# mierl/rootless-coll-mpi-ops

Measured on AMD Instinct MI355X. Metric: rootless bcast msgs/s, higher is better.
Workload: dtype u8; 1 GPU; rootless bcast storm over one world of 256 workgroup-ranks (256 per GPU), 64 B payload, random originators, 262144 bcasts per step; value = rootless bcasts/s, each delivered to all 255 other ranks; ranks_per_gpu=256, world_ranks=256, payload_bytes=64, waves_per_rank=8, parallelism=one world sharded over 1 GPU(s), contiguous rank ranges

## Files before the change

include/rlo_hip.h:

```cpp
#ifndef RLO_HIP_H
#define RLO_HIP_H
#include <stddef.h>
#include <stdint.h>

#ifdef __cplusplus
extern "C" {
#endif

#define RLO_OK 0
#define RLO_E_INVAL (-1)
#define RLO_E_HIP (-2)
#define RLO_E_OCCUPANCY (-3)
#define RLO_E_DEVICE (-4)
#define RLO_E_NOPROGRAM (-5)
#define RLO_E_NODEVICE (-6)
#define RLO_E_NOTCONNECTED (-7)
#define RLO_E_AGAIN (-8)
#define RLO_E_TIMEOUT (-9)
#define RLO_E_STALE (-10)

#define RLO_DERR_TIMEOUT 1
#define RLO_DERR_VOTE_RING 2
#define RLO_DERR_PID_COLLISION 3
#define RLO_DERR_VOTE_ORPHAN 4
#define RLO_DERR_LOG_FULL 5
#define RLO_DERR_BAD_SLOT 6
#define RLO_DERR_HOST_CMD 7
#define RLO_DERR_BULK 8
#define RLO_DERR_XCD 9

int rlo_topology(int n, int rank, int* level, int* last_wall, int* send_channel_cnt, int* send_list_len,
                 int* send_list );
int rlo_children(int n, int rank, int origin, int from , int* out );

typedef struct rlo_world rlo_world_t;

typedef struct {
    int32_t n_ranks;
    uint32_t max_payload;
    uint32_t ring_slots;
    int32_t device;
    uint64_t bulk_max;
    uint32_t bulk_slots;
    uint32_t movers;
    uint32_t proposal_pool;
    uint32_t flags;
} rlo_world_cfg_t;

typedef struct {
    int32_t n_ranks, max_in_degree, max_fanout, edges;
    uint32_t ring_slots, slot_stride, vote_slots;
    uint32_t peers;
    uint64_t fwd_bytes, vote_bytes, ctrl_bytes;
    int32_t cus, blocks_per_cu;
    int32_t part, n_parts, rank_begin, rank_end;
    int32_t sys_scope;
    int32_t waves;
    uint32_t bulk_slots, movers;
    uint64_t bulk_max, heap_bytes;
    uint32_t proposal_pool;
    uint32_t pull;
    uint32_t nsmall;
    uint32_t stage2_bytes;
    uint32_t ll_ok;
    uint32_t pend_hbm;
    uint32_t dyn_lds, static_lds;
    uint32_t last_kernel;
    uint32_t info_pad;
} rlo_world_info_t;

int rlo_world_create(const rlo_world_cfg_t* cfg, rlo_world_t** out);

#define RLO_PART_BLOB_BYTES 512u
#define RLO_PEER_OTHER_GPU 1u
#define RLO_PEER_IMPORTED 2u
#define RLO_PART_UNCACHED 1u
#define RLO_PART_PEND_HBM 4u
#define RLO_PART_ONE_XCD 8u
#define RLO_PART_CHUNKED 2u
typedef struct {
    int32_t n_ranks;
    int32_t n_parts, part;
    const int32_t* part_begin;
    uint32_t max_payload, ring_slots;
    int32_t device;
    uint32_t flags;
    uint64_t bulk_max;
    uint32_t bulk_slots, movers;
    uint32_t proposal_pool, pad;
} rlo_part_cfg_t;
int rlo_part_create(const rlo_part_cfg_t* cfg, rlo_world_t** out);
int rlo_part_export(rlo_world_t* w, void* blob, uint32_t cap);
int rlo_part_connect(rlo_world_t* w, const void* blobs , int n_parts);
int rlo_part_import(rlo_world_t* w, const void* blob , int q);
int rlo_world_destroy(rlo_world_t* w);
int rlo_part_close_imports(rlo_world_t* w);
int rlo_world_query(const rlo_world_t* w, rlo_world_info_t* out);

#define RLO_TRIM_IMPORTS 1u
#define RLO_TRIM_FREE 2u
#define RLO_TRIM_RETIRED 4u
#define RLO_TRIM_EXPORTED 8u
int rlo_pool_trim(uint32_t what, uint64_t* freed_bytes);
int rlo_pool_stats(uint64_t* out, uint32_t cap);

#define RLO_FLAG_LOG 1u
#define RLO_FLAG_HIST 2u
#define RLO_FLAG_PROF 4u
#define RLO_FLAG_TIMELINE 8u

#define RLO_ORDER_RANDOM 0u
#define RLO_ORDER_SLOTS 1u
typedef struct {
    uint64_t seed;
    int64_t k;
    uint32_t len;
    uint32_t window;
    uint32_t flags;
    uint32_t log_cap;
    uint32_t len_max;
    uint32_t order;
// ... 30 lines not shown
} rlo_log_rec_t;

typedef struct {
    uint32_t cmd_slots;
    uint32_t pickup_slots;
    uint32_t idle_timeout_s;
    uint32_t flags;
    uint32_t pool;
    uint32_t pad;
} rlo_host_cfg_t;
int rlo_program_host(rlo_world_t* w, const rlo_host_cfg_t* cfg);

#define RLO_CMD_BCAST 0u
#define RLO_CMD_PROPOSAL 2u
#define RLO_CMD_JUDGE 16u
#define RLO_CMD_OWN_JUDGE 17u
#define RLO_CMD_QUIT 18u
#define RLO_CMD_BULK 10u
#define RLO_CMD_BULK_RELEASE 19u
typedef struct {
    uint32_t kind;
    int32_t origin;
    int32_t id;
    uint32_t pseq;
    int32_t vote;
    uint32_t pad;
} rlo_cmd_t;
int rlo_host_post(rlo_world_t* w, int rank, const rlo_cmd_t* cmd, const void* payload, uint32_t len);

#define RLO_EV_DELIVER_BCAST (1u | (0u << 8))
#define RLO_EV_DELIVER_DECISION (1u | (4u << 8))
#define RLO_EV_DELIVER_BULK (1u | (10u << 8))
#define RLO_EV_ACTION 3u
#define RLO_EV_RESULT 4u
#define RLO_EV_JUDGE 6u
#define RLO_EV_OWN_JUDGE 7u
#define RLO_EV_JUDGED 8u
int rlo_host_poll(rlo_world_t* w, int rank, rlo_log_rec_t* ev, void* payload, uint32_t cap);
int rlo_host_running(rlo_world_t* w);
int rlo_host_cmd_count(rlo_world_t* w, int rank, uint64_t* consumed, uint64_t* posted);
int rlo_device_count(void);
int rlo_device_numa_node(int device);

typedef struct { uint32_t nchunks, stripe, chunk, tile, total_tiles, direct; } rlo_bulk_plan_t;
int rlo_bulk_plan(int n, uint64_t len, int cross, rlo_bulk_plan_t* out);
typedef struct {
    int32_t n_ranks, n_parts, part;
    uint32_t max_payload, ring_slots, flags;
    uint64_t bulk_max;
    uint32_t bulk_slots, movers, proposal_pool;
    int32_t cus;
} rlo_plan_cfg_t;
int rlo_layout_plan(const rlo_plan_cfg_t* cfg, rlo_world_info_t* out);
int rlo_storm_lengths(uint64_t seed, uint64_t k, uint32_t len, uint32_t len_max, uint32_t* out);
int rlo_host_bulk_stage(rlo_world_t* w, int rank, const void* data, uint64_t len, uint32_t timeout_us, uint32_t* q);
int rlo_host_bulk_copy(rlo_world_t* w, int rank, const rlo_log_rec_t* ev, void* dst);

int rlo_host_share(rlo_world_t* w, const char* shm_name, uint64_t stage_bytes);
int rlo_host_unlink(rlo_world_t* w);
int rlo_host_proxy(rlo_world_t* w);
int rlo_host_wait_started(rlo_world_t* w, uint32_t timeout_ms);
int rlo_host_fail(rlo_world_t* w);
int rlo_host_device_judge(rlo_world_t* w, const rlo_iar_cfg_t* cfg);

typedef struct rlo_client rlo_client_t;
int rlo_client_attach(const char* shm_name, int rank, rlo_client_t** out);
int rlo_client_detach(rlo_client_t* c);
int rlo_client_state(rlo_client_t* c);
int rlo_client_post(rlo_client_t* c, const rlo_cmd_t* cmd, const void* payload, uint32_t len);
int rlo_client_poll(rlo_client_t* c, rlo_log_rec_t* ev, void* payload, uint32_t cap);
int rlo_client_cmd_count(rlo_client_t* c, uint64_t* consumed, uint64_t* posted);
int rlo_client_bulk_put(rlo_client_t* c, const void* data, uint64_t len, uint32_t timeout_us, uint32_t* q);
int rlo_client_bulk_get(rlo_client_t* c, const rlo_log_rec_t* ev, void* dst);
int rlo_client_debug(rlo_client_t* c, uint64_t* out);
int rlo_client_hdiag(rlo_client_t* c, uint64_t* out);
int rlo_client_fwd(rlo_client_t* c, uint64_t* fwd, int64_t* fwd_ns);

int rlo_reset(rlo_world_t* w, void* stream);
#define RLO_LAUNCH_NO_RESET 1u
int rlo_launch_ex(rlo_world_t* w, void* stream, uint32_t flags);
int rlo_launch(rlo_world_t* w, void* stream);
int rlo_stream_create(int device, void** stream);
int rlo_stream_destroy(void* stream);
int rlo_wait(rlo_world_t* w);
int rlo_run(rlo_world_t* w, void* stream, float* kernel_ms);
int rlo_last_kernel_ms(rlo_world_t* w, float* ms);

typedef struct {
    uint64_t bcast_delivered, bcast_sum, originated;
    uint64_t dec_delivered, dec_approved, actions, judge_calls;
    uint64_t own_decided, own_approved, proposals_recv;
    uint64_t iterations, busy_iterations, stalls, log_count;
    uint64_t t_start, t_end;
    uint32_t error, error_aux;
    uint64_t prof[8];
    uint64_t dbg[8];
    uint32_t hist[128];
    uint64_t unmarked_slots;
} rlo_rank_stats_t;


int rlo_stats(rlo_world_t* w, rlo_rank_stats_t* out, int n);
int rlo_log(rlo_world_t* w, int rank, rlo_log_rec_t* out, uint32_t cap, uint8_t* payload, uint32_t payload_stride);
int rlo_latencies(rlo_world_t* w, uint64_t* ticks, uint32_t cap);
int rlo_round_ticks(rlo_world_t* w, uint64_t* ticks, uint32_t cap);

int rlo_device_error(rlo_world_t* w, uint32_t* code, uint32_t* aux);
int rlo_bulk_debug(rlo_world_t* w, uint64_t* out, uint32_t cap);
const char* rlo_strerror(int code);
int rlo_last_hip_error(void);

#ifdef __cplusplus
}
#endif
#endif
```

rootless-coll-mpi-ops_amd/csrc/rlo_device.hpp:

```cpp
#pragma once
#include <stdint.h>

namespace rlo {

constexpr int kBlock = 256;
constexpr int kWaves = kBlock / 64;
constexpr int kMaxFanout = 16;
constexpr int kMaxIn = 32;
constexpr int kMaxOut = 2 * kMaxFanout;
constexpr int kHdr = 16;
constexpr int kVoteSlot = 16;
constexpr int kMaxCand = 256;
constexpr int kStagePasses = 4;
constexpr int kHistBins = 128;
constexpr int kMaxParts = 64;
constexpr int kPoolMax = 16;
constexpr int kCtrlHdrWords = 16;
constexpr int kCtrlNonceWord = 15;
constexpr uint32_t kTlRoundsMax = 64, kTlGlobal = 8, kTlCols = 9;
enum TlCol : uint32_t { TLC_ARRIVE = 0, TLC_DONE = 1, TLC_PARENT = 2, TLC_ISSUE = 3, TLC_PASS = 4,
                        TLC_FWD = 5,
                        TLC_NEXT = 6,
                        TLC_P1 = 7, TLC_P2 = 8 };
enum TlEvent : uint32_t { TL_ORIGIN = 0, TL_POSTED = 1, TL_CLAIMED = 2, TL_MOVED = 3, TL_ROUND = 4, TL_VERIFIED = 5,
                          TL_GEN = 6, TL_DRAINED = 7 };
constexpr int kLatCap = 8192;
constexpr int kLatWords = 16 + kLatCap / 2;

enum Tag : uint32_t { TAG_BCAST = 0, TAG_PROPOSAL = 2, TAG_VOTE = 3, TAG_DECISION = 4, TAG_BULK = 10 };

enum Mode : uint32_t {
    MODE_STORM = 1u,
    MODE_LAT = 2u,
    MODE_IAR = 4u,
    MODE_LOG = 16u,
    MODE_HIST = 32u,
    MODE_PROF = 64u,
    MODE_LAZYPUB = 256u,
    MODE_NOSPIN = 512u,
    MODE_NOACQ = 1024u,
    MODE_NOFAST = 2048u,
    MODE_HDIAG = 4096u,
    MODE_PIPE = 8192u,
    MODE_LL = 16384u,
    MODE_TL = 32768u,
    MODE_HOPPROF = 131072u,
    MODE_NOHPW = 262144u,
    MODE_XCD1 = 524288u,
    MODE_CORRUPT = 65536u,
    MODE_HOST = 128u,
};

enum HostCmd : uint32_t { CMD_JUDGE = 16, CMD_OWN_JUDGE = 17, CMD_QUIT = 18, CMD_BULK_RELEASE = 19 };
constexpr int kHctlWords = 64;
constexpr int kHctlInjTail = 0, kHctlInjHead = 16, kHctlPkTail = 32, kHctlPkHead = 48;
constexpr int kHctlState = 40;
constexpr int kHctlDiag = 20;
constexpr int kHctlBeat = 41;

enum Judge : uint32_t { JUDGE_APPROVE = 0, JUDGE_MASK = 1, JUDGE_ISP = 2, JUDGE_HASH = 3 };

enum LogKind : uint32_t { LOG_DELIVER = 1, LOG_JUDGE = 2, LOG_ACTION = 3, LOG_RESULT = 4, LOG_ERROR = 5,
                          LOG_JREQ = 6,
                          LOG_OWN_JREQ = 7,
                          LOG_JUDGED = 8 };

enum Err : uint32_t { ERR_NONE = 0, ERR_TIMEOUT = 1, ERR_VOTE_RING = 2, ERR_PID_COLLISION = 3, ERR_VOTE_ORPHAN = 4,
                      ERR_LOG_FULL = 5, ERR_BAD_SLOT = 6, ERR_HOST_CMD = 7,
                      ERR_BULK = 8, ERR_XCD = 9 };


struct RankTopo {
    int32_t level, last_wall, scc, sll;
    int32_t send_list[kMaxFanout];
    int32_t n_in;
    int32_t in_src[kMaxIn];
    uint32_t in_data[kMaxIn][2];
    uint32_t vin_data[kMaxFanout];
    uint32_t inbox_ctrl, n_inbox;
    uint32_t outbox_ctrl, n_outbox;
    uint64_t out_ring[kMaxFanout][2];
    uint64_t out_tail[kMaxFanout][2];
    uint64_t in_head[kMaxIn][2];
    uint64_t vout_ring[kMaxIn];
    uint64_t vout_tail[kMaxIn];
    uint64_t vin_head[kMaxFanout];
    uint64_t in_base[kMaxIn];
    uint32_t orig_data, orig_pad;
    uint32_t in_bell, vin_bell;
    uint64_t out_bell[kMaxFanout];
    uint64_t vout_bell[kMaxIn];
};

constexpr uint32_t kBellChunks = 8;
__host__ __device__ inline uint32_t bell_tag(uint64_t s) { return ((uint32_t)s & 0x3fffffffu) + 1u; }
constexpr uint32_t kBellWords = 2 * kBellChunks * 2;

struct RankStats {
    uint64_t bcast_delivered, bcast_sum, originated;
    uint64_t dec_delivered, dec_approved, actions, judge_calls;
    uint64_t own_decided, own_approved, proposals_recv;
    uint64_t iterations, busy_iterations, stalls, log_count;
    uint64_t t_start, t_end;
    uint32_t error, error_aux;
    uint64_t prof[8];
    uint64_t dbg[8];
    uint32_t hist[kHistBins];
    uint64_t unmarked_slots;
};

constexpr uint32_t kPkRecBytes = 32, kPkMaxSlots = 16384, kPkNoPayload = 0xffffu, kPkTaggedPayload = 0x8000u;
__host__ __device__ inline uint32_t pk_tag(uint64_t seq, uint32_t epoch) { return (((uint32_t)seq << 1) | 1u) ^ epoch; }
__host__ __device__ inline uint32_t pk_tag16(uint64_t seq, uint32_t epoch) { return pk_tag(seq, epoch) & 0xffffu; }
__host__ __device__ inline uint32_t pk_payload_stride(uint32_t max_payload) { return max_payload >= 256u ? max_payload : 256u; }

struct LogRec {
    uint32_t kind;
    int32_t origin;
    int32_t from;
    uint32_t id;
    uint32_t len;
    int32_t vote;
    uint32_t aux;
    uint32_t payload_idx;
};

struct Params {
    int32_t n, rank_begin, rank_end;
    uint32_t mode;
    const RankTopo* topo;
    uint8_t* fwd_region;
    uint32_t fwd_region_bytes;
    uint32_t fwd_cap, fwd_stride;
    uint8_t* vote_region;
    uint32_t vote_region_bytes;
    uint32_t vote_cap;
    uint64_t* ctrl;
    uint32_t ctrl_bytes;
    uint32_t sys_scope;
    uint32_t n_parts;
    uint32_t* err_flag[kMaxParts];
    uint64_t seed;
    uint32_t len, window;
    const int64_t* sched_off;
    const uint32_t* sched_ids;
    const int64_t* expect_bcast;
    uint32_t lat_rounds;
    const int32_t* lat_origin;
    uint32_t* lat_count;
    uint64_t* lat_out;
    uint32_t* lat_round;
    uint32_t* xcd_word;
    uint64_t* lat_obs;
    uint32_t* tl;
    uint32_t tl_rounds;
    const uint32_t* lat_own_off;
    const uint32_t* lat_own;
    uint32_t judge_kind, judge_ppm;
    uint64_t judge_seed;
    const uint8_t* judge_mask;
    const char* judge_isp;
// ... 171 lines not shown
```

rootless-coll-mpi-ops_amd/csrc/rlo_kernel.hip:

```cpp
#include <hip/hip_runtime.h>

#include <type_traits>

#include "rlo_kernel_common.hpp"

namespace rlo {

struct CandL {
    uint32_t w0, id, w2, t0;
    uint32_t src;
    uint32_t need;
    uint32_t logidx;
    uint32_t kind, group;
    uint32_t relay;
};

struct PostReq {
    uint32_t cls, kind, origin, lr, slot, bid, len, ntiles, from, logidx, q, gen;
    uint64_t j0;
};
constexpr uint32_t kPostQ = 16;
struct BulkSh {
    PostReq pq[kPostQ];
    uint32_t npost;
    BulkJob mv_job;
    uint32_t mv_ti, mv_stop;
    unsigned long long mv_sum;
    uint32_t bq[kPass];
    uint32_t blen[kPass];
    uint32_t bact[kMaxPend];
    uint32_t nbact, ncomp;
    uint64_t fbase, dbase;
    uint32_t nstable;
    uint64_t cmask[kMaxPend / 64];
    uint32_t bonw[kMaxPend / 32];
    uint64_t sdone[8];
    uint32_t bulk_q;
};
struct NoBulkSh {};
struct BulkPend {
    uint32_t bid, len, ntiles;
    int32_t from;
    uint32_t t0, q, pad0, pad1;
};

template <int W, bool BULK>
struct Shared {
    typename std::conditional<BULK, BulkSh, NoBulkSh>::type b;
    static constexpr int kWaves = W, kMaxCand = 64 * W;
    RankTopo t;
    uint64_t ring_head[2 * kMaxIn];
    uint32_t ring_base[2 * kMaxIn], ring_take[2 * kMaxIn];
    uint64_t ract;
    uint64_t out_tail0[kMaxOut];
    uint32_t ofree[kMaxOut];
    uint32_t n_oi[kMaxOut];
    uint32_t R, C, nstorm, storm_base, loc_kind, lat_id, exit_now;
    uint32_t hbase, nh, ev_n, quit, gap_lo, gap_hi, nchmax;
    uint64_t hhead, hin_head, pk_tail;
    int64_t prop_idx;
    uint32_t storm_ids[kPass];
    uint64_t vhead[kMaxFanout];
    uint32_t vbase[kMaxFanout], va[kMaxFanout], vtot;
    uint32_t wcnt[kWaves][kMaxOut];
    uint32_t first_bad[kGroups];
    CandL cand[kMaxCand];
    alignas(16) uint16_t pos[kMaxCand][kMaxFanout];
    uint16_t big[kMaxCand];
    uint32_t nbig, bm, bq0, nblk;
    uint32_t blk_c[128], blk_q0[128];
    uint32_t nblk2[2];
    uint64_t vout_tail[kMaxIn], vout_head[kMaxIn];
    uint64_t pubw[4][64], snap[4][64];
    int32_t own_pid[kPoolMax];
    uint32_t own_word[kPoolMax], own_state[kPoolMax], own_decision[kPoolMax];
    uint32_t own_needed, own_rr;
    unsigned long long own_iter;
    int64_t own_n;
    uint32_t loc_nd, loc_n;
    uint8_t loc_slot[2 * kPoolMax];
    uint32_t lat_pos, lat_pos_n, lat_own_next, lat_seen, error, error_aux, progressed;
    uint32_t hwait;
    uint64_t hp[2];
    uint32_t a_done, cseq;
    uint64_t hd[8], hd_t0;
    uint64_t relay_tail, relay_rel;
    uint32_t relay_n, ref_any, rq_n, rq_h, relay_free;
    uint64_t rq_relay[kRelQ];
    uint64_t rq_out[kRelQ][kMaxOut];
    unsigned long long bcast_delivered, dec_delivered, dec_approved, actions, judge_calls, originated;
    unsigned long long own_decided, own_approved, proposals_recv, log_count, stalls, stale;
    uint64_t prof[8], prof_t, dbg[8];
    uint64_t hpt[9];
    uint32_t tl_clk[4];
    uint32_t tl_bfid;
    int64_t expect_dec;
    uint32_t hist[kHistBins];
};



// ... 518 lines not shown
                }
                for (int sh = 32; sh >= 1; sh >>= 1) acc += __shfl_xor(acc, sh);
                if ((tid & 63) == 0) atomicAdd((unsigned long long*)&S.mv_sum, acc);
            }
        }
        if (tid == 0) atomicAdd((unsigned long long*)&P.jctl[kJctlTilesDone + cls], (unsigned long long)jb.ntiles);
        if (jb.kind == JOB_VERIFY) {
            __syncthreads();
            if (tid == 0) {
                const uint32_t ps = jb.parent;
                (void)__hip_atomic_fetch_add(&P.jsum[cls * P.jslots + ps], (uint64_t)S.mv_sum, __ATOMIC_RELAXED,
                                             __HIP_MEMORY_SCOPE_AGENT);
                S.mv_sum = 0;
                __builtin_amdgcn_fence(__ATOMIC_RELEASE, "agent");
                asm volatile("s_waitcnt vmcnt(0)" ::: "memory");
                const uint32_t old = atomicAdd(&P.jdone[cls * P.jslots + ps], jb.ntiles);
                if (old + jb.ntiles == jb.total) {
                    __builtin_amdgcn_fence(__ATOMIC_ACQUIRE, "agent");
                    const uint64_t part = __hip_atomic_load(&P.jsum[cls * P.jslots + ps], __ATOMIC_RELAXED,
                                                            __HIP_MEMORY_SCOPE_AGENT);
                    const uint64_t tot = part + chunk_mix(0xFFFFFFFFu, u32x4{(uint32_t)o, jb.bid, TAG_BCAST, len});
                    atomicAdd((unsigned long long*)&P.stats[jb.lr].bcast_sum, (unsigned long long)tot);
                    if (jb.logidx != ~0u)
                        st_sys16(reinterpret_cast<u32x4*>(&P.log[(size_t)jb.lr * P.log_cap + jb.logidx]) + 1,
                                 u32x4{len, 0xffffffffu, (uint32_t)tot, (uint32_t)(tot >> 32)});
                    const uint32_t nt = n > 2 ? bulk_stripe_tiles(pl, len, (uint32_t)((me - o - 1 + n) % n)) : 0u;
                    bulk_slot_release(P, me, o, s, sys, bulk_total_tiles(pl, len) + nt, jb.bid);
                    tl_mark(P, jb.bid, TL_VERIFIED);
                    __hip_atomic_store(&P.jdone[cls * P.jslots + ps], 0u, __ATOMIC_RELAXED, __HIP_MEMORY_SCOPE_AGENT);
                    __hip_atomic_store(&P.jsum[cls * P.jslots + ps], 0ull, __ATOMIC_RELAXED, __HIP_MEMORY_SCOPE_AGENT);
                    __builtin_amdgcn_fence(__ATOMIC_RELEASE, "agent");
                    asm volatile("s_waitcnt vmcnt(0)" ::: "memory");
                    __hip_atomic_store(&P.jfree[cls * P.jslots + ps], (uint64_t)(jb.pjob >> lg) + 1ull, __ATOMIC_RELAXED,
                                       __HIP_MEMORY_SCOPE_AGENT);
                }
            }
        }
        BAR();
    }
}


constexpr uint32_t kPmAll = 0xFFFFFFFFu;
constexpr uint32_t kPmLat = ~(uint32_t)(MODE_STORM | MODE_IAR | MODE_HOST);
constexpr uint32_t kPmIar = ~(uint32_t)(MODE_STORM | MODE_LAT | MODE_HOST);
constexpr uint32_t kPmStorm = ~(uint32_t)(MODE_LAT | MODE_IAR | MODE_HOST);
constexpr uint32_t kPmHost = ~(uint32_t)(MODE_STORM | MODE_LAT);

template <int W, bool BULK, bool LL, bool PH = false, uint32_t PM = kPmAll>
__global__ __launch_bounds__(64 * W) void rlo_progress_kernel(Params P) {
#define PMODE(x) ((PM & (uint32_t)(x)) ? (P.mode & (uint32_t)(x)) : 0u)
#define PULL_ON (W == 4 && !BULK && P.pull != 0u)
    constexpr int kWaves = W, kBlock = 64 * W, kMaxCand = 64 * W;
    constexpr uint32_t kHostBase = kMaxCand - kPass;
    extern __shared__ __attribute__((aligned(16))) uint8_t dyn_lds[];
    __shared__ Shared<W, BULK> S;
    if constexpr (BULK) {
        if (blockIdx.x >= P.n_local) {
            if (threadIdx.x == 0) S.b.mv_sum = 0;
            __syncthreads();
            mover_run<W>(P, S, (int)threadIdx.x);
            return;
        }
    }
    const uint32_t nsmall = P.nsmall;
    const uint32_t nmagic = nsmall > 1 ? 0xFFFFFFFFu / nsmall + 1u : 0u;
    const uint32_t pend_bytes = P.pend_hbm ? 0u : 16u * (uint32_t)P.n * P.pend_slots;
    PendState* pend;
    if constexpr (PH)
        pend = (PendState*)(__attribute__((address_space(1))) PendState*)(P.pend_hbm + (size_t)blockIdx.x * (uint32_t)P.n * P.pend_slots);
    else
        pend = reinterpret_cast<PendState*>(dyn_lds);
    uint16_t* olist = reinterpret_cast<uint16_t*>(dyn_lds + pend_bytes);
    uint8_t* stage = dyn_lds + pend_bytes + P.nout_max * (2u * kMaxCand);
    uint8_t* stage2 = stage + (uint32_t)kMaxCand * nsmall * 16u;
    constexpr uint32_t kSubMax = W == 4 ? 4u : 1u;
    constexpr uint32_t kPair = W == 4 ? 2u : 1u;

    const uint32_t s2_units = P.stage2_bytes >> 10;
#define STG(c, q) (stage + (((uint32_t)(c) * nsmall + (uint32_t)(q)) << 4))
#define OL(oi, r) olist[(uint32_t)(oi) * (uint32_t)kMaxCand + (uint32_t)(r)]
#define PEND(o, q) pend[(uint32_t)(o) * P.pend_slots + ((uint32_t)(q) & (P.pend_slots - 1u))]

    const int lr = blockIdx.x;
    const int me = P.rank_begin + lr;
    const int tid = threadIdx.x, w = tid >> 6;
    int lane = tid & 63;
    uint64_t lt_mask = (1ull << lane) - 1ull;
    const __amdgpu_buffer_rsrc_t rf = mk_rsrc(P.fwd_region, P.fwd_region_bytes);
    const __amdgpu_buffer_rsrc_t rv = mk_rsrc(P.vote_region, P.vote_region_bytes);
    const uint32_t fcap_m = P.fwd_cap - 1, vcap_m = P.vote_cap - 1;
    const bool host = PM == kPmHost || (PMODE(MODE_HOST)) != 0;
    const bool eager = host || !(PMODE(MODE_LAZYPUB | MODE_STORM));
    const bool hjudge = host && P.host_judge != 0;
    const uint32_t my_mask = ((PMODE(MODE_IAR)) && !hjudge && P.judge_kind == JUDGE_MASK) ? P.judge_mask[me] : 0u;
    const __amdgpu_buffer_rsrc_t rh =
        mk_rsrc(host ? P.hin + (size_t)lr * P.hin_cap * P.fwd_stride : P.fwd_region, host ? P.hin_cap * P.fwd_stride : 16u);
    uint64_t* const hctl = host ? P.hctl + (size_t)lr * kHctlWords : nullptr;
    uint64_t* const hctl_dev = host ? P.hctl_dev + (size_t)lr * kHctlWords : nullptr;
    const uint32_t hcap_m = host ? P.hin_cap - 1u : 0u;
    constexpr uint32_t kLLCmdSlotB = kBellChunks * 32u;
    const __amdgpu_buffer_rsrc_t rll = mk_rsrc(host && P.hll ? P.hll + (size_t)lr * P.hin_cap * kLLCmdSlotB : P.fwd_region,
                                               host && P.hll ? P.hin_cap * kLLCmdSlotB : 16u);
    const bool ll_cmds = host && (uint32_t)kMaxCand * nsmall * 16u >= kLLCmdBell + 256u;
    [[maybe_unused]] BulkPend* const bpend = reinterpret_cast<BulkPend*>(dyn_lds + (BULK ? P.bpend_off : 0u));
    [[maybe_unused]] const uint32_t bsl = BULK ? P.bulk_slots : 1u;

    {
        const uint32_t* src = reinterpret_cast<const uint32_t*>(&P.topo[lr]);
        uint32_t* dst = reinterpret_cast<uint32_t*>(&S.t);
        for (int i = tid; i < (int)(sizeof(RankTopo) / 4); i += kBlock) dst[i] = src[i];
        if (PH || !P.pend_hbm)
            for (int i = tid; i < P.n * (int)P.pend_slots; i += kBlock) pend[i] = PendState{0, 0, 0, 0, 0, 0};
        if constexpr (BULK) {
            for (int i = tid; i < P.n * (int)P.bulk_slots; i += kBlock) bpend[i] = BulkPend{0u, 0u, 0u, -1, 0u, 0u, 0u, 0u};
        }
        for (int i = tid; i < kHistBins; i += kBlock) S.hist[i] = 0;
        for (int i = tid; i < 4 * 64; i += kBlock) { (&S.pubw[0][0])[i] = 0; (&S.snap[0][0])[i] = 0; }
        if (tid < kMaxIn) { S.vout_tail[tid] = 0; S.vout_head[tid] = 0; }
        if (tid < 8) { S.prof[tid] = 0; S.dbg[tid] = 0; S.hd[tid] = 0; }
        if (tid == 0) S.tl_bfid = 0;
        if (tid == 0) {
            S.prof_t = __builtin_amdgcn_s_memtime();
            for (int k = 0; k < kPoolMax; k++) {
                S.own_pid[k] = -1;
                S.own_word[k] = 0; S.own_state[k] = 0; S.own_decision[k] = 0;
            }
            S.own_needed = 0; S.own_rr = 0; S.loc_nd = 0; S.loc_n = 0;
            S.own_iter = 0;
            S.own_n = ((PMODE(MODE_IAR)) && !host) ? (P.prop_off[lr + 1] - P.prop_off[lr]) : 0;
            S.lat_pos = 0;
            S.lat_seen = 0;
            S.lat_pos_n = (PMODE(MODE_LAT)) ? P.lat_own_off[lr + 1] - P.lat_own_off[lr] : 0u;
            S.lat_own_next = S.lat_pos_n ? P.lat_own[P.lat_own_off[lr]] : 0xffffffffu;
            S.expect_dec = ((PMODE(MODE_IAR)) && !host) ? P.expect_dec[lr] : 0;
            S.hbase = 0; S.nh = 0; S.ev_n = 0; S.quit = 0; S.hhead = 0; S.hin_head = 0; S.pk_tail = 0;
            S.bcast_delivered = S.dec_delivered = S.dec_approved = S.actions = S.judge_calls = S.originated = 0;
            S.own_decided = S.own_approved = S.proposals_recv = S.log_count = S.stalls = S.stale = 0;
            S.error = 0; S.error_aux = 0; S.exit_now = 0; S.progressed = 0; S.hd_t0 = 0; S.hwait = 0;
            S.hp[0] = 0; S.hp[1] = 0; S.a_done = 0; S.cseq = 0;
            S.relay_tail = 0; S.relay_rel = 0; S.relay_n = 0; S.ref_any = 0; S.rq_n = 0; S.rq_h = 0; S.relay_free = 0;
            if constexpr (BULK) {
                S.b.nbact = 0; S.b.ncomp = 0; S.b.bulk_q = 0; S.b.nstable = 0; S.b.npost = 0;
                S.b.fbase = reinterpret_cast<uint64_t>(bulk_flags(P, me, 0, 0));
                S.b.dbase = reinterpret_cast<uint64_t>(bulk_done(P, me, 0u));
                for (int i = 0; i < kMaxPend / 64; i++) S.b.cmask[i] = 0;
                for (int i = 0; i < kMaxPend / 32; i++) S.b.bonw[i] = 0;
            }
        }
    }
    if constexpr (PH) VM_DRAIN();
    BAR();
    if (host && tid == 0) pub64_sys(&hctl[kHctlState], 1ull);
    if (!PH && P.pend_hbm && (PMODE(MODE_IAR | MODE_HOST)) && tid == 0) set_error(S, P, ERR_HOST_CMD, 0x9E4Du);
    const uint64_t t_start = now_ticks();
    unsigned long long acc_sum = 0;

    const RankTopo& t = S.t;
    const int level = uni(t.level), last_wall = uni(t.last_wall), scc = uni(t.scc), sll = uni(t.sll);
    const int n_in = uni(t.n_in), n_in2 = 2 * n_in, nout = 2 * sll;
    const uint32_t inbox = (uint32_t)uni((int)t.inbox_ctrl), outbox = (uint32_t)uni((int)t.outbox_ctrl);
    const uint32_t sl_r = lane < sll ? (uint32_t)t.send_list[lane] : 0u;
    const bool sys = P.sys_scope != 0;
    const uint32_t oring_bytes = P.fwd_cap * P.fwd_stride;
#define OTPTR t.out_tail[lane >> 1][lane & 1]
#define IHPTR t.in_head[lane >> 1][lane & 1]
#define VHPTR t.vin_head[lane]
#define VTPTR t.vout_tail[lane]
#define ORING(oi) uni64(t.out_ring[(oi) >> 1][(oi) & 1])
    uint64_t in_head_r = 0, out_tail_r = 0, vin_head_r = 0;
#define PUB_IN S.pubw[0][lane]
#define PUB_OUT S.pubw[1][lane]
#define PUB_VIN S.pubw[2][lane]
#define PUB_VOUT S.pubw[3][lane]
    uint32_t win_r = kMaxCand;
    uint64_t hpoll = 0;
    bool peer_failed = false;
    uint64_t idle_since = 0;
    uint32_t idle_n = 0;
    bool idle_prev = false;
    uint64_t p_h = 0;
    uint32_t p_lat = 0;
    const int64_t sched_base = (PMODE(MODE_STORM)) ? P.sched_off[lr] : 0;
    const int64_t sched_n = (PMODE(MODE_STORM)) ? P.sched_off[lr + 1] - sched_base : 0;
    const int64_t expect_bcast = (PMODE(MODE_STORM | MODE_LAT)) ? P.expect_bcast[lr] : 0;
    int64_t sched_next = 0;
    uint64_t n_iter = 0, n_busy = 0, n_stalls = 0;
    bool done_w0 = false;
    uint32_t rbase_r = 0, rtake_r = 0, noi_r = 0;
    const bool llm = LL && (PMODE(MODE_LL)) && !(PMODE(MODE_PROF | MODE_NOFAST));
    const bool hpw = W == 4 && host && llm && ll_cmds && P.hll != nullptr && !(P.mode & MODE_NOHPW);
    uint32_t a_it = 0;
    const __amdgpu_buffer_rsrc_t rc = mk_rsrc(P.ctrl, P.ctrl_bytes);
    const uint32_t in_bell = (uint32_t)uni((int)t.in_bell), vin_bell = (uint32_t)uni((int)t.vin_bell);
    bool ll_prog = false;

#define KIDS_U(o, f) (PM != kPmAll ? kids_of_u(me, (o), (f), level, last_wall, scc, sll, sl_r, lane) \
                               : kids_of(me, (o), (f), level, last_wall, scc, sll, sl_r))
#define NEED_U(k, o) (PM != kPmAll ? need_of_u((k), (o), sll, sl_r, lane) : need_of((k), (o), sll, sl_r))
    auto fwd_small = [&](u32x4 v, uint32_t nch, uint32_t need) {
        const uint32_t q = (uint32_t)lane;
        uint64_t obase = 0, bbase = 0;
        if constexpr (PM != kPmAll) {
            if (lane < nout) {
                obase = t.out_ring[lane >> 1][lane & 1];
                if (LL && llm) bbase = t.out_bell[lane >> 1];
            }
        }
        for (uint32_t m = need; m; m &= m - 1) {
            const int oi = __builtin_ctz(m);
            const uint64_t slot = rdl64(out_tail_r, oi);
            const __amdgpu_buffer_rsrc_t ro =
                mk_rsrc(reinterpret_cast<void*>(PM != kPmAll ? rdl64(obase, oi) : ORING(oi)), oring_bytes);
            if (q < nch) st_ring(ro, (uint32_t)(slot & fcap_m) * P.fwd_stride + 16u * q, v, sys);
            if (LL && llm && nch <= kBellChunks && q < nch) {
                const uint32_t T = bell_tag(slot) | ((uint32_t)(oi & 1) << 31);
                const __amdgpu_buffer_rsrc_t rb = mk_rsrc(
// ... 554 lines not shown

    auto lat_observe = [&](uint32_t latr) {
        const uint32_t done_r = rdl32(latr, 1), seen = S.lat_seen;
        if (done_r > seen) {
            const uint64_t tn = now_ticks();
            for (uint32_t k = seen + (uint32_t)lane; k < done_r && k < P.lat_rounds; k += 64u) P.lat_obs[k] = tn;
            if (lane == 0) S.lat_seen = done_r;
        }
    };

    auto bulk_eval = [&]() -> bool {
        bool any = false;
        if constexpr (BULK) {
            const uint32_t nb = (uint32_t)uni((int)S.b.nbact);
            if (TL_ON(P) && lane == 0) S.tl_clk[1] = (uint32_t)now_ticks();
            const __amdgpu_buffer_rsrc_t rfl = mk_rsrc(reinterpret_cast<void*>(uni64(S.b.fbase)), (uint32_t)P.n * bsl * kBulkLine);
            for (uint32_t u = 0; u * 64u < nb; u++) {
                const uint32_t i = u * 64u + (uint32_t)lane;
                bool dn = false;
                if (i < nb) {
                    const uint32_t e = S.b.bact[i];
                    uint32_t tc = 0;
                    if (e >= (uint32_t)P.n * bsl) {
                        bulk_fault(P, 7, e);
                    } else if (P.bulk_cross) {
                        tc = bflag_ld(reinterpret_cast<uint32_t*>(uni64(S.b.fbase) + (uint64_t)e * kBulkLine) + kBulkTflag, sys);
                    } else {
                        u32x4 q[4];
#pragma unroll
                        for (int k = 0; k < 4; k++) q[k] = sys ? ld_sys(rfl, e * kBulkLine + 16u * k) : ld_sc1(rfl, e * kBulkLine + 16u * k);
#pragma unroll
                        for (int k = 0; k < 4; k++) tc += q[k].x + q[k].y + q[k].z + q[k].w;
                    }
                    dn = e < (uint32_t)P.n * bsl && tc >= bpend[e].ntiles;
                    if (TL_ON(P) && dn) {
                        tl_put(P, bpend[e].bid, TLC_PASS, lr, (uint32_t)now_ticks());
                        tl_put(P, bpend[e].bid, TLC_ISSUE, lr, S.tl_clk[1]);
                    }
                }
                const uint64_t m = __ballot(dn);
                any |= m != 0ull;
                if (lane == 0) S.b.cmask[u] = m;
            }
            if (lane == 0) S.b.nstable = nb;
        }
        return any;
    };

    for (;;) {
        asm volatile("" : "+v"(lane));
        lt_mask = (1ull << lane) - 1ull;
        a_it++;
        uint64_t in_tail_r = 0, out_head_r = 0, vin_tail_r = 0, vout_head_r = 0;
        uint32_t errf = 0, sid = 0, latr = 0;
        if (w == 0) {
            uint32_t ll_run = 0;
            bool bev = false;
            uint64_t dnw = 0;
            for (uint32_t sp = 0;; sp++) {
                bev = false;
                if (hpw) {
                    if (lane < 2) hpoll = S.hp[lane];
                } else if (host && lane < 2 && ((sp & 3u) == 0u || S.hwait != 0u)) {
                    hpoll = poll64_sys(&hctl_dev[lane == 0 ? kHctlInjTail : kHctlPkHead]);
                }
                if (TL_ON(P) && lane == 0) {
                    S.tl_clk[0] = (uint32_t)now_ticks();
                    if (BULK && S.tl_bfid) { tl_put(P, S.tl_bfid - 1u, TLC_NEXT, lr, S.tl_clk[0]); S.tl_bfid = 0; }
                }
                [[maybe_unused]] u32x4 ba, bb, vb;
                if constexpr (LL) {
                    const uint32_t bk = (uint32_t)lane >> 3, bq = (uint32_t)lane & 7u;
                    const uint32_t bo = llm && (int)bk < n_in ? (in_bell + bk * kBellWords) * 8u + 32u * bq : kOob;
                    ba = ld_sc1(rc, bo);
                    bb = ld_sc1(rc, bo == kOob ? kOob : bo + 16u);
                    vb = ld_sc1(rc, llm && lane < sll ? (vin_bell + 2u * (uint32_t)lane) * 8u : kOob);
                }
                in_tail_r = ld64_sc1(rc, lane < n_in2 ? (inbox + (uint32_t)lane) * 8u : kOob);
                vin_tail_r = ld64_sc1(rc, lane < sll ? (inbox + (uint32_t)(n_in2 + lane)) * 8u : kOob);
                out_head_r = ld64_sc1(rc, lane < nout ? (outbox + (uint32_t)lane) * 8u : kOob);
                vout_head_r = ld64_sc1(rc, lane < n_in ? (outbox + (uint32_t)(nout + lane)) * 8u : kOob);
                errf = ld32_sc1(rc, 0u);
                if constexpr (BULK) {
                    const __amdgpu_buffer_rsrc_t rd = mk_rsrc(reinterpret_cast<void*>(uni64(S.b.dbase)), bsl * kBulkLine);
                    dnw = ld64_sys(rd, lane < (int)bsl ? (uint32_t)lane * kBulkLine : kOob);
                }
                if constexpr ((PM & MODE_LAT) != 0u)
                    latr = __hip_atomic_load((PMODE(MODE_LAT)) ? P.lat_round : P.error_flag, __ATOMIC_RELAXED,
                                             __HIP_MEMORY_SCOPE_SYSTEM);
                if constexpr (LL) {
                    if (llm) {
                        if ((PMODE(MODE_LAT)) && me == 0) lat_observe(latr);
                        bool need_full = false;
                        const uint32_t nb0 = nact_of(S.b);
                        const uint32_t nll = ll_pass(ba, bb, vb, in_tail_r, vin_tail_r, out_head_r, hpoll, latr, errf, need_full);
                        if (nll) ll_prog = true;
                        if (need_full) { SPIN_WHY(2); break; }
                        if (BULK && nact_of(S.b) != nb0) { SPIN_WHY(3); break; }
                        if (nll) {
                            if (++ll_run < 64u) { sp = 0; continue; }
                            SPIN_WHY(3);
                            break;
                        }
                    }
                }
                if ((PMODE(MODE_LAT)) && me == 0 && !(LL && llm)) lat_observe(latr);
                if (!idle_prev || sp >= kIdleSpin) { SPIN_WHY(idle_prev ? 1 : 0); break; }
                bool bmoved = false;
                if constexpr (BULK) {
                    if (uni((int)S.b.npost) != 0) { SPIN_WHY(4); break; }
                    if (uni((int)S.b.nbact) != 0) {
                        bev = true;
                        if (bulk_eval()) { SPIN_WHY(5); break; }
                    }
                    bmoved = lane < (int)bsl && dnw != S.b.sdone[lane];
                }
                const bool moved =
                    llm ? (in_tail_r != S.snap[0][lane] && in_tail_r > in_head_r) ||
                              (vin_tail_r != S.snap[1][lane] && vin_tail_r > vin_head_r) ||
                              (latr != p_lat && rdl32(latr, 1) == S.lat_own_next) || errf != 0
                        : in_tail_r != S.snap[0][lane] || vin_tail_r != S.snap[1][lane] || out_head_r != S.snap[2][lane] ||
                              vout_head_r != S.snap[3][lane] || hpoll != p_h || latr != p_lat || errf != 0 || bmoved;
                if (__ballot(moved)) { SPIN_WHY(6); break; }
            }
            if (hpw && lane == 0) S.a_done = a_it;
            S.snap[0][lane] = in_tail_r; S.snap[1][lane] = vin_tail_r; S.snap[2][lane] = out_head_r;
            S.snap[3][lane] = vout_head_r; p_h = hpoll; p_lat = latr;
            if (host && (n_iter & 4095u) == 0 && lane < 3) pub64_sys(&hctl[kHctlBeat + lane], lane == 2 ? n_iter : hpoll);
            if constexpr (BULK) {
                if (lane < (int)bsl) S.b.sdone[lane] = dnw;
                if (!bev) (void)bulk_eval();
            }
            if ((PMODE(MODE_LAT)) && me == 0) lat_observe(latr);
            if ((PMODE(MODE_STORM)) && sched_next + lane < sched_n && (uint32_t)lane < P.window)
                sid = P.sched_ids[sched_base + sched_next + lane];
        } else if (hpw && w == 1) {
            for (;;) {
                const uint64_t hh = uni64(S.hin_head);
                const uint8_t* slot = reinterpret_cast<const uint8_t*>(
                    uni64(reinterpret_cast<uint64_t>(P.hll + ((uint64_t)lr * P.hin_cap + (hh & hcap_m)) * kLLCmdSlotB)));
                su16 sa;
                uint64_t ht = 0, hk = 0;
                u32x4 cv = {0u, 0u, 0u, 0u};
                uint32_t scov = 2u;
                if constexpr (PM == kPmHost) {
                    su16 sb;
                    su8 sc;
                    spoll_cmd5(slot, &hctl_dev[kHctlInjTail], &hctl_dev[kHctlPkHead], sa, sb, sc, ht, hk);
#pragma unroll
                    for (int p = 0; p < 4; p++) {
                        if (lane == p) cv = u32x4{sa[4 * p], sa[4 * p + 1], sa[4 * p + 2], sa[4 * p + 3]};
                        if (lane == 4 + p) cv = u32x4{sb[4 * p], sb[4 * p + 1], sb[4 * p + 2], sb[4 * p + 3]};
                    }
                    if (lane == 8) cv = u32x4{sc[0], sc[1], sc[2], sc[3]};
                    if (lane == 9) cv = u32x4{sc[4], sc[5], sc[6], sc[7]};
                    scov = 5u;
                } else {
                    spoll_cmd(slot, &hctl_dev[kHctlInjTail], &hctl_dev[kHctlPkHead], sa, ht, hk);
#pragma unroll
                    for (int p = 0; p < 4; p++)
                        if (lane == p) cv = u32x4{sa[4 * p], sa[4 * p + 1], sa[4 * p + 2], sa[4 * p + 3]};
                }
                if (lane == 0) { S.hp[0] = ht; S.hp[1] = hk; }
                {
                    const uint32_t T0 = bell_tag(hh);
                    const bool head_ok = sa[1] == T0 && sa[3] == T0 && sa[5] == T0 && sa[7] == T0;
                    if (head_ok && ((kHdr + (sa[4] & 0xffffu) + 15u) >> 4) > scov && lane >= (int)(2u * scov) && lane < 16)
                        cv = ld_sys(rll, (uint32_t)(hh & hcap_m) * kLLCmdSlotB + 16u * (uint32_t)lane);
                }
                const uint32_t T = bell_tag(hh);
                const uint64_t tok = __ballot(lane < 16 && cv.y == T && cv.w == T);
                const uint32_t cn = (kHdr + (rdl32(cv.x, 1) & 0xffffu) + 15u) >> 4;
                const uint64_t cm = (1ull << (2u * min(cn, kBellChunks))) - 1ull;
                if ((tok & 3ull) == 3ull && cn <= kBellChunks && (tok & cm) == cm &&
                    (uint32_t)uni((int)S.cseq) != T) {
                    if (lane == 0) *lds_word(&S.cseq) = 0u;
                    asm volatile("s_waitcnt lgkmcnt(0)" ::: "memory");
                    if (lane < 16)
                        *lds_dword(stage + kLLCmdBell + 8u * (uint32_t)lane) = (uint64_t)cv.x | ((uint64_t)cv.z << 32);
                    asm volatile("s_waitcnt lgkmcnt(0)" ::: "memory");
                    if (lane == 0) *lds_word(&S.cseq) = T;
                }
                if (__builtin_amdgcn_readfirstlane((int)S.a_done) == (int)a_it) break;
            }
        }
        VM_DRAIN();
        BAR();
        PROF_STAMP(0);

        if (w == 0) {
            if (lane < nout && out_tail_r != PUB_OUT) { PUB_OUT = out_tail_r; pub64(OTPTR, out_tail_r, sys); }
            if (lane < n_in2 && in_head_r != PUB_IN) { PUB_IN = in_head_r; pub64(IHPTR, in_head_r, sys); }
            if (lane < sll && vin_head_r != PUB_VIN) { PUB_VIN = vin_head_r; pub64(VHPTR, vin_head_r, sys); }
            if (lane < n_in) {
                const uint64_t vt = S.vout_tail[lane];
                if (vt != PUB_VOUT) { PUB_VOUT = vt; pub64(VTPTR, vt, sys); }
                S.vout_head[lane] = vout_head_r;
            }
            peer_failed = __builtin_amdgcn_readfirstlane(errf) != 0;
            PSX(1);
            uint32_t relay_free = kMaxCand;
            if (PULL_ON) {
                const uint32_t nq = S.rq_n;
                uint32_t nrel = 0, e = S.rq_h;
                uint64_t rel = S.relay_rel;
                for (; nrel < nq; nrel++, e = (e + 1u) % (uint32_t)kRelQ) {
                    const bool ok = lane >= nout || out_head_r >= S.rq_out[e][lane];
                    if (__ballot(!ok)) break;
                    rel = S.rq_relay[e];
                }
                if (lane == 0 && nrel) { S.rq_h = e; S.rq_n = nq - nrel; S.relay_rel = rel; }
                const uint64_t used = S.relay_tail - rel;
                relay_free = used >= P.relay_cap ? 0u : P.relay_cap - (uint32_t)used;
                if (lane == 0) S.relay_free = relay_free;
            }
            bool hblock = false;
            uint32_t hlim = kMaxCand;
            if (host) {
                if (lane == 0) pub64_sys(&hctl[kHctlInjHead], S.hin_head);
                if (lane == 1) pub64_sys(&hctl[kHctlPkTail], S.pk_tail);
                const uint64_t pk_head = rdl64(hpoll, 1);
                const uint32_t pk_free = P.log_cap - (uint32_t)(S.pk_tail - pk_head);
                const uint32_t own_ev = 2u * P.own_pool + 2u;
                hblock = pk_free < own_ev + 4u;
                hlim = hblock ? 0u : (pk_free - own_ev) / 2u;
                if ((PMODE(MODE_HDIAG)) && lane == 0) {
                    S.hd[3]++;
                    if (hblock) S.hd[2]++;
                }
            }
            if constexpr (BULK) {
                const uint32_t nb = S.b.nbact;
                const uint32_t nst = S.b.nstable;
                if (nb) {
                    uint32_t climit = kMaxPend;
                    if (host) {
                        const uint32_t pk_free = P.log_cap - (uint32_t)(S.pk_tail - rdl64(hpoll, 1));
                        climit = pk_free >= 24u ? (pk_free - 16u) / 2u : 0u;
                    }
                    uint32_t seen = 0, kept = 0;
                    for (uint32_t u = 0; u * 64u < nb; u++) {
                        const uint32_t i = u * 64u + (uint32_t)lane;
                        const uint64_t m = S.b.cmask[u];
                        const uint64_t mv = u * 64u < nst ? m & (nst - u * 64u >= 64u ? ~0ull : ((1ull << (nst - u * 64u)) - 1ull)) : 0ull;
                        bool fin = ((mv >> lane) & 1ull) && seen + (uint32_t)__popcll(mv & lt_mask) < climit;
// ... 204 lines not shown
                    nh = run;
                    gap_lo = C;
                    hbase = kHostBase + ncp;
                    if ((uint32_t)lane >= ncp && (uint32_t)lane < ncp + nh) {
                        S.cand[kHostBase + lane].src = (uint32_t)((S.hin_head + lane) & hcap_m) * P.fwd_stride;
                        S.cand[kHostBase + lane].group = kGroupLocal + K_HOST;
                    }
                    if (lane == 0) { S.hhead = S.hin_head + ncp; S.hin_head += ncp; }
                    if (nh) C = hbase + nh;
                }
            }
            if (!LL && (PMODE(MODE_STORM)) && sched_next < sched_n) {
                const bool deep = lane < nout && (out_tail_r - out_head_r) * 2 >= P.fwd_cap;
                const bool allow = !backlog && R < 2 * kPass && __ballot(deep) == 0;
                if ((PMODE(MODE_PROF)) && lane == 0) { if (!allow) S.dbg[5]++; else S.dbg[2]++; }
                if (allow) {
                    const int64_t rem = sched_n - sched_next;
                    uint32_t ww = rem < (int64_t)P.window ? (uint32_t)rem : P.window;
                    if (ww > kMaxCand - C) ww = kMaxCand - C;
                    if constexpr (BULK) {
                        uint32_t ln = 0, isb = 0;
                        if ((uint32_t)lane < ww) {
                            ln = P.len_hi > P.len_lo ? storm_len_of(P.seed, sid, P.len_lo, P.len_hi) : P.len;
                            isb = ln > P.ring_cap ? 1u : 0u;
                        }
                        uint32_t nbk = 0;
                        const uint32_t q = S.b.bulk_q + wave_excl_scan(isb, &nbk);
                        const bool ok = !isb || S.b.sdone[q & (bsl - 1u)] >= (uint64_t)(q / bsl) * (uint64_t)(P.n - 1);
                        const uint64_t bad = __ballot((uint32_t)lane < ww && !ok);
                        if (bad) ww = (uint32_t)__builtin_ctzll(bad);
                        if (bad && lane == 0) atomicAdd((unsigned long long*)&P.jctl[kJctlSlotWaits], 1ull);
                        if ((uint32_t)lane < ww) {
                            S.b.bq[lane] = isb ? q : ~0u;
                            S.b.blen[lane] = ln;
                        }
                    }
                    storm_base = C;
                    nstorm = ww;
                    C += ww;
                    if ((uint32_t)lane < ww) S.storm_ids[lane] = sid;
                }
            }
            if ((PMODE(MODE_LAT)) && C < kMaxCand) {
                bool lat_ok = true;
                if constexpr (BULK) {
                    if (P.len > P.ring_cap) {
                        const uint32_t q = S.b.bulk_q;
                        lat_ok = S.b.sdone[q & (bsl - 1u)] >= (uint64_t)(q / bsl) * (uint64_t)(P.n - 1);
                    }
                }
                if (lat_ok && S.lat_own_next != 0xffffffffu && rdl32(latr, 1) == S.lat_own_next) { lat_id = S.lat_own_next; C++; }
            }
            uint32_t fastdone = 0;
            if ((!host || hlim >= 2u) && R == 1u && C == 1u && vtot == 0u && !(PMODE(MODE_PROF | MODE_NOFAST))) {
                const int fg = __builtin_ctzll(__ballot(lane < n_in2 && take > 0u));
                const uint64_t h0 = rdl64(in_head_r, fg);
                const uint32_t fsrc = (uint32_t)uni((int)t.in_data[fg >> 1][fg & 1]) + (uint32_t)(h0 & fcap_m) * P.fwd_stride;
                u32x4 v = {0u, 0u, 0u, 0u};
                if ((uint32_t)lane < nsmall) v = ld_sc1(rf, fsrc + 16u * (uint32_t)lane);
                const uint32_t fneed = lone(v, fg, fsrc, false, out_head_r);
                if (fneed == kHeld || fneed == kAsked) {
                    VM_DRAIN();
                    if (lane == fg) rtake_r = 0u;
                    R = 0;
                    C = 0;
                    fastdone = fneed == kAsked ? 1u : 0u;
                } else if (fneed != ~0u) {
                    VM_DRAIN();
                    noi_r = lane < nout ? ((fneed >> lane) & 1u) : 0u;
                    R = 0;
                    C = 0;
                    fastdone = 1;
                }
            }
            if (lane == 0) {
                S.ract = ract;
                S.vtot = vtot;
                S.R = R; S.C = C; S.nstorm = nstorm; S.storm_base = storm_base; S.loc_kind = loc_kind;
                S.lat_id = lat_id; S.prop_idx = prop_idx; S.nbig = 0; S.progressed = fastdone | (ll_prog ? 1u : 0u);
                S.hbase = hbase; S.nh = nh; S.gap_lo = gap_lo; S.gap_hi = hbase; S.nchmax = 0;
                S.exit_now = done_w0;
                if (PMODE(MODE_PROF)) S.dbg[0] += R;
            }
            ll_prog = false;
        }
        BAR();
        PST(7, 3);
        if (S.exit_now) {
            if constexpr (BULK) {
                if (w == 0) flush_posts(S.b, P, lane);
            }
            break;
        }
        const uint32_t R = S.R, C = S.C;
        const uint32_t nstorm = S.nstorm, storm_base = S.storm_base, loc_kind = S.loc_kind;

        if (C != 0 || S.vtot != 0) {
            const uint32_t vtot = S.vtot;
            u32x4 vreg[4] = {{0u, 0u, 0u, 0u}, {0u, 0u, 0u, 0u}, {0u, 0u, 0u, 0u}, {0u, 0u, 0u, 0u}};
            if (w == 1 && vtot) {
    #pragma unroll
                for (int u = 0; u < 4; u++) {
                    const uint32_t i = (uint32_t)u * 64u + lane;
                    if (i < vtot) {
                        int j = 0;
                        while (i >= S.vbase[j] + S.va[j]) j++;
                        const uint64_t slot = S.vhead[j] + (i - S.vbase[j]);
// ... 266 lines not shown
                    const uint32_t x = S.wcnt[v][lane];
                    if (v < w) pre += x;
                    tot += x;
                }
                const uint32_t f = S.ofree[lane];
                room_r = f > pre ? f - pre : 0u;
                tight_l = tot > f;
            }
            bool fits = active && judge >= 0;
            for (uint32_t m = wneed & (uint32_t)__ballot(tight_l); m; m &= m - 1) {
                const int oi = __builtin_ctz(m);
                const bool bit = (need >> oi) & 1u;
                const uint64_t b = __ballot(bit);
                if (b && bit && (uint32_t)__popcll(b & lt_mask) >= rdl32(room_r, oi)) {
                    fits = false;
                    if ((PMODE(MODE_PROF | MODE_HIST)) == MODE_PROF) atomicAdd(&S.hist[oi], 1u);
                }
            }
            if (active && !fits) atomicMin(&S.first_bad[group], c);
            BAR();
            const bool admitted = active && fits && c < S.first_bad[group];
            const uint32_t an = admitted ? need : 0u;
            const uint32_t len = w2 & 0xffffu;
            const bool isbig = admitted && ((kHdr + len + 15u) >> 4) > nsmall;
            const uint32_t nch_s = (kHdr + len + 15u) >> 4;
            const uint32_t wadm = wave_or(an);
            for (uint32_t m = wave_or(active && !admitted ? need : 0u); m; m &= m - 1) {
                const int oi = __builtin_ctz(m);
                const uint64_t b = __ballot((an >> oi) & 1u);
                if (lane == 0) S.wcnt[w][oi] = (uint32_t)__popcll(b);
            }
            {
                const uint32_t mx = wave_max(admitted && !isbig ? (kHdr + len + 15u) >> 4 : 0u);
                if (lane == 0 && mx) atomicMax(&S.nchmax, mx);
            }
            BAR();
            uint32_t pre_r = 0;
            if (lane < nout) {
                uint32_t tot = 0;
                for (int v = 0; v < kWaves; v++) {
                    const uint32_t x = S.wcnt[v][lane];
                    if (v < w) pre_r += x;
                    tot += x;
                }
                if (w == 0) { S.n_oi[lane] = tot; noi_r = tot; }
            }
            for (uint32_t m = wadm; m; m &= m - 1) {
                const int oi = __builtin_ctz(m);
                const bool bit = (an >> oi) & 1u;
                const uint64_t b = __ballot(bit);
                if (bit) {
                    const uint32_t rel = rdl32(pre_r, oi) + (uint32_t)__popcll(b & lt_mask);
                    OL(oi, rel) = (uint16_t)(c | (isbig ? kBigFlag : (nch_s << 9)));
                    if (isbig) S.pos[c][oi >> 1] = (uint16_t)rel;
                }
            }
            const uint64_t amask = __ballot(admitted);
            PST(3, 7);

            const uint32_t tag = (w0 >> 16) & 0xffu;
            const int vote = (int)(int8_t)(w0 >> 24);
            const uint32_t pseq = w2 >> 24;
            uint32_t logidx = ~0u;
            bool lat_deliv = false;
            uint32_t lat_tn = 0;
            if (admitted) {
                if (kind == K_RING) {
                    if (tag == TAG_BCAST) {
                        if (PMODE(MODE_HIST | MODE_LAT)) {
                            const uint64_t tn = now_ticks();
                            if (PMODE(MODE_HIST)) atomicAdd(&S.hist[hist_bin((uint32_t)tn - t0)], 1u);
                            if (PMODE(MODE_LAT)) {
                                tl_mark(P, id, kTlGlobal + (uint32_t)lr);
                                tl_parent(P, id, lr, from);
                                lat_deliv = true;
                                lat_tn = (uint32_t)tn - t0;
                            }
                        }
                        logidx = log_put<PM>(S, P, lr, LOG_DELIVER | (TAG_BCAST << 8), origin, from, id, len, -1,
                                         (uint32_t)now_ticks() - t0);
                    } else if (tag == TAG_PROPOSAL) {
                        const int32_t pid = (int32_t)id;
                        const int k = (int)(group >> 1);
                        atomicAdd(&S.proposals_recv, 1ull);
                        if (own_has(S, P, pid)) {
                            set_error(S, P, ERR_PID_COLLISION, (uint32_t)pid);
                        } else {
                            atomicAdd(&S.judge_calls, 1ull);
                            if (!host) log_put<PM>(S, P, lr, LOG_JUDGE, origin, from, (uint32_t)pid, len, judge, 0);
                            else if (!hjudge) {
                                const uint32_t slot = log_put<PM>(S, P, lr, LOG_JUDGED, origin, from, (uint32_t)pid, len, judge,
                                                              pseq);
                                uint8_t* dst = P.log_payload + ((size_t)lr * P.log_cap + slot) * P.log_stride;
                                for (uint32_t q = 0; 16u * q < len && 16u * q < P.log_stride; q++)
                                    st_sys16(dst + 16u * q, ld_sc1(rf, src + kHdr + 16u * q));
                            }
                            PendState* ps = &PEND(origin, pseq);
                            if (!judge) {
                                ps->valid = PS_NONE;
                                emit_vote<LL>(S, P, me, (uint32_t)k, origin, pid, pseq, 0);
                            } else {
                                const uint32_t nk = (uint32_t)__builtin_popcount(kids);
                                ps->pid = pid;
                                ps->word = 0;
                                ps->parent_k = (uint16_t)k;
                                ps->needed = (uint8_t)nk;
                                ps->pseq = pseq | ((len - 16u) << 8);
// ... 187 lines not shown
                    if (cl.kind == K_RING) {
                        if (PULL_ON && ((cl.w2 >> 16) & 0xffu) == kRefMark) {
                            const u32x4 ref = *reinterpret_cast<const u32x4*>(STG(cc, 1));
                            const uint32_t roff = (uint32_t)uni((int)ref.x);
                            const bool rok = uni((int)ref.y) == (int)~roff && (uint32_t)uni((int)ref.z) == kRefMagic;
                            if (!rok && lane == 0) set_error(S, P, ERR_BAD_SLOT, 0x5EF0000u | (pq & 0xffffu));
                            const __amdgpu_buffer_rsrc_t rr =
                                mk_rsrc(reinterpret_cast<void*>(uni64(t.in_base[cl.group >> 1]) + roff),
                                        (uint32_t)uni((int)(rok ? (pch + 1u) * 16u : 0u)));
                            if (rok && pq < pch) {
                                if (sys) __builtin_amdgcn_raw_ptr_buffer_load_lds(rr, lds_ptr(dst), 16, 16u * (pq + 1u), 0, 0, kAuxSc1 | 1);
                                else __builtin_amdgcn_raw_ptr_buffer_load_lds(rr, lds_ptr(dst), 16, 16u * (pq + 1u), 0, 0, kAuxSc1);
                            }
                        } else if (pq < pch) {
                            dma16(rf, dst, cl.src + 16u * (pq + 1u));
                        }
                    } else if (cl.kind == K_HOST) {
                        if (pq < pch)
                            __builtin_amdgcn_raw_ptr_buffer_load_lds(rh, lds_ptr(dst), 16, cl.src + 16u * (pq + 1u), 0, 0, kAuxSc1 | 1);
                    } else if (pq < pch) {
                        *reinterpret_cast<u32x4*>(dst + 16u * lane) =
                            gen_chunk(P, cl.kind, me, cl.id, cl.w2 & 0xffffu, cl.src, (int)(int8_t)(cl.w0 >> 24), pq + 1u);
                    }
                    }
                }
            };
            auto big_drain = [&]() {
                if ((PMODE(MODE_PROF)) && tid == 0) {
                    const uint64_t c0 = __builtin_amdgcn_s_memtime();
                    VM_DRAIN();
                    S.dbg[3] += __builtin_amdgcn_s_memtime() - c0;
                    if (!PULL_ON) S.dbg[4]++;
                } else {
                    VM_DRAIN();
                }
            };
            if (nbig) {
                if (tid == 0) { S.bm = 0; S.bq0 = 0; }
                plan_big(0u);
                BAR();
                issue_big(0u);
                big_drain();
                ACQ_NEXT();
            }

#ifdef RLO_AB_NQ2
            const uint32_t nq = min(max(S.nchmax, 1u), 2u);
#else
            const uint32_t nq = max(S.nchmax, 1u);
#endif
            const uint32_t qmagic = nq > 1 ? 0xFFFFFFFFu / nq + 1u : 0u;
            const uint32_t dr = div_small(64u, qmagic), dq = 64u - dr * nq;
            const uint32_t stg_msg = nsmall << 4, stride = P.fwd_stride;
            const uint32_t nit_r = lane < nout ? S.n_oi[lane] * nq : 0u;
            uint32_t items = 0;
            const uint32_t ibase_r = wave_excl_scan(nit_r, &items);
            const uint32_t lo = items * (uint32_t)w / (uint32_t)kWaves, hi = items * (uint32_t)(w + 1) / (uint32_t)kWaves;
            for (uint64_t mo = __ballot(nit_r != 0 && ibase_r < hi && ibase_r + nit_r > lo); mo; mo &= mo - 1) {
                const int oi = __builtin_ctzll(mo);
                const uint32_t ib = rdl32(ibase_r, oi), ie = ib + rdl32(nit_r, oi);
                const uint32_t a = max(lo, ib) - ib, b = min(hi, ie) - ib;
                const uint32_t s0 = (uint32_t)S.out_tail0[oi];
                const __amdgpu_buffer_rsrc_t ro = mk_rsrc(reinterpret_cast<void*>(ORING(oi)), oring_bytes);
                uint32_t i = a + (uint32_t)lane;
                uint32_t r = div_small(i, qmagic), q = i - r * nq;
                for (; i < b; i += 256u) {
                    uint32_t rr[4], qq[4], e[4];
                    rr[0] = r;
                    qq[0] = q;
#pragma unroll
                    for (int u = 1; u < 4; u++) {
                        rr[u] = rr[u - 1] + dr;
                        qq[u] = qq[u - 1] + dq;
                        if (qq[u] >= nq) { qq[u] -= nq; rr[u]++; }
                    }
#pragma unroll
                    for (int u = 0; u < 4; u++) e[u] = i + 64u * u < b ? (uint32_t)OL(oi, rr[u]) : (uint32_t)kBigFlag;
                    u32x4 x[4];
#pragma unroll
                    for (int u = 0; u < 4; u++) {
                        const bool v = !(e[u] & kBigFlag) && qq[u] < ((e[u] >> 9) & 0x3fu);
                        x[u] = u32x4{0u, 0u, 0u, 0u};
                        if (v) x[u] = *reinterpret_cast<const u32x4*>(stage + __umul24(e[u] & 0x1ffu, stg_msg) + (qq[u] << 4));
                        e[u] = v ? 1u : 0u;
                    }
#pragma unroll
                    for (int u = 0; u < 4; u++)
                        if (e[u]) st_ring(ro, __umul24((s0 + rr[u]) & fcap_m, stride) + (qq[u] << 4), x[u], sys);
                    r = rr[3] + dr;
                    q = qq[3] + dq;
                    if (q >= nq) { q -= nq; r++; }
                }
            }
            if (admitted && !isbig && kind == K_RING && tag == TAG_BCAST) {
                const uint32_t nch = (kHdr + len + 15u) >> 4;
                acc_sum += chunk_mix(0xFFFFFFFFu, u32x4{(uint32_t)origin, id, TAG_BCAST, len});
                for (uint32_t q = 1; q < nch; q++) {
                    const u32x4 v = *reinterpret_cast<const u32x4*>(STG(c, q));
                    acc_sum += chunk_mix(q - 1u, v);
                    if (logidx != ~0u)
                        st_sys16(P.log_payload + ((size_t)lr * P.log_cap + logidx) * P.log_stride + 16u * (q - 1), v);
                }
            }


            if (nbig) {
                constexpr bool kRegs = W == 4;
                const uint32_t ot0_r = kRegs && lane < nout ? (uint32_t)S.out_tail0[lane] : 0u;
                const uint64_t oring_r = kRegs && lane < nout ? t.out_ring[lane >> 1][lane & 1] : 0ull;
#define G3_SLOT(oi) (kRegs ? rdl32(ot0_r, oi) + rdl32(posr, (oi) >> 1) : (uint32_t)S.out_tail0[oi] + S.pos[cc][(oi) >> 1])
#define G3_RING(oi) (kRegs ? rdl64(oring_r, oi) : ORING(oi))
                uint32_t cur = 0;
                for (;;) {
                    const bool more = S.bm < nbig;
                    if (more && pipe) {
                        BAR();
                        plan_big(cur ^ 1u);
                        BAR();
                        issue_big(cur ^ 1u);
                    }
                    const uint32_t nblk = S.nblk2[cur];
                    for (uint32_t b0 = (uint32_t)w; b0 < nblk; b0 += kWaves) {
                        const uint32_t b = cur * hg + b0;
                        const uint32_t cc = S.blk_c[b], qw = S.blk_q0[b], q0b = qw & 0xffffu;
                        const CandL& cl = S.cand[cc];
                        const uint32_t blen = cl.w2 & 0xffffu, pch = (blen + 15u) >> 4;
                        const uint32_t nsub = min(gsub, (pch - q0b + 63u) >> 6);
                        const uint32_t rly = cl.relay;
                        const uint32_t posr = kRegs && lane < sll ? (uint32_t)S.pos[cc][lane] : 0u;
                        const bool hdr = q0b == 0u && lane == 0;
                        const uint32_t hw2 = cl.w2 & 0xff00ffffu;
                        const bool bc = cl.kind == K_RING && ((cl.w0 >> 16) & 0xffu) == TAG_BCAST;
                        if (bc && hdr) acc_sum += chunk_mix(0xFFFFFFFFu, u32x4{cl.w0 & 0xffffu, cl.id, TAG_BCAST, blen});
                        if (PULL_ON && rly != ~0u && q0b == 0u) {
                            const u32x4 hv = lane == 0 ? u32x4{cl.w0, cl.id, hw2 | (kRefMark << 16), cl.t0}
                                                       : u32x4{rly, ~rly, kRefMagic, 0u};
                            for (uint32_t a2 = (uint32_t)uni((int)cl.need); a2; a2 &= a2 - 1) {
                                const int oi = __builtin_ctz(a2);
                                const uint32_t slot = G3_SLOT(oi);
                                const __amdgpu_buffer_rsrc_t ro = mk_rsrc(reinterpret_cast<void*>(G3_RING(oi)), oring_bytes);
                                if (lane <= 1) st_ring(ro, (slot & fcap_m) * P.fwd_stride + 16u * lane, hv, sys);
                            }
                        }
                        for (uint32_t u0 = 0; u0 < nsub; u0 += kPair) {
// ... 16 lines not shown
#pragma unroll
                                    for (uint32_t u = 0; u < kPair; u++)
                                        if (u0 + u < nsub && pq + 64u * u < pch) st_ring(ro, s0 + 16u * (pq + 1u) + 1024u * u, vv[u], sys);
                                    if (hdr && u0 == 0u) st_ring(ro, s0, hv, sys);
                                }
                            }
                            if (bc) {
#pragma unroll
                                for (uint32_t u = 0; u < kPair; u++) {
                                    const uint32_t pp = pq + 64u * u;
                                    if (u0 + u < nsub && pp < pch) {
                                        acc_sum += chunk_mix(pp, vv[u]);
                                        if (cl.logidx != ~0u && 16u * (pp + 1u) <= P.log_stride)
                                            st_sys16(P.log_payload + ((size_t)lr * P.log_cap + cl.logidx) * P.log_stride + 16u * pp, vv[u]);
                                    }
                                }
                            }
                        }
                    }
                    if (!more) break;
                    if (pipe) {
                        cur ^= 1u;
                    } else {
                        BAR();
                        plan_big(cur);
                        BAR();
                        issue_big(cur);
                    }
                    big_drain();
                    ACQ_NEXT();
                }
#undef G3_SLOT
#undef G3_RING
            }
            if (lat_deliv) {
                const uint32_t old = sys ? __hip_atomic_fetch_add(&P.lat_count[id], 1u, __ATOMIC_RELAXED, __HIP_MEMORY_SCOPE_SYSTEM)
                                         : atomicAdd(&P.lat_count[id], 1u);
                if (old + 1u == (uint32_t)(P.n - 1)) {
                    tl_mark(P, id, TL_ROUND);
                    P.lat_out[id] = (uint64_t)lat_tn;
                    if (sys) __hip_atomic_store(P.lat_round, id + 1u, __ATOMIC_RELAXED, __HIP_MEMORY_SCOPE_SYSTEM);
                    else __hip_atomic_store(P.lat_round, id + 1u, __ATOMIC_RELAXED, __HIP_MEMORY_SCOPE_AGENT);
                }
            }
            PST(5, 7);
        }

        if (eager && (C != 0 || S.vtot != 0)) {
            VM_DRAIN();
            BAR();
        }
        if (w == 0) {
            if constexpr (BULK) flush_posts(S.b, P, lane);
            if (lane < n_in2) {
                const uint32_t bse = rbase_r, tk = rtake_r, fb = S.first_bad[lane];
                if (fb < bse + tk) n_stalls++;
                uint32_t adm = fb == 0xffffffffu ? tk : (fb > bse ? fb - bse : 0u);
                if (adm > tk) adm = tk;
                in_head_r += adm;
                if (adm < tk) win_r = max(adm + adm / 2u, 16u);
                else if (adm == tk && tk == win_r) win_r = min(2u * win_r, (uint32_t)kMaxCand);
                if (PMODE(MODE_PROF)) atomicAdd((unsigned long long*)&S.dbg[1], (unsigned long long)adm);
            }
            PSX(4);
            if (eager) {
                if (lane < n_in2 && in_head_r != PUB_IN) { PUB_IN = in_head_r; pub64(IHPTR, in_head_r, sys); }
                if (lane < n_in) {
                    const uint64_t vt = S.vout_tail[lane];
                    if (vt != PUB_VOUT) { PUB_VOUT = vt; pub64(VTPTR, vt, sys); }
                }
            }
            if (lane < nout) {
                out_tail_r += noi_r;
                if (PULL_ON && S.ref_any) {
                    const uint32_t qn = S.rq_n;
                    const uint32_t e = (S.rq_h + (qn == (uint32_t)kRelQ ? qn - 1u : qn)) % (uint32_t)kRelQ;
                    S.rq_out[e][lane] = out_tail_r;
                }
            }
            if (PULL_ON && lane == 0) {
                if (S.ref_any) {
                    const uint32_t qn = S.rq_n;
                    const uint32_t e = (S.rq_h + (qn == (uint32_t)kRelQ ? qn - 1u : qn)) % (uint32_t)kRelQ;
                    S.relay_tail += min(S.relay_n, S.relay_free);
                    S.rq_relay[e] = S.relay_tail;
                    if (qn < (uint32_t)kRelQ) S.rq_n = qn + 1u;
                }
                S.relay_n = 0;
                S.ref_any = 0;
            }
            if (lane < nout) {
                if (eager && out_tail_r != PUB_OUT) { PUB_OUT = out_tail_r; pub64(OTPTR, out_tail_r, sys); }
                if ((PMODE(MODE_PROF | MODE_HIST)) == MODE_PROF) {
                    S.hist[32 + lane] += noi_r;
                    S.hist[64 + lane] += S.ofree[lane] >> 4;
                }
                if (PMODE(MODE_PROF))
                    atomicMax((unsigned long long*)&S.dbg[7], (unsigned long long)(out_tail_r - S.out_tail0[lane] +
                                                                                   (P.fwd_cap - S.ofree[lane])));
            }
            PSX(5);
            if constexpr (BULK) {
                if (nstorm) {
                    const uint32_t fb = S.first_bad[kGroupLocal + K_STORM];
                    uint32_t adm = fb == 0xffffffffu ? nstorm : (fb > storm_base ? fb - storm_base : 0u);
                    if (adm > nstorm) adm = nstorm;
                    const uint64_t bm = __ballot((uint32_t)lane < adm && S.b.bq[lane] != ~0u);
                    if (lane == 0) S.b.bulk_q += (uint32_t)__popcll(bm);
                }
            }
            if (lane == 0) {
                if (nstorm) {
                    const uint32_t fb = S.first_bad[kGroupLocal + K_STORM];
                    uint32_t adm = fb == 0xffffffffu ? nstorm : (fb > storm_base ? fb - storm_base : 0u);
                    if (adm > nstorm) adm = nstorm;
                    sched_next += adm;
                }
                if (host) {
                    if (S.nh) {
                        const uint32_t fb = S.first_bad[kGroupLocal + K_HOST];
                        uint32_t adm = fb == 0xffffffffu ? S.nh : (fb > S.hbase ? fb - S.hbase : 0u);
                        if (adm > S.nh) adm = S.nh;
                        S.hin_head = S.hhead + adm;
                    }
                    if (S.ev_n) {
                        S.pk_tail += S.ev_n;
                        S.log_count += S.ev_n;
                        S.ev_n = 0;
                        pub64_sys(&hctl[kHctlPkTail], S.pk_tail);
                    }
                }
                n_iter++;
                if (S.progressed) {
                    n_busy++;
                    idle_n = 0;
                } else if ((++idle_n & 63u) == 1u) {
                    const uint64_t tn = now_ticks();
                    if (idle_n == 1) idle_since = tn;
                    else if (tn - idle_since > P.timeout_ticks) set_error(S, P, ERR_TIMEOUT, 0);
                }
                if ((n_iter & 1023u) == 0 && now_ticks() - t_start > P.deadline_ticks) set_error(S, P, ERR_TIMEOUT, 1);
                bool done = true;
                if (PMODE(MODE_STORM)) done &= sched_next == sched_n;
                if (PMODE(MODE_STORM | MODE_LAT)) done &= (int64_t)S.bcast_delivered == expect_bcast;
                if (PMODE(MODE_LAT)) done &= S.lat_pos >= S.lat_pos_n;
                if ((PMODE(MODE_IAR)) && !host) {
                    bool idle = true;
                    for (uint32_t k = 0; k < P.pend_slots; k++) idle &= S.own_state[k] == 0u;
                    done &= (int64_t)S.own_iter == S.own_n && idle && (int64_t)S.dec_delivered == S.expect_dec;
                }
                if (host) done = S.quit != 0;
                if (S.error == ERR_TIMEOUT) done = true;
                if (peer_failed) done = true;
                done_w0 = done;
            }
            done_w0 = __builtin_amdgcn_readfirstlane((int)done_w0) != 0;
            sched_next = (int64_t)uni64((uint64_t)sched_next);
            idle_prev = C == 0 && S.vtot == 0 && !done_w0 && !(PMODE(MODE_NOSPIN));
        }
        PROF_STAMP(6);
    }
#undef STG
#undef OL
#undef OTPTR
#undef IHPTR
#undef VHPTR
#undef VTPTR
#undef ORING
#undef PUB_IN
#undef PUB_OUT
#undef PUB_VIN
#undef PUB_VOUT

    if constexpr (BULK) {
        if (tid == 0 && !(P.mode & (MODE_PROF | MODE_TL | MODE_HOPPROF))) {
            const uint32_t nb = S.b.nbact;
            S.dbg[0] = ((uint64_t)S.b.bulk_q << 32) | nb;
            for (uint32_t i = 0; i < 3 && i < nb; i++) {
                const uint32_t e = S.b.bact[i];
                const uint32_t tf = bulk_tcount(P, bulk_flags(P, me, (int)(e / bsl), e % bsl), sys);
                const uint32_t sf = bflag_ld(bulk_flags(P, me, (int)(e / bsl), e % bsl), sys);
                S.dbg[1 + 2 * i] = ((uint64_t)e << 32) | bpend[e].ntiles;
                S.dbg[2 + 2 * i] = ((uint64_t)sf << 32) | tf;
            }
            for (uint32_t i = 0; i < bsl && i < 1; i++) S.dbg[7] = S.b.sdone[0] | (S.b.sdone[bsl > 1 ? 1 : 0] << 32);
        }
    }
    __syncthreads();
    if (w == 0) atomicAdd((unsigned long long*)&S.stalls, (unsigned long long)n_stalls);
    atomicAdd((unsigned long long*)&P.stats[lr].bcast_sum, acc_sum);
    for (int i = tid; i < kHistBins; i += kBlock) P.stats[lr].hist[i] = S.hist[i];
    if (tid < 8) { P.stats[lr].prof[tid] = S.prof[tid]; P.stats[lr].dbg[tid] = S.dbg[tid]; }
    if constexpr (BULK) {
        if (tid == 0) {
            __builtin_amdgcn_fence(__ATOMIC_RELEASE, "agent");
            asm volatile("s_waitcnt vmcnt(0)" ::: "memory");
            atomicAdd((unsigned long long*)&P.jctl[kJctlExited], 1ull);
        }
    }
    if (tid == 0) {
        RankStats& st = P.stats[lr];
        st.bcast_delivered = S.bcast_delivered;
        st.originated = S.originated;
        st.dec_delivered = S.dec_delivered;
        st.dec_approved = S.dec_approved;
        st.actions = S.actions;
        st.judge_calls = S.judge_calls;
        st.own_decided = S.own_decided;
        st.own_approved = S.own_approved;
        st.proposals_recv = S.proposals_recv;
        st.iterations = n_iter;
        st.busy_iterations = n_busy;
        st.stalls = S.stalls;
        st.unmarked_slots = S.stale;
        st.log_count = S.log_count;
        st.t_start = t_start;
        st.t_end = now_ticks();
        st.error = S.error;
        st.error_aux = S.error_aux;
        if (host && (PMODE(MODE_HDIAG)))
            for (int i = 0; i < 8; i++) pub64_sys(&hctl[kHctlDiag + i], S.hd[i]);
        if (host) pub64_sys(&hctl[kHctlState], 2ull);
    }
}

}

template <int W, bool B, bool L, bool H = false, uint32_t PM = rlo::kPmAll>
static hipError_t grant_dyn_lds(size_t dyn_lds) {
    static size_t granted = 0;
    if (dyn_lds > granted) {
        hipError_t e = hipFuncSetAttribute((const void*)rlo::rlo_progress_kernel<W, B, L, H, PM>,
                                           hipFuncAttributeMaxDynamicSharedMemorySize, (int)dyn_lds);
        if (e != hipSuccess) return e;
        granted = dyn_lds;
    }
    return hipSuccess;
}

template <int W, bool B, bool L, bool H = false, uint32_t PM = rlo::kPmAll>
static hipError_t launch_v(const rlo::Params* p, int blocks, size_t dyn_lds, hipStream_t stream) {
    hipError_t e = grant_dyn_lds<W, B, L, H, PM>(dyn_lds);
    if (e != hipSuccess) return e;
    hipLaunchKernelGGL((rlo::rlo_progress_kernel<W, B, L, H, PM>), dim3(blocks), dim3(64 * W), dyn_lds, stream, *p);
    return hipGetLastError();
}

template <int W, bool B, bool L, bool H = false, uint32_t PM = rlo::kPmAll>
static hipError_t occ_one(int* blocks, size_t dyn_lds) {
    hipError_t e = grant_dyn_lds<W, B, L, H, PM>(dyn_lds);
    if (e != hipSuccess) return e;
    return hipOccupancyMaxActiveBlocksPerMultiprocessor(blocks, rlo::rlo_progress_kernel<W, B, L, H, PM>, 64 * W, dyn_lds);
}

template <int W, bool B, bool L, bool H, uint32_t... PMs>
static hipError_t occ_v(int* blocks, size_t dyn_lds) {
    hipError_t e = occ_one<W, B, L, H>(blocks, dyn_lds);
    if (e != hipSuccess) return e;
    const hipError_t es[] = {hipSuccess, [&]() -> hipError_t {
        int b = 0;
        const hipError_t r = occ_one<W, B, L, H, PMs>(&b, dyn_lds);
        if (r == hipSuccess && b < *blocks) *blocks = b;
        return r;
    }()...};
    for (hipError_t x : es)
        if (x != hipSuccess) return x;
    return hipSuccess;
// ... 58 lines not shown
```

rootless-coll-mpi-ops_amd/csrc/rlo_kernel_common.hpp:

```cpp
#pragma once
#include <hip/hip_runtime.h>

#include "rlo_device.hpp"

namespace rlo {

typedef uint32_t u32x4 __attribute__((ext_vector_type(4)));

static constexpr int kAuxSc1 = 16;
static constexpr uint32_t kGolden32 = 0x9E3779B9u;
static constexpr uint64_t kGolden64 = 0x9E3779B97F4A7C15ull;
static constexpr int kPass = 64;
static constexpr uint32_t kIdleSpin = 256;
static constexpr int kRelQ = 16;
static constexpr uint32_t kLLBell = 0, kLLBellVote = 1024, kLLVote = 1152, kLLRing = 2176, kBellJudge = 3328;
static constexpr uint32_t kLLVotes = 4;
static constexpr uint32_t kLLCmd = 4096, kLLCmds = 8;
static constexpr uint32_t kLLCmdBell = 5120;
static constexpr uint32_t kHeld = 0xFFFFFFFEu, kAsked = 0xFFFFFFFDu;

enum CandKind : uint32_t { K_RING = 0, K_STORM = 1, K_PROP = 2, K_DEC = 3, K_LAT = 4, K_HOST = 5, K_BAD = 7 };
enum PendValid : uint8_t { PS_NONE = 0, PS_ACTIVE = 1, PS_JREQ = 2, PS_JYES = 3, PS_JNO = 4 };
static constexpr int kGroupLocal = 2 * kMaxIn;
static constexpr int kGroups = kGroupLocal + 8;
// ... 16 lines not shown
        asm volatile("" ::: "memory");                     \
    } while (0)
#define VM_DRAIN() asm volatile("s_waitcnt vmcnt(0)" ::: "memory")
#define ACQ_NEXT()                                                             \
    do {                                                                       \
        if (!(P.mode & MODE_NOACQ)) asm volatile("buffer_inv sc1" ::: "memory"); \
    } while (0)

__device__ __forceinline__ __amdgpu_buffer_rsrc_t mk_rsrc(void* base, uint32_t bytes) {
    return __builtin_amdgcn_make_buffer_rsrc(base, 0, bytes, 0x00020000);
}
__device__ __forceinline__ u32x4 ld_sc1(__amdgpu_buffer_rsrc_t r, uint32_t off) {
    return __builtin_amdgcn_raw_buffer_load_b128(r, off, 0, kAuxSc1);
}
constexpr uint32_t kOob = 0xFFFFFFF0u;
__device__ __forceinline__ uint64_t ld64_sc1(__amdgpu_buffer_rsrc_t r, uint32_t off) {
    typedef uint32_t u32x2 __attribute__((ext_vector_type(2)));
    const u32x2 v = __builtin_amdgcn_raw_buffer_load_b64(r, off, 0, kAuxSc1);
    return (uint64_t)v.x | ((uint64_t)v.y << 32);
}
__device__ __forceinline__ uint64_t ld64_sys(__amdgpu_buffer_rsrc_t r, uint32_t off) {
    typedef uint32_t u32x2 __attribute__((ext_vector_type(2)));
    const u32x2 v = __builtin_amdgcn_raw_buffer_load_b64(r, off, 0, kAuxSc1 | 1);
    return (uint64_t)v.x | ((uint64_t)v.y << 32);
}
__device__ __forceinline__ uint32_t ld32_sc1(__amdgpu_buffer_rsrc_t r, uint32_t off) {
    return __builtin_amdgcn_raw_buffer_load_b32(r, off, 0, kAuxSc1);
}
__device__ __forceinline__ void st_sc1(__amdgpu_buffer_rsrc_t r, uint32_t off, u32x4 v) {
    __builtin_amdgcn_raw_buffer_store_b128(v, r, off, 0, kAuxSc1);
}
__device__ __forceinline__ uint8_t ld8_sc1(__amdgpu_buffer_rsrc_t r, uint32_t off) {
    return __builtin_amdgcn_raw_buffer_load_b8(r, off, 0, kAuxSc1);
}
__device__ __forceinline__ __attribute__((address_space(3))) void* lds_ptr(uint8_t* p) {
    return (__attribute__((address_space(3))) void*)(p);
}
__device__ __forceinline__ void dma16(__amdgpu_buffer_rsrc_t r, uint8_t* dst, uint32_t off) {
    __builtin_amdgcn_raw_ptr_buffer_load_lds(r, lds_ptr(dst), 16, off, 0, 0, kAuxSc1);
}
__device__ __forceinline__ uint64_t poll64(uint64_t* p) {
    return __hip_atomic_load(p, __ATOMIC_RELAXED, __HIP_MEMORY_SCOPE_AGENT);
}
typedef __attribute__((address_space(1))) uint64_t gu64;
__device__ __forceinline__ gu64* gptr64(uint64_t addr) { return (gu64*)addr; }
__device__ __forceinline__ void pub64(uint64_t addr, uint64_t v, bool sys) {
    gu64* p = gptr64(addr);
    if (sys) __hip_atomic_store(p, v, __ATOMIC_RELAXED, __HIP_MEMORY_SCOPE_SYSTEM);
    else __hip_atomic_store(p, v, __ATOMIC_RELAXED, __HIP_MEMORY_SCOPE_AGENT);
}
__device__ __forceinline__ void st_ring(__amdgpu_buffer_rsrc_t r, uint32_t off, u32x4 v, bool sys) {
    if (sys) __builtin_amdgcn_raw_buffer_store_b128(v, r, off, 0, kAuxSc1 | 1);
    else __builtin_amdgcn_raw_buffer_store_b128(v, r, off, 0, kAuxSc1);
}
__device__ __forceinline__ void st_sys16(void* p, u32x4 v) {
    gu64* q = gptr64(reinterpret_cast<uint64_t>(p));
    __hip_atomic_store(q, (uint64_t)v.x | ((uint64_t)v.y << 32), __ATOMIC_RELAXED, __HIP_MEMORY_SCOPE_SYSTEM);
    __hip_atomic_store(q + 1, (uint64_t)v.z | ((uint64_t)v.w << 32), __ATOMIC_RELAXED, __HIP_MEMORY_SCOPE_SYSTEM);
}
__device__ __forceinline__ u32x4 ld_sys(__amdgpu_buffer_rsrc_t r, uint32_t off) {
    return __builtin_amdgcn_raw_buffer_load_b128(r, off, 0, kAuxSc1 | 1);
}
__device__ __forceinline__ uint64_t poll64_sys(uint64_t* p) {
    return __hip_atomic_load(p, __ATOMIC_RELAXED, __HIP_MEMORY_SCOPE_SYSTEM);
}
typedef uint32_t su16 __attribute__((ext_vector_type(16)));
typedef uint32_t su8 __attribute__((ext_vector_type(8)));
__device__ __forceinline__ void spoll_cmd5(const uint8_t* slot, const uint64_t* w0, const uint64_t* w1, su16& a, su16& b,
                                           su8& c, uint64_t& x0, uint64_t& x1) {
    asm volatile(
        "s_load_dwordx16 %0, %5, 0x0 glc\n\t"
        "s_load_dwordx16 %1, %5, 0x40 glc\n\t"
        "s_load_dwordx8 %2, %5, 0x80 glc\n\t"
        "s_load_dwordx2 %3, %6, 0x0 glc\n\t"
        "s_load_dwordx2 %4, %7, 0x0 glc\n\t"
        "s_waitcnt lgkmcnt(0)"
        : "=&s"(a), "=&s"(b), "=&s"(c), "=&s"(x0), "=&s"(x1)
        : "s"(slot), "s"(w0), "s"(w1)
        : "memory");
}
__device__ __forceinline__ void spoll_cmd(const uint8_t* slot, const uint64_t* w0, const uint64_t* w1, su16& a,
                                          uint64_t& x0, uint64_t& x1) {
    asm volatile(
        "s_load_dwordx16 %0, %3, 0x0 glc\n\t"
        "s_load_dwordx2 %1, %4, 0x0 glc\n\t"
        "s_load_dwordx2 %2, %5, 0x0 glc\n\t"
        "s_waitcnt lgkmcnt(0)"
        : "=&s"(a), "=&s"(x0), "=&s"(x1)
        : "s"(slot), "s"(w0), "s"(w1)
        : "memory");
}
__device__ __forceinline__ void pub64_sys(uint64_t* p, uint64_t v) {
    __hip_atomic_store(gptr64(reinterpret_cast<uint64_t>(p)), v, __ATOMIC_RELAXED, __HIP_MEMORY_SCOPE_SYSTEM);
}
__device__ __forceinline__ uint32_t poll32(uint32_t* p) {
    return __hip_atomic_load(p, __ATOMIC_RELAXED, __HIP_MEMORY_SCOPE_AGENT);
}
__device__ __forceinline__ uint64_t now_ticks() { return __builtin_amdgcn_s_memrealtime(); }
#ifdef RLO_DIAG
#define TL_ON(P) (((P).mode & MODE_TL) != 0u)
#else
#define TL_ON(P) false
#endif
typedef __attribute__((address_space(1))) uint32_t gu32;
__device__ __forceinline__ void tl_mark(const Params& P, uint32_t r, uint32_t ev) {
    if (TL_ON(P) && r < P.tl_rounds)
// ... 360 lines not shown
```

rootless-coll-mpi-ops_amd/csrc/rlo_world.cpp:

```cpp
#include <fcntl.h>
#include <hip/hip_runtime.h>
#include <sys/mman.h>
#include <sys/stat.h>
#include <unistd.h>

#include <algorithm>
#include <atomic>
#include <cctype>
#include <chrono>
#include <mutex>
#include <cstddef>
#include <cstdio>
#include <cstdlib>
#include <cstring>
#include <random>
#include <string>
#include <thread>
#include <vector>

#include "rlo_device.hpp"
#include "rlo_hip.h"
#include "rlo_shm.hpp"

extern "C" hipError_t rlo_launch_progress(const rlo::Params* p, int blocks, size_t dyn_lds, hipStream_t stream, int variant);
// ... 85 lines not shown
uint32_t pow2_floor(uint64_t x) {
    uint32_t p = 1;
    while ((uint64_t)p * 2 <= x && p < (1u << 30)) p <<= 1;
    return p;
}

template <class T>
struct DevBuf {
    T* p = nullptr;
    size_t n = 0;
    void release() {
        if (p) (void)hipFree(p);
        p = nullptr;
        n = 0;
    }
    int alloc(size_t count) {
        release();
        if (count == 0) count = 1;
        if (hipMalloc(&p, count * sizeof(T)) != hipSuccess) { p = nullptr; return RLO_E_HIP; }
        n = count;
        return RLO_OK;
    }
    int upload(const std::vector<T>& v) {
        int rc = alloc(v.size());
        if (rc) return rc;
        if (!v.empty() && hipMemcpy(p, v.data(), v.size() * sizeof(T), hipMemcpyHostToDevice) != hipSuccess) return RLO_E_HIP;
        return RLO_OK;
    }
};

struct Edge { int src, dst, j, k; };

struct Layout {
    int n = 0, nparts = 0;
    std::vector<int> pb;
    std::vector<int> part_of;
    std::vector<Topo> T;
    std::vector<Edge> E;
    std::vector<std::vector<int>> in_edges;
    int max_in = 0, max_fan = 0;
    uint32_t cap = 0, stride = 0, vote_cap = 0;
    std::vector<uint64_t> fwd_bytes, vote_bytes, ctrl_words;
    std::vector<uint64_t> fwd_off, vote_off;
    std::vector<uint32_t> inbox, outbox;
    std::vector<uint32_t> fbell, vbell;
    std::vector<uint64_t> lat_base;
    uint64_t bulk_max = 0;
    uint32_t bslots = 0, bcap = 0;
    std::vector<uint64_t> heap_bytes, bflag_bytes;
    uint32_t pend_slots = 2;
    bool pull = false;
    uint32_t relay_cap = 0;
    std::vector<uint64_t> orig_off;
};

int build_layout(int n, int nparts, const int32_t* pb, uint32_t max_payload, uint32_t ring_slots, uint64_t bulk_max,
                 uint32_t bulk_slots, Layout& L) {
    if (n < 2 || n > 65535 || nparts < 1 || nparts > rlo::kMaxParts) return RLO_E_INVAL;
    L.n = n;
    L.nparts = nparts;
    L.pb.assign(nparts + 1, 0);
    if (pb) {
        for (int p = 0; p <= nparts; p++) L.pb[p] = pb[p];
    } else {
        for (int p = 0; p <= nparts; p++) L.pb[p] = (int)((int64_t)n * p / nparts);
    }
    if (L.pb[0] != 0 || L.pb[nparts] != n) return RLO_E_INVAL;
    for (int p = 0; p < nparts; p++)
        if (L.pb[p + 1] <= L.pb[p]) return RLO_E_INVAL;
    L.part_of.assign(n, 0);
    for (int p = 0; p < nparts; p++)
        for (int r = L.pb[p]; r < L.pb[p + 1]; r++) L.part_of[r] = p;
    L.stride = rlo::kHdr + max_payload;

    L.T.assign(n, Topo{});
    for (int r = 0; r < n; r++)
        if (topo_of(n, r, &L.T[r])) return RLO_E_INVAL;
    L.in_edges.assign(n, {});
    for (int r = 0; r < n; r++)
        for (int j = 0; j < L.T[r].sll; j++) {
            L.in_edges[L.T[r].send_list[j]].push_back((int)L.E.size());
            L.E.push_back({r, L.T[r].send_list[j], j, 0});
        }
    for (int c = 0; c < n; c++) {
        if ((int)L.in_edges[c].size() > rlo::kMaxIn) return RLO_E_INVAL;
        L.max_in = std::max(L.max_in, (int)L.in_edges[c].size());
        for (int k = 0; k < (int)L.in_edges[c].size(); k++) L.E[L.in_edges[c][k]].k = k;
    }
    for (int r = 0; r < n; r++) L.max_fan = std::max(L.max_fan, L.T[r].sll);

    std::vector<uint64_t> rings(nparts, 0), vrings(nparts, 0);
    for (const Edge& e : L.E) {
        rings[L.part_of[e.dst]] += 2;
        vrings[L.part_of[e.src]] += 1;
    }
    {
        const char* pe = std::getenv("RLO_PULL");
        const bool want = pe ? std::atoi(pe) != 0 : L.stride / 16u > 24u;
        L.pull = want && L.stride > 8u * 16u && !bulk_max;
    }
    if (L.pull)
        for (int r = 0; r < n; r++) rings[L.part_of[r]] += 1;
    const uint64_t max_rings = *std::max_element(rings.begin(), rings.end());
    uint32_t cap = ring_slots ? pow2_ceil(ring_slots) : (L.stride <= 384u ? 2048u : 512u);
    const uint64_t limit = 0xFFFF0000ull;
    if (max_rings * cap * L.stride > limit) cap = pow2_floor(limit / (max_rings * L.stride));
    if (cap < 16) return RLO_E_INVAL;
    L.cap = cap;
    L.vote_cap = std::max<uint32_t>(64u, pow2_ceil(L.pend_slots * (uint32_t)n));

    const uint64_t ring_bytes = (uint64_t)cap * L.stride;
    L.fwd_bytes.assign(nparts, 0);
    L.vote_bytes.assign(nparts, 0);
    L.fwd_off.assign(L.E.size(), 0);
    L.vote_off.assign(L.E.size(), 0);
    for (size_t e = 0; e < L.E.size(); e++) {
        const int pd = L.part_of[L.E[e].dst], ps = L.part_of[L.E[e].src];
        L.fwd_off[e] = L.fwd_bytes[pd];
        L.fwd_bytes[pd] += 2 * ring_bytes;
        L.vote_off[e] = L.vote_bytes[ps];
        L.vote_bytes[ps] += (uint64_t)L.vote_cap * rlo::kVoteSlot;
    }
    L.orig_off.assign(n, 0);
    if (L.pull) {
        L.relay_cap = cap;
        for (uint32_t f = 4; f > 1; f /= 2) {
            bool fits = true;
            for (int p = 0; p < nparts; p++) {
                const uint64_t nlp = (uint64_t)(L.pb[p + 1] - L.pb[p]);
                fits &= L.fwd_bytes[p] + nlp * f * ring_bytes <= limit;
            }
            if (fits) { L.relay_cap = f * cap; break; }
        }
        for (int r = 0; r < n; r++) {
            L.orig_off[r] = L.fwd_bytes[L.part_of[r]];
            L.fwd_bytes[L.part_of[r]] += (uint64_t)L.relay_cap * L.stride;
        }
    }
    if (*std::max_element(L.vote_bytes.begin(), L.vote_bytes.end()) > limit) return RLO_E_INVAL;

    L.ctrl_words.assign(nparts, 0);
    L.lat_base.clear();
    L.inbox.assign(n, 0);
    L.outbox.assign(n, 0);
    L.fbell.assign(n, 0);
    L.vbell.assign(n, 0);
    for (int p = 0; p < nparts; p++) {
        uint64_t words = rlo::kCtrlHdrWords;
        for (int r = L.pb[p]; r < L.pb[p + 1]; r++) {
            L.inbox[r] = (uint32_t)words;
            words += (2 * L.in_edges[r].size() + L.T[r].sll + 15) & ~15ull;
            L.outbox[r] = (uint32_t)words;
            words += (2 * L.T[r].sll + L.in_edges[r].size() + 15) & ~15ull;
        }
        L.lat_base.push_back(words);
        words += rlo::kLatWords;
        for (int r = L.pb[p]; r < L.pb[p + 1]; r++) {
            L.fbell[r] = (uint32_t)words;
            words += (uint64_t)L.in_edges[r].size() * rlo::kBellWords;
            L.vbell[r] = (uint32_t)words;
            words += (2ull * L.T[r].sll + 15) & ~15ull;
        }
        L.ctrl_words[p] = words;
    }
    L.heap_bytes.assign(nparts, 0);
    L.bflag_bytes.assign(nparts, 0);
    if (bulk_max) {
        L.bslots = bulk_slots ? bulk_slots : ((uint64_t)n * 2u <= (uint64_t)rlo::kMaxPend ? 2u : 1u);
        if ((L.bslots & (L.bslots - 1)) || L.bslots > 8 || (uint64_t)n * L.bslots > (uint64_t)rlo::kMaxPend) return RLO_E_INVAL;
        if (bulk_max > 0xFFF00000ull) return RLO_E_INVAL;
        L.bulk_max = bulk_max;
        L.bcap = (uint32_t)((bulk_max + 65535u) & ~65535ull);
        for (int p = 0; p < nparts; p++) {
            const uint64_t nlp = (uint64_t)(L.pb[p + 1] - L.pb[p]);
            L.heap_bytes[p] = nlp * (uint64_t)n * L.bslots * L.bcap;
            L.bflag_bytes[p] = (nlp * (uint64_t)n * L.bslots + nlp * L.bslots) * rlo::kBulkLine;
        }
    }
    return RLO_OK;
}

struct PartBlob {
    uint32_t magic, version;
    int32_t part, nparts, n, device;
    uint32_t cap, stride, vote_cap, pad;
    uint64_t token;
    uint64_t fwd_ptr, vote_ptr, ctrl_ptr;
    uint64_t fwd_bytes, vote_bytes, ctrl_bytes;
    char bus[32];
    hipIpcMemHandle_t hf, hv, hc;
    uint64_t heap_ptr, bflag_ptr, heap_bytes, bflag_bytes;
    hipIpcMemHandle_t hh, hb;
    uint64_t nonce;
};
static_assert(sizeof(PartBlob) <= RLO_PART_BLOB_BYTES, "blob");
constexpr uint32_t kBlobMagic = 0x524C4F50u;

uint64_t process_token() {
    static uint64_t tok = 0;
    if (!tok) {
        std::random_device rd;
        tok = ((uint64_t)rd() << 32) ^ rd() ^ ((uint64_t)getpid() << 17) ^ (uint64_t)(uintptr_t)&tok;
        if (!tok) tok = 1;
    }
    return tok;
}
// ... 305 lines not shown
}

int plan_lds(const Layout& L, int nl, int nmov, int cus, uint32_t flags, OccFn occ, LdsPlan* out) {
    uint32_t ns_force = 0;
    if (const char* e = diag_env("RLO_NSMALL"))
        if (L.stride / 16u > 24u) ns_force = std::max(2u, std::min(8u, (uint32_t)std::atoi(e)));
    if (L.bulk_max) return plan_variant(L, nl, nmov, cus, 5, false, occ, ns_force, out);
    const char* env = diag_env("RLO_WAVES");
    const int force = env ? std::atoi(env) : 0;
    const bool small = L.stride <= 8u * 16u;
    const bool hbm_only = (flags & RLO_PART_PEND_HBM) != 0;
    if (force != 4 && (small || force == 8) && nl <= cus) {
        if (!hbm_only && plan_variant(L, nl, nmov, cus, 8, false, occ, ns_force, out) == RLO_OK) return RLO_OK;
        if (plan_variant(L, nl, nmov, cus, 8, true, occ, ns_force, out) == RLO_OK) return RLO_OK;
    }
    if (force == 8) return RLO_E_OCCUPANCY;
    const uint32_t ns0 = ns_force ? ns_force : (L.stride / 16u <= 24u ? L.stride / 16u : 5u);
    for (uint32_t ns = ns0; ns >= 1; ns--) {
        if (!hbm_only && plan_variant(L, nl, nmov, cus, 4, false, occ, ns, out) == RLO_OK) return RLO_OK;
        if (plan_variant(L, nl, nmov, cus, 4, true, occ, ns, out) == RLO_OK) return RLO_OK;
    }
    return RLO_E_OCCUPANCY;
}

int size_lds(rlo_world* w) {
    LdsPlan p;
    const int rc = plan_lds(w->L, w->nl, (int)w->nmov, w->cus, w->flags, occ_device, &p);
    if (rc) return rc;
    w->variant = p.variant;
    w->waves = p.waves;
    w->nsmall = p.nsmall;
    w->stage2 = p.stage2;
    w->dyn_lds = p.dyn_lds;
    w->bpend_off = p.bpend_off;
    w->blocks_per_cu = p.blocks_per_cu;
    w->ll_ok = p.ll_ok;
    w->pend_hbm = p.pend_hbm;
    return RLO_OK;
}

void build_topo(rlo_world* w) {
    const Layout& L = w->L;
    const uint64_t ring_bytes = (uint64_t)L.cap * L.stride;
    w->topo.assign(w->nl, rlo::RankTopo{});
    for (int r = w->rb; r < w->rb + w->nl; r++) {
        rlo::RankTopo& t = w->topo[r - w->rb];
        t.level = L.T[r].level;
        t.last_wall = L.T[r].last_wall;
        t.scc = L.T[r].scc;
        t.sll = L.T[r].sll;
        for (int j = 0; j < L.T[r].sll; j++) t.send_list[j] = L.T[r].send_list[j];
        t.n_in = (int)L.in_edges[r].size();
        t.inbox_ctrl = L.inbox[r];
        t.n_inbox = 2 * t.n_in + t.sll;
        t.outbox_ctrl = L.outbox[r];
        t.n_outbox = 2 * t.sll + t.n_in;
        t.orig_data = (uint32_t)L.orig_off[r];
        t.in_bell = L.fbell[r];
        t.vin_bell = L.vbell[r];
    }
    for (size_t e = 0; e < L.E.size(); e++) {
        const Edge& ed = L.E[e];
        const int ps = L.part_of[ed.src], pd = L.part_of[ed.dst];
        if (ps == w->part) {
            rlo::RankTopo& t = w->topo[ed.src - w->rb];
            for (int vc = 0; vc < 2; vc++) {
                t.out_ring[ed.j][vc] = (uint64_t)(uintptr_t)(w->pf[pd] + L.fwd_off[e] + vc * ring_bytes);
                t.out_tail[ed.j][vc] = (uint64_t)(uintptr_t)(w->pc[pd] + L.inbox[ed.dst] + 2 * ed.k + vc);
            }
            t.vin_data[ed.j] = (uint32_t)L.vote_off[e];
            t.vin_head[ed.j] = (uint64_t)(uintptr_t)(w->pc[pd] + L.outbox[ed.dst] + 2 * L.T[ed.dst].sll + ed.k);
            t.out_bell[ed.j] = (uint64_t)(uintptr_t)(w->pc[pd] + L.fbell[ed.dst] + (uint64_t)rlo::kBellWords * ed.k);
        }
        if (pd == w->part) {
            rlo::RankTopo& t = w->topo[ed.dst - w->rb];
            for (int vc = 0; vc < 2; vc++) {
                t.in_data[ed.k][vc] = (uint32_t)(L.fwd_off[e] + vc * ring_bytes);
                t.in_head[ed.k][vc] = (uint64_t)(uintptr_t)(w->pc[ps] + L.outbox[ed.src] + 2 * ed.j + vc);
            }
            t.in_src[ed.k] = ed.src;
            t.in_base[ed.k] = (uint64_t)(uintptr_t)w->pf[ps];
            t.vout_ring[ed.k] = (uint64_t)(uintptr_t)(w->pv[ps] + L.vote_off[e]);
            t.vout_tail[ed.k] = (uint64_t)(uintptr_t)(w->pc[ps] + L.inbox[ed.src] + 2 * L.in_edges[ed.src].size() + ed.j);
            t.vout_bell[ed.k] = (uint64_t)(uintptr_t)(w->pc[ps] + L.vbell[ed.src] + 2 * ed.j);
        }
    }
}

}


extern "C" {

int rlo_last_hip_error(void) { return g_last_hip; }

const char* rlo_strerror(int code) {
    switch (code) {
        case RLO_OK: return "ok";
        case RLO_E_INVAL: return "invalid argument";
        case RLO_E_HIP: return "HIP runtime error";
        case RLO_E_OCCUPANCY: return "ranks cannot all be co-resident";
        case RLO_E_DEVICE: return "device-side engine error";
        case RLO_E_NOPROGRAM: return "no program loaded";
        case RLO_E_NODEVICE: return "no HIP device";
        case RLO_E_NOTCONNECTED: return "part not connected";
        case RLO_E_AGAIN: return "ring full, retry";
        case RLO_E_TIMEOUT: return "shared host service: no answer in time";
        case RLO_E_STALE: return "a peer part's mapped memory is not that part's current memory (stale IPC mapping)";
        default: return "unknown";
    }
}

int rlo_topology(int n, int rank, int* level, int* last_wall, int* scc, int* sll, int* send_list) {
    Topo t;
    int rc = topo_of(n, rank, &t);
    if (rc) return rc;
    if (level) *level = t.level;
    if (last_wall) *last_wall = t.last_wall;
    if (scc) *scc = t.scc;
    if (sll) *sll = t.sll;
    if (send_list) std::memcpy(send_list, t.send_list, sizeof(int) * t.sll);
    return RLO_OK;
}

int rlo_children(int n, int rank, int origin, int from, int* out) {
    Topo t;
    int rc = topo_of(n, rank, &t);
    if (rc) return rc;
    int c = 0;
    if (from < 0) {
        for (int i = t.sll - 1; i >= 0; i--) out[c++] = t.send_list[i];
    } else if (t.level > 0) {
        if (from > t.last_wall) {
            for (int j = t.scc; j >= 0; j--) out[c++] = t.send_list[j];
        } else {
            for (int j = t.scc - 1; j >= 0; j--)
                if (!passed(rank, origin, t.send_list[j])) out[c++] = t.send_list[j];
        }
    }
    return c;
}

int rlo_part_create(const rlo_part_cfg_t* cfg, rlo_world_t** out) {
    if (!cfg || !out || cfg->n_parts < 1 || cfg->part < 0 || cfg->part >= cfg->n_parts) return RLO_E_INVAL;
    int ndev = 0;
    if (hipGetDeviceCount(&ndev) != hipSuccess || ndev == 0) return RLO_E_NODEVICE;
    rlo_world* w = new rlo_world();
    w->max_payload = (std::max<uint32_t>(cfg->max_payload ? cfg->max_payload : 4096u, 16u) + 15u) & ~15u;
    if (w->max_payload > 65520u) { delete w; return RLO_E_INVAL; }
    w->flags = cfg->flags;
    const bool one_xcd = (cfg->flags & RLO_PART_ONE_XCD) != 0;
    if (one_xcd && (cfg->n_parts != 1 || cfg->bulk_max || cfg->n_ranks > 256)) { delete w; return RLO_E_INVAL; }
    if (!diag_env("RLO_CACHED_RINGS") && !one_xcd) w->flags |= RLO_PART_UNCACHED;
    {
        const uint32_t pp = cfg->proposal_pool ? cfg->proposal_pool : 2u;
        if ((pp & (pp - 1u)) || pp > (uint32_t)rlo::kPoolMax) { delete w; return RLO_E_INVAL; }
        w->L.pend_slots = pp;
    }
    int rc = build_layout(cfg->n_ranks, cfg->n_parts, cfg->part_begin, w->max_payload, cfg->ring_slots, cfg->bulk_max,
                          cfg->bulk_slots, w->L);
    if (rc) { delete w; return rc; }
    w->part = cfg->part;
    w->rb = w->L.pb[w->part];
    w->nl = w->L.pb[w->part + 1] - w->rb;
    if (cfg->device >= 0 && hipSetDevice(cfg->device) != hipSuccess) { delete w; return RLO_E_HIP; }
    (void)hipGetDevice(&w->device);
    hipDeviceProp_t prop;
    if (hipGetDeviceProperties(&prop, w->device) != hipSuccess) { delete w; return RLO_E_HIP; }
    w->cus = prop.multiProcessorCount;
    if (w->L.bulk_max) {
        int mv = (int)cfg->movers;
        if (mv == 0) mv = std::max(16, w->cus - w->nl) & ~1;
        if (mv < 2) { delete w; return RLO_E_OCCUPANCY; }
        w->nmov = (uint32_t)mv;
        {
            const uint32_t bm = (uint32_t)std::min<uint64_t>(w->L.bulk_max, 0xFFF00000ull);
            const rlo::BulkPlan pl = rlo::bulk_plan(w->L.n, bm, true);
            const rlo::BulkPlan p1 = rlo::bulk_plan(w->L.n, bm, false);
            const uint64_t ts = std::max(rlo::bulk_total_tiles(pl, bm), rlo::bulk_total_tiles(p1, bm));
            const uint64_t tg = std::max(rlo::bulk_stripe_tiles(pl, bm, 0), rlo::bulk_stripe_tiles(p1, bm, 0));
            const uint64_t tv = (bm + rlo::kVerifyTile - 1) / rlo::kVerifyTile;
            const uint64_t K = rlo::kMaxSub;
            const uint64_t nl = (uint64_t)w->nl, B = w->L.bslots, N = (uint64_t)w->L.n;
            const uint64_t need = nl * B * std::min<uint64_t>(rlo::kMaxSubScatter, ts) + nl * N * B * (std::min(K, tg) + std::min(K, tv)) + 64;
            if (need > (1ull << 26)) { delete w; return RLO_E_INVAL; }
            w->jslots = pow2_ceil((uint32_t)need);
        }
    }
    rc = size_lds(w);
    if (rc) { delete w; return rc; }
    const int me = w->part;
    if (alloc_region(w, (void**)&w->fwd, w->L.fwd_bytes[me] + kNonceTail) || alloc_region(w, (void**)&w->vote, w->L.vote_bytes[me]) ||
        alloc_region(w, (void**)&w->ctrl, w->L.ctrl_words[me] * 8)) {
        rlo_world_destroy(w);
        return RLO_E_HIP;
    }
    if (one_xcd) {
        const hipError_t e = hipExtMallocWithFlags((void**)&w->d_xcd, 256, hipDeviceMallocUncached);
        if (e != hipSuccess) { g_last_hip = (int)e; w->d_xcd = nullptr; rlo_world_destroy(w); return RLO_E_HIP; }
    }
    if (w->pend_hbm) {
        const uint32_t keep = w->flags;
        w->flags |= RLO_PART_UNCACHED;
        const int e = alloc_region(w, (void**)&w->pend_mem, (uint64_t)w->nl * w->L.n * w->L.pend_slots * 16u);
        w->flags = keep;
        if (e) { rlo_world_destroy(w); return RLO_E_HIP; }
    }
    if (w->L.bulk_max) {
        w->jmem_bytes = job_mem(w->jslots, (uint32_t)w->nl).bytes;
        const uint32_t keep = w->flags;
        w->flags |= RLO_PART_UNCACHED;
        const int e = alloc_region(w, (void**)&w->heap, w->L.heap_bytes[me]) ||
                      alloc_region(w, (void**)&w->bflag, w->L.bflag_bytes[me] + kNonceTail) || alloc_region(w, (void**)&w->jmem, w->jmem_bytes);
        w->flags = keep;
        if (e) { rlo_world_destroy(w); return RLO_E_HIP; }
        (void)hipMemset(w->bflag, 0, w->L.bflag_bytes[me]);
        w->host_bulk_q.assign(w->nl, 0);
    }
    (void)hipMemset(w->fwd, 0, std::max<uint64_t>(w->L.fwd_bytes[me], 1));
    (void)hipMemset(w->vote, 0, std::max<uint64_t>(w->L.vote_bytes[me], 1));
    (void)hipMemset(w->ctrl, 0, w->L.ctrl_words[me] * 8);
    if (w->d_stats.alloc(w->nl)) { rlo_world_destroy(w); return RLO_E_HIP; }
// ... 310 lines not shown
    for (void* r : {(void*)w->fwd, (void*)w->vote, (void*)w->ctrl, (void*)w->heap, (void*)w->bflag, (void*)w->jmem,
                    (void*)w->pend_mem})
        release_region(r);
    w->d_bheap.release(); w->d_bflag.release(); w->d_part_of.release(); w->d_part_begin.release();
    w->d_topo.release(); w->d_stats.release();
    w->d_sched_off.release(); w->d_expect_bcast.release(); w->d_prop_off.release(); w->d_expect_dec.release();
    w->d_sched_ids.release(); w->d_prop_data_off.release(); w->d_prop_data_len.release(); w->d_isp_off.release();
    w->d_lat_count.release(); w->d_lat_round.release(); w->d_lat_origin.release(); w->d_prop_pid.release();
    w->d_lat_out.release(); w->d_lat_own_off.release(); w->d_lat_own.release(); w->d_mask.release(); w->d_prop_data.release(); w->d_log_payload.release();
    w->d_isp.release(); w->d_log.release();
    if (w->d_xcd) (void)hipFree(w->d_xcd);
    host_free(w);
    if (w->ev0) (void)hipEventDestroy(w->ev0);
    if (w->ev1) (void)hipEventDestroy(w->ev1);
    delete w;
    return RLO_OK;
}

int rlo_world_query(const rlo_world_t* w, rlo_world_info_t* o) {
    if (!w || !o) return RLO_E_INVAL;
    std::memset(o, 0, sizeof *o);
    o->n_ranks = w->L.n;
    o->max_in_degree = w->L.max_in;
    o->max_fanout = w->L.max_fan;
    o->edges = (int)w->L.E.size();
    o->ring_slots = w->L.cap;
    o->slot_stride = w->L.stride;
    o->vote_slots = w->L.vote_cap;
    o->fwd_bytes = w->L.fwd_bytes[w->part];
    o->vote_bytes = w->L.vote_bytes[w->part];
    o->ctrl_bytes = w->L.ctrl_words[w->part] * 8;
    o->cus = w->cus;
    o->blocks_per_cu = w->blocks_per_cu;
    o->part = w->part;
    o->n_parts = w->L.nparts;
    o->rank_begin = w->rb;
    o->rank_end = w->rb + w->nl;
    o->sys_scope = w->sys_scope;
    o->peers = w->peers;
    o->waves = w->waves;
    o->bulk_slots = w->L.bslots;
    o->movers = w->nmov;
    o->bulk_max = w->L.bulk_max;
    o->heap_bytes = w->L.heap_bytes[w->part];
    o->proposal_pool = w->L.pend_slots;
    o->pull = w->L.pull && w->nsmall >= 2 ? 1u : 0u;
    o->nsmall = w->nsmall;
    o->stage2_bytes = w->stage2;
    o->ll_ok = w->ll_ok ? 1u : 0u;
    o->pend_hbm = w->pend_hbm ? 1u : 0u;
    o->dyn_lds = (uint32_t)w->dyn_lds;
    o->last_kernel = w->last_hop ? 1u : 0u;
    o->static_lds = (uint32_t)rlo_kernel_static_lds(w->variant);
    return RLO_OK;
}

static uint32_t ll_mode(const rlo_world* w, uint32_t max_msg) {
    if (!w->ll_ok || diag_env("RLO_NO_LL")) return 0u;
    if (w->variant == 8 && (rlo::kHdr + max_msg + 15u) / 16u > w->nsmall) return 0u;
    return rlo::MODE_LL;
}

static void base_params(rlo_world* w) {
    w->have_program = false;
    rlo::Params& P = w->P;
    std::memset(&P, 0, sizeof P);
    P.n = w->L.n;
    P.rank_begin = w->rb;
    P.rank_end = w->rb + w->nl;
    P.topo = w->d_topo.p;
    P.fwd_region = w->fwd;
    P.fwd_region_bytes = (uint32_t)std::max<uint64_t>(w->L.fwd_bytes[w->part], 1);
    P.fwd_cap = w->L.cap;
    P.fwd_stride = w->L.stride;
    P.vote_region = w->vote;
    P.vote_region_bytes = (uint32_t)std::max<uint64_t>(w->L.vote_bytes[w->part], 1);
    P.vote_cap = w->L.vote_cap;
    P.ctrl = w->ctrl;
    P.ctrl_bytes = (uint32_t)(w->L.ctrl_words[w->part] * 8);
    P.sys_scope = (uint32_t)w->sys_scope;
    P.n_parts = (uint32_t)w->L.nparts;
    for (int q = 0; q < w->L.nparts; q++) P.err_flag[q] = reinterpret_cast<uint32_t*>(w->pc[q]);
    P.error_flag = reinterpret_cast<uint32_t*>(w->ctrl);
    P.stats = w->d_stats.p;
    P.nsmall = w->nsmall;
    P.nout_max = 2u * (uint32_t)w->L.max_fan;
    P.stage2_bytes = w->stage2;
    P.timeout_ticks = 100000000ull * 10;
    P.deadline_ticks = 100000000ull * 120;
    P.window = 32;
    P.n_local = (uint32_t)w->nl;
    P.ring_cap = w->L.stride - rlo::kHdr;
    P.pend_slots = w->L.pend_slots;
    P.pend_hbm = reinterpret_cast<rlo::PendState*>(w->pend_mem);
    P.pull = w->L.pull && w->nsmall >= 2 ? 1u : 0u;
    P.relay_cap = w->L.relay_cap;
    P.own_pool = 1;
    if (w->L.bulk_max) {
        const JobMem m = job_mem(w->jslots, (uint32_t)w->nl);
        P.bulk_slots = w->L.bslots;
        P.bulk_cap = w->L.bcap;
        P.nmov = w->nmov;
        P.bulk_cross = ((w->peers & RLO_PEER_OTHER_GPU) || (w->flags & RLO_PART_CHUNKED)) ? 1u : 0u;
        P.bheap = w->d_bheap.p;
        P.bflag = w->d_bflag.p;
        P.part_of = w->d_part_of.p;
// ... 1 lines not shown
        P.jslots = w->jslots;
        P.bpend_off = w->bpend_off;
        P.jobs = reinterpret_cast<rlo::BulkJob*>(w->jmem + m.jobs);
        P.jctl = reinterpret_cast<uint64_t*>(w->jmem + m.jctl);
        P.jclaim = reinterpret_cast<uint64_t*>(w->jmem + m.jclaim);
        P.jfree = reinterpret_cast<uint64_t*>(w->jmem + m.jfree);
        P.jdone = reinterpret_cast<uint32_t*>(w->jmem + m.jdone);
        P.jsum = reinterpret_cast<uint64_t*>(w->jmem + m.jsum);
    }
}

static int setup_log(rlo_world* w, uint32_t flags, uint32_t log_cap, bool payload) {
    rlo::Params& P = w->P;
    if (!(flags & RLO_FLAG_LOG)) return RLO_OK;
    if (log_cap == 0) log_cap = 1024;
    if (w->d_log.alloc((size_t)w->nl * log_cap)) return RLO_E_HIP;
    P.log = w->d_log.p;
    P.log_cap = log_cap;
    P.mode |= rlo::MODE_LOG;
    if (payload) {
        P.log_stride = w->max_payload;
        if (w->d_log_payload.alloc((size_t)w->nl * log_cap * P.log_stride)) return RLO_E_HIP;
        P.log_payload = w->d_log_payload.p;
    }
    return RLO_OK;
}

int rlo_program_storm(rlo_world_t* w, const rlo_storm_cfg_t* cfg) {
    if (!w || !cfg || cfg->k < 0 || cfg->k > 0xFFFFFFFFll || cfg->order > RLO_ORDER_SLOTS) return RLO_E_INVAL;
    const uint32_t hi = std::max(cfg->len, cfg->len_max);
    if (hi > (w->L.bulk_max ? w->L.bulk_max : w->max_payload)) return RLO_E_INVAL;
    if (cfg->len_max > cfg->len && !w->L.bulk_max) return RLO_E_INVAL;
    if (!w->connected) return RLO_E_NOTCONNECTED;
    base_params(w);
    rlo::Params& P = w->P;
    const int n = w->L.n, nl = w->nl, rb = w->rb;
    std::vector<int64_t> off(nl + 1, 0), expect(nl, 0), per(n, 0);
    std::vector<uint32_t> org((size_t)std::max<int64_t>(cfg->k, 1));
    for (int64_t b = 0; b < cfg->k; b++) {
        org[b] = cfg->order == RLO_ORDER_SLOTS ? (uint32_t)(b % n)
                                               : (uint32_t)(splitmix64(cfg->seed + (uint64_t)b) % (uint64_t)n);
        per[org[b]]++;
        if ((int)org[b] >= rb && (int)org[b] < rb + nl) off[org[b] - rb + 1]++;
    }
    for (int r = 0; r < nl; r++) off[r + 1] += off[r];
    std::vector<uint32_t> ids((size_t)std::max<int64_t>(off[nl], 1));
    std::vector<int64_t> fill(off.begin(), off.end() - 1);
    for (int64_t b = 0; b < cfg->k; b++)
        if ((int)org[b] >= rb && (int)org[b] < rb + nl) ids[fill[org[b] - rb]++] = (uint32_t)b;
    for (int r = 0; r < nl; r++) expect[r] = cfg->k - per[rb + r];
    if (w->d_sched_off.upload(off) || w->d_sched_ids.upload(ids) || w->d_expect_bcast.upload(expect)) return RLO_E_HIP;
    P.mode = rlo::MODE_STORM | ((cfg->flags & RLO_FLAG_HIST) ? rlo::MODE_HIST : 0u) |
             ((cfg->flags & RLO_FLAG_PROF) ? rlo::MODE_PROF : 0u);
    P.seed = cfg->seed;
    P.len = cfg->len;
    P.len_lo = cfg->len;
    P.len_hi = hi;
    P.storm_order = cfg->order;
    P.window = std::min<uint32_t>(cfg->window ? cfg->window : 64, 64u);
    P.sched_off = w->d_sched_off.p;
    P.sched_ids = w->d_sched_ids.p;
    P.expect_bcast = w->d_expect_bcast.p;
    int rc = setup_log(w, cfg->flags, cfg->log_cap, true);
    if (rc) return rc;
    w->have_program = true;
    return RLO_OK;
}

int rlo_program_latency(rlo_world_t* w, uint32_t rounds, uint32_t len, uint64_t seed, uint32_t flags) {
    if (!w || rounds == 0 || len > (w->L.bulk_max ? w->L.bulk_max : w->max_payload)) return RLO_E_INVAL;
    if (!w->connected) return RLO_E_NOTCONNECTED;
    if (w->L.nparts != 1 && rounds > (uint32_t)rlo::kLatCap) return RLO_E_INVAL;
#ifndef RLO_DIAG
    if (flags & RLO_FLAG_TIMELINE) return RLO_E_INVAL;
#endif
    base_params(w);
    rlo::Params& P = w->P;
    const int n = w->L.n;
    std::vector<int32_t> org(rounds);
    std::vector<int64_t> expect(w->nl, 0);
    for (uint32_t i = 0; i < rounds; i++) org[i] = (int32_t)(splitmix64(seed + i) % (uint64_t)n);
    for (int lr = 0; lr < w->nl; lr++)
        for (uint32_t i = 0; i < rounds; i++) expect[lr] += org[i] != w->rb + lr;
    std::vector<uint32_t> own_off(w->nl + 1, 0), own;
    for (int lr = 0; lr < w->nl; lr++) {
        for (uint32_t i = 0; i < rounds; i++)
            if (org[i] == w->rb + lr) own.push_back(i);
        own_off[lr + 1] = (uint32_t)own.size();
    }
    if (own.empty()) own.push_back(0);
    if (w->d_lat_own_off.upload(own_off) || w->d_lat_own.upload(own)) return RLO_E_HIP;
    if (w->d_lat_origin.upload(org) || w->d_expect_bcast.upload(expect) || w->d_lat_count.alloc(rounds) ||
        w->d_lat_out.alloc(rounds) || w->d_lat_round.alloc(1) || w->d_lat_obs.alloc(rounds))
        return RLO_E_HIP;
    P.mode = rlo::MODE_LAT | ((flags & RLO_FLAG_HIST) ? rlo::MODE_HIST : 0u) | ((flags & RLO_FLAG_PROF) ? rlo::MODE_PROF : 0u) |
             ll_mode(w, len);
    P.len = len;
    P.seed = seed;
    P.lat_rounds = rounds;
    P.hop_chunks = (rlo::kHdr + len + 15u) / 16u;
    P.lat_origin = w->d_lat_origin.p;
    P.lat_count = w->d_lat_count.p;
    P.lat_out = w->d_lat_out.p;
    P.lat_round = w->d_lat_round.p;
    P.lat_obs = w->d_lat_obs.p;
    if (w->L.nparts != 1) {
// ... 591 lines not shown
int rlo_latencies(rlo_world_t* w, uint64_t* ticks, uint32_t cap) {
    if (!w || !ticks || !w->d_lat_out.p) return RLO_E_INVAL;
    uint32_t n = std::min(cap, w->lat_rounds);
    HIPCHK(hipSetDevice(w->device));
    HIPCHK(hipMemcpy(ticks, w->d_lat_out.p, sizeof(uint64_t) * n, hipMemcpyDeviceToHost));
    return (int)n;
}

int rlo_timeline(rlo_world_t* w, uint32_t* out, uint64_t cap, uint32_t* stride) {
    if (!w || !out) return RLO_E_INVAL;
    const uint32_t st = rlo::kTlGlobal + rlo::kTlCols * (uint32_t)w->nl;
    if (stride) *stride = st;
    if (!w->tl_rows || !w->d_tl.p) return 0;
    const uint32_t rows = (uint32_t)std::min<uint64_t>(w->tl_rows, cap / st);
    HIPCHK(hipSetDevice(w->device));
    HIPCHK(hipMemcpy(out, w->d_tl.p, sizeof(uint32_t) * rows * st, hipMemcpyDeviceToHost));
    return (int)rows;
}

int rlo_round_ticks(rlo_world_t* w, uint64_t* ticks, uint32_t cap) {
    if (!w || !ticks || !w->d_lat_obs.p) return RLO_E_INVAL;
    if (w->rb != 0) return RLO_E_INVAL;
    uint32_t n = std::min(cap, w->lat_rounds);
    HIPCHK(hipSetDevice(w->device));
    HIPCHK(hipMemcpy(ticks, w->d_lat_obs.p, sizeof(uint64_t) * n, hipMemcpyDeviceToHost));
    return (int)n;
}

}


extern "C" {

int rlo_bulk_plan(int n, uint64_t len, int cross, rlo_bulk_plan_t* out) {
    if (n < 2 || !out || len == 0 || len > 0xFFF00000ull) return RLO_E_INVAL;
    const rlo::BulkPlan p = rlo::bulk_plan(n, (uint32_t)len, cross != 0);
    out->nchunks = p.nchunks;
    out->stripe = p.stripe;
    out->chunk = p.chunk;
    out->tile = p.tile;
    out->total_tiles = rlo::bulk_total_tiles(p, (uint32_t)len);
    out->direct = p.direct;
    return RLO_OK;
}

int rlo_layout_plan(const rlo_plan_cfg_t* cfg, rlo_world_info_t* o) {
    if (!cfg || !o || cfg->n_parts < 1 || cfg->part < 0 || cfg->part >= cfg->n_parts) return RLO_E_INVAL;
    Layout L;
    const uint32_t mp = (std::max<uint32_t>(cfg->max_payload ? cfg->max_payload : 4096u, 16u) + 15u) & ~15u;
    if (mp > 65520u) return RLO_E_INVAL;
    const uint32_t pp = cfg->proposal_pool ? cfg->proposal_pool : 2u;
    if ((pp & (pp - 1u)) || pp > (uint32_t)rlo::kPoolMax) return RLO_E_INVAL;
    L.pend_slots = pp;
    int rc = build_layout(cfg->n_ranks, cfg->n_parts, nullptr, mp, cfg->ring_slots, cfg->bulk_max, cfg->bulk_slots, L);
    if (rc) return rc;
    const int cus = cfg->cus > 0 ? cfg->cus : 256;
    const int nl = L.pb[cfg->part + 1] - L.pb[cfg->part];
    int nmov = 0;
    if (L.bulk_max) nmov = cfg->movers ? (int)cfg->movers : (std::max(16, cus - nl) & ~1);
    LdsPlan p;
    rc = plan_lds(L, nl, nmov, cus, cfg->flags, occ_model, &p);
    if (rc) return rc;
    std::memset(o, 0, sizeof *o);
    o->n_ranks = L.n;
    o->max_in_degree = L.max_in;
    o->max_fanout = L.max_fan;
    o->edges = (int)L.E.size();
    o->ring_slots = L.cap;
    o->slot_stride = L.stride;
    o->vote_slots = L.vote_cap;
    o->fwd_bytes = L.fwd_bytes[cfg->part];
    o->vote_bytes = L.vote_bytes[cfg->part];
    o->ctrl_bytes = L.ctrl_words[cfg->part] * 8;
    o->cus = cus;
    o->blocks_per_cu = p.blocks_per_cu;
    o->part = cfg->part;
    o->n_parts = L.nparts;
    o->rank_begin = L.pb[cfg->part];
    o->rank_end = L.pb[cfg->part + 1];
    o->waves = p.waves;
    o->bulk_slots = L.bslots;
    o->movers = (uint32_t)nmov;
    o->bulk_max = L.bulk_max;
    o->heap_bytes = L.heap_bytes[cfg->part];
    o->proposal_pool = L.pend_slots;
    o->pull = L.pull && p.nsmall >= 2 ? 1u : 0u;
    o->nsmall = p.nsmall;
    o->stage2_bytes = p.stage2;
    o->ll_ok = p.ll_ok ? 1u : 0u;
    o->pend_hbm = p.pend_hbm ? 1u : 0u;
    o->dyn_lds = (uint32_t)p.dyn_lds;
    o->static_lds = (uint32_t)rlo_kernel_static_lds(p.variant);
    return RLO_OK;
}

int rlo_storm_lengths(uint64_t seed, uint64_t k, uint32_t len, uint32_t len_max, uint32_t* out) {
    if (!out && k) return RLO_E_INVAL;
    const uint32_t hi = len_max > len ? len_max : len;
    for (uint64_t b = 0; b < k; b++) out[b] = hi > len ? rlo::storm_len_of(seed, b, len, hi) : len;
    return RLO_OK;
}

int rlo_host_bulk_stage(rlo_world_t* w, int rank, const void* data, uint64_t len, uint32_t timeout_us, uint32_t* q_out) {
    if (!w || !w->h_cmd || !w->L.bulk_max || rank < w->rb || rank >= w->rb + w->nl || !q_out) return RLO_E_INVAL;
    if (len == 0 || len > w->L.bulk_max || (len && !data)) return RLO_E_INVAL;
    const int lr = rank - w->rb;
    const uint32_t B = w->L.bslots, q = w->host_bulk_q[lr], s = q & (B - 1u);
    const uint64_t need = (uint64_t)(q / B) * (uint64_t)(w->L.n - 1);
    const volatile uint64_t* done = reinterpret_cast<const volatile uint64_t*>(
        w->bflag + ((uint64_t)w->nl * w->L.n * B + (uint64_t)lr * B + s) * rlo::kBulkLine);
    const auto t0 = std::chrono::steady_clock::now();
    while (*done < need) {
        if (std::chrono::steady_clock::now() - t0 > std::chrono::microseconds(timeout_us)) return RLO_E_AGAIN;
    }
    HIPCHK(hipSetDevice(w->device));
    uint8_t* dst = w->heap + (((uint64_t)lr * w->L.n + (uint64_t)rank) * B + s) * w->L.bcap;
    HIPCHK(hipMemcpy(dst, data, len, hipMemcpyHostToDevice));
    w->host_bulk_q[lr] = q + 1;
    *q_out = q;
    return RLO_OK;
}

int rlo_host_bulk_copy(rlo_world_t* w, int rank, const rlo_log_rec_t* ev, void* dst) {
    if (!w || !ev || !w->L.bulk_max || rank < w->rb || rank >= w->rb + w->nl || !dst) return RLO_E_INVAL;
    if (ev->kind != RLO_EV_DELIVER_BULK || ev->origin < 0 || ev->origin >= w->L.n || ev->aux >= w->L.bslots ||
        ev->len > w->L.bulk_max)
        return RLO_E_INVAL;
    const int lr = rank - w->rb;
    HIPCHK(hipSetDevice(w->device));
    const uint8_t* src = w->heap + (((uint64_t)lr * w->L.n + (uint64_t)ev->origin) * w->L.bslots + ev->aux) * w->L.bcap;
    HIPCHK(hipMemcpy(dst, src, ev->len, hipMemcpyDeviceToHost));
    return RLO_OK;
}


int rlo_host_share(rlo_world_t* w, const char* name, uint64_t stage_bytes) {
    if (!w || !name || name[0] != '/' || std::strlen(name) > 200 || w->have_program || w->shm) return RLO_E_INVAL;
    if (stage_bytes == 0) stage_bytes = 4ull << 20;
    w->share_stage = (stage_bytes + 4095u) & ~uint64_t(4095);
    w->shm_name = name;
    return RLO_OK;
}

int rlo_host_unlink(rlo_world_t* w) {
    if (!w || !w->shm) return RLO_E_INVAL;
    if (w->shm_linked) shm_unlink(w->shm_name.c_str());
// ... 121 lines not shown
```

rootless-coll-mpi-ops_amd/rlo/__init__.py:

```python
from ._lib import load, RloError, LIB_PATH
from .world import World, topology, children, hist_percentile, bulk_plan, storm_lengths, layout_plan, pool_trim, pool_stats
from . import _lib as abi
from .host import HostWorld

load()
```

rootless-coll-mpi-ops_amd/rlo/_lib.py:

```python
import ctypes
import os
import re

PKG_DIR = os.path.dirname(os.path.dirname(os.path.abspath(__file__)))
LIB_PATH = os.path.join(PKG_DIR, "lib", "librlo_hip.so")
if os.environ.get("RLO_DIAG_LIB") == "1":
    LIB_PATH = os.path.join(PKG_DIR, "lib_diag", "librlo_hip.so")
_AB = os.environ.get("RLO_LIB_DIR", "")
if re.fullmatch(r"lib_[a-z0-9_]+", _AB):
    LIB_PATH = os.path.join(PKG_DIR, _AB, "librlo_hip.so")

RLO_OK = 0
RLO_E_INVAL, RLO_E_HIP, RLO_E_OCCUPANCY, RLO_E_DEVICE, RLO_E_NOPROGRAM, RLO_E_NODEVICE = -1, -2, -3, -4, -5, -6
RLO_E_NOTCONNECTED = -7
RLO_E_AGAIN = -8
RLO_PART_BLOB_BYTES = 512
RLO_PART_UNCACHED = 1
RLO_PART_CHUNKED = 2
RLO_PART_PEND_HBM = 4
RLO_PART_ONE_XCD = 8
RLO_PEER_OTHER_GPU, RLO_PEER_IMPORTED = 1, 2
RLO_LAUNCH_NO_RESET = 1
RLO_TRIM_IMPORTS, RLO_TRIM_FREE, RLO_TRIM_RETIRED, RLO_TRIM_EXPORTED = 1, 2, 4, 8
RLO_FLAG_LOG, RLO_FLAG_HIST, RLO_FLAG_PROF, RLO_FLAG_TIMELINE = 1, 2, 4, 8
RLO_JUDGE_APPROVE, RLO_JUDGE_MASK, RLO_JUDGE_ISP, RLO_JUDGE_HASH = 0, 1, 2, 3
DERR = {1: "timeout", 2: "vote ring", 3: "pid collision", 4: "vote orphan", 5: "log full", 6: "bad slot", 7: "host command",
        8: "bulk index"}
RLO_CMD_BCAST, RLO_CMD_PROPOSAL, RLO_CMD_JUDGE, RLO_CMD_OWN_JUDGE, RLO_CMD_QUIT = 0, 2, 16, 17, 18
RLO_CMD_BULK, RLO_CMD_BULK_RELEASE = 10, 19
RLO_EV_DELIVER_BCAST, RLO_EV_DELIVER_DECISION, RLO_EV_DELIVER_BULK = 1, 1 | (4 << 8), 1 | (10 << 8)
RLO_ORDER_RANDOM, RLO_ORDER_SLOTS = 0, 1
TAG_BULK = 10
RLO_EV_ACTION, RLO_EV_RESULT, RLO_EV_JUDGE, RLO_EV_OWN_JUDGE, RLO_EV_JUDGED = 3, 4, 6, 7, 8


class WorldCfg(ctypes.Structure):
    _fields_ = [("n_ranks", ctypes.c_int32), ("max_payload", ctypes.c_uint32), ("ring_slots", ctypes.c_uint32),
                ("device", ctypes.c_int32), ("bulk_max", ctypes.c_uint64), ("bulk_slots", ctypes.c_uint32),
                ("movers", ctypes.c_uint32), ("proposal_pool", ctypes.c_uint32), ("flags", ctypes.c_uint32)]


class WorldInfo(ctypes.Structure):
    _fields_ = [("n_ranks", ctypes.c_int32), ("max_in_degree", ctypes.c_int32), ("max_fanout", ctypes.c_int32),
                ("edges", ctypes.c_int32), ("ring_slots", ctypes.c_uint32), ("slot_stride", ctypes.c_uint32),
                ("vote_slots", ctypes.c_uint32), ("peers", ctypes.c_uint32), ("fwd_bytes", ctypes.c_uint64),
                ("vote_bytes", ctypes.c_uint64), ("ctrl_bytes", ctypes.c_uint64), ("cus", ctypes.c_int32),
                ("blocks_per_cu", ctypes.c_int32), ("part", ctypes.c_int32), ("n_parts", ctypes.c_int32),
                ("rank_begin", ctypes.c_int32), ("rank_end", ctypes.c_int32), ("sys_scope", ctypes.c_int32),
                ("waves", ctypes.c_int32), ("bulk_slots", ctypes.c_uint32), ("movers", ctypes.c_uint32),
                ("bulk_max", ctypes.c_uint64), ("heap_bytes", ctypes.c_uint64), ("proposal_pool", ctypes.c_uint32),
                ("pull", ctypes.c_uint32), ("nsmall", ctypes.c_uint32), ("stage2_bytes", ctypes.c_uint32),
                ("ll_ok", ctypes.c_uint32), ("pend_hbm", ctypes.c_uint32), ("dyn_lds", ctypes.c_uint32),
                ("static_lds", ctypes.c_uint32), ("last_kernel", ctypes.c_uint32), ("info_pad", ctypes.c_uint32)]


class PlanCfg(ctypes.Structure):
    _fields_ = [("n_ranks", ctypes.c_int32), ("n_parts", ctypes.c_int32), ("part", ctypes.c_int32),
                ("max_payload", ctypes.c_uint32), ("ring_slots", ctypes.c_uint32), ("flags", ctypes.c_uint32),
                ("bulk_max", ctypes.c_uint64), ("bulk_slots", ctypes.c_uint32), ("movers", ctypes.c_uint32),
                ("proposal_pool", ctypes.c_uint32), ("cus", ctypes.c_int32)]


class PartCfg(ctypes.Structure):
    _fields_ = [("n_ranks", ctypes.c_int32), ("n_parts", ctypes.c_int32), ("part", ctypes.c_int32),
                ("part_begin", ctypes.c_void_p), ("max_payload", ctypes.c_uint32), ("ring_slots", ctypes.c_uint32),
                ("device", ctypes.c_int32), ("flags", ctypes.c_uint32), ("bulk_max", ctypes.c_uint64),
                ("bulk_slots", ctypes.c_uint32), ("movers", ctypes.c_uint32), ("proposal_pool", ctypes.c_uint32),
                ("pad", ctypes.c_uint32)]


class StormCfg(ctypes.Structure):
    _fields_ = [("seed", ctypes.c_uint64), ("k", ctypes.c_int64), ("len", ctypes.c_uint32), ("window", ctypes.c_uint32),
                ("flags", ctypes.c_uint32), ("log_cap", ctypes.c_uint32), ("len_max", ctypes.c_uint32),
                ("order", ctypes.c_uint32)]


class IarCfg(ctypes.Structure):
    _fields_ = [("judge_kind", ctypes.c_uint32), ("judge_ppm", ctypes.c_uint32), ("judge_seed", ctypes.c_uint64),
                ("judge_mask", ctypes.c_void_p), ("judge_isp", ctypes.c_char_p), ("flags", ctypes.c_uint32),
                ("log_cap", ctypes.c_uint32), ("pool", ctypes.c_uint32), ("pad", ctypes.c_uint32)]


class HostCfg(ctypes.Structure):
    _fields_ = [("cmd_slots", ctypes.c_uint32), ("pickup_slots", ctypes.c_uint32), ("idle_timeout_s", ctypes.c_uint32),
                ("flags", ctypes.c_uint32), ("pool", ctypes.c_uint32), ("pad", ctypes.c_uint32)]


class Cmd(ctypes.Structure):
    _fields_ = [("kind", ctypes.c_uint32), ("origin", ctypes.c_int32), ("id", ctypes.c_int32), ("pseq", ctypes.c_uint32),
                ("vote", ctypes.c_int32), ("pad", ctypes.c_uint32)]


class RankStats(ctypes.Structure):
    _fields_ = [(f, ctypes.c_uint64) for f in (
        "bcast_delivered", "bcast_sum", "originated", "dec_delivered", "dec_approved", "actions", "judge_calls",
        "own_decided", "own_approved", "proposals_recv", "iterations", "busy_iterations", "stalls", "log_count",
        "t_start", "t_end")] + [("error", ctypes.c_uint32), ("error_aux", ctypes.c_uint32), ("prof", ctypes.c_uint64 * 8),
                           ("dbg", ctypes.c_uint64 * 8),
                           ("hist", ctypes.c_uint32 * 128), ("unmarked_slots", ctypes.c_uint64)]


class BulkPlan(ctypes.Structure):
    _fields_ = [("nchunks", ctypes.c_uint32), ("stripe", ctypes.c_uint32), ("chunk", ctypes.c_uint32),
                ("tile", ctypes.c_uint32), ("total_tiles", ctypes.c_uint32), ("direct", ctypes.c_uint32)]


class LogRec(ctypes.Structure):
    _fields_ = [("kind", ctypes.c_uint32), ("origin", ctypes.c_int32), ("from_", ctypes.c_int32), ("id", ctypes.c_uint32),
                ("len", ctypes.c_uint32), ("vote", ctypes.c_int32), ("aux", ctypes.c_uint32), ("payload_idx", ctypes.c_uint32)]


EXPORTS = ["rlo_topology", "rlo_children", "rlo_world_create", "rlo_world_destroy", "rlo_part_close_imports", "rlo_part_import", "rlo_world_query",
           "rlo_part_create", "rlo_part_export", "rlo_part_connect", "rlo_reset", "rlo_launch_ex",
           "rlo_stream_create", "rlo_stream_destroy",
           "rlo_program_storm", "rlo_program_latency", "rlo_program_iar", "rlo_launch", "rlo_wait", "rlo_run",
           "rlo_last_kernel_ms", "rlo_stats", "rlo_log", "rlo_latencies", "rlo_round_ticks", "rlo_timeline", "rlo_strerror", "rlo_last_hip_error",
           "rlo_device_error", "rlo_bulk_debug",
           "rlo_program_host", "rlo_host_post", "rlo_host_poll", "rlo_host_running", "rlo_host_cmd_count",
           "rlo_device_count", "rlo_device_numa_node", "rlo_host_bulk_stage", "rlo_host_bulk_copy", "rlo_bulk_plan", "rlo_layout_plan",
           "rlo_storm_lengths", "rlo_host_share", "rlo_host_unlink", "rlo_host_proxy", "rlo_host_wait_started",
           "rlo_host_fail", "rlo_client_attach", "rlo_client_detach", "rlo_client_state", "rlo_client_post",
           "rlo_client_poll", "rlo_client_cmd_count", "rlo_client_bulk_put", "rlo_client_bulk_get", "rlo_client_debug", "rlo_client_hdiag", "rlo_client_fwd", "rlo_host_device_judge",
           "rlo_pool_trim", "rlo_pool_stats"]

_lib = None


def load():
    global _lib
    if _lib is not None:
        return _lib
    if not os.path.exists(LIB_PATH):
        raise ImportError("librlo_hip.so not built (%s): run `make -C rootless-coll-mpi-ops_amd`" % LIB_PATH)
    L = ctypes.CDLL(LIB_PATH)
    ip = ctypes.POINTER(ctypes.c_int)
    vp = ctypes.c_void_p
    L.rlo_topology.argtypes = [ctypes.c_int, ctypes.c_int, ip, ip, ip, ip, ip]
    L.rlo_children.argtypes = [ctypes.c_int] * 4 + [ip]
    L.rlo_world_create.argtypes = [ctypes.POINTER(WorldCfg), ctypes.POINTER(vp)]
    L.rlo_world_destroy.argtypes = [vp]
    L.rlo_part_close_imports.argtypes = [vp]
    L.rlo_pool_trim.argtypes = [ctypes.c_uint32, ctypes.POINTER(ctypes.c_uint64)]
    L.rlo_pool_stats.argtypes = [ctypes.POINTER(ctypes.c_uint64), ctypes.c_uint32]
    L.rlo_part_import.argtypes = [vp, ctypes.c_char_p, ctypes.c_int]
    L.rlo_world_query.argtypes = [vp, ctypes.POINTER(WorldInfo)]
    L.rlo_program_storm.argtypes = [vp, ctypes.POINTER(StormCfg)]
    L.rlo_program_latency.argtypes = [vp, ctypes.c_uint32, ctypes.c_uint32, ctypes.c_uint64, ctypes.c_uint32]
    L.rlo_program_iar.argtypes = [vp, ctypes.POINTER(IarCfg), ctypes.c_int64, vp, vp, vp, vp, vp]
    L.rlo_part_create.argtypes = [ctypes.POINTER(PartCfg), ctypes.POINTER(vp)]
    L.rlo_part_export.argtypes = [vp, vp, ctypes.c_uint32]
    L.rlo_part_connect.argtypes = [vp, vp, ctypes.c_int]
    L.rlo_reset.argtypes = [vp, vp]
    L.rlo_launch_ex.argtypes = [vp, vp, ctypes.c_uint32]
    L.rlo_launch.argtypes = [vp, vp]
    L.rlo_stream_create.argtypes = [ctypes.c_int, ctypes.POINTER(vp)]
    L.rlo_stream_destroy.argtypes = [vp]
    L.rlo_wait.argtypes = [vp]
    L.rlo_run.argtypes = [vp, vp, ctypes.POINTER(ctypes.c_float)]
    L.rlo_last_kernel_ms.argtypes = [vp, ctypes.POINTER(ctypes.c_float)]
    L.rlo_stats.argtypes = [vp, ctypes.POINTER(RankStats), ctypes.c_int]
    L.rlo_log.argtypes = [vp, ctypes.c_int, ctypes.POINTER(LogRec), ctypes.c_uint32, vp, ctypes.c_uint32]
    L.rlo_latencies.argtypes = [vp, ctypes.POINTER(ctypes.c_uint64), ctypes.c_uint32]
    L.rlo_round_ticks.argtypes = [vp, ctypes.POINTER(ctypes.c_uint64), ctypes.c_uint32]
    L.rlo_timeline.argtypes = [vp, ctypes.POINTER(ctypes.c_uint32), ctypes.c_uint64, ctypes.POINTER(ctypes.c_uint32)]
    L.rlo_program_host.argtypes = [vp, ctypes.POINTER(HostCfg)]
    L.rlo_host_post.argtypes = [vp, ctypes.c_int, ctypes.POINTER(Cmd), vp, ctypes.c_uint32]
    L.rlo_host_poll.argtypes = [vp, ctypes.c_int, ctypes.POINTER(LogRec), vp, ctypes.c_uint32]
    L.rlo_host_running.argtypes = [vp]
    L.rlo_host_cmd_count.argtypes = [vp, ctypes.c_int, ctypes.POINTER(ctypes.c_uint64), ctypes.POINTER(ctypes.c_uint64)]
    L.rlo_device_count.argtypes = []
    L.rlo_device_numa_node.argtypes = [ctypes.c_int]
    L.rlo_host_bulk_stage.argtypes = [vp, ctypes.c_int, vp, ctypes.c_uint64, ctypes.c_uint32,
                                      ctypes.POINTER(ctypes.c_uint32)]
    L.rlo_host_bulk_copy.argtypes = [vp, ctypes.c_int, ctypes.POINTER(LogRec), vp]
    L.rlo_bulk_plan.argtypes = [ctypes.c_int, ctypes.c_uint64, ctypes.c_int, ctypes.POINTER(BulkPlan)]
    L.rlo_layout_plan.argtypes = [ctypes.POINTER(PlanCfg), ctypes.POINTER(WorldInfo)]
    L.rlo_storm_lengths.argtypes = [ctypes.c_uint64, ctypes.c_uint64, ctypes.c_uint32, ctypes.c_uint32,
                                    ctypes.POINTER(ctypes.c_uint32)]
    L.rlo_host_device_judge.argtypes = [vp, ctypes.POINTER(IarCfg)]
    L.rlo_host_share.argtypes = [vp, ctypes.c_char_p, ctypes.c_uint64]
    L.rlo_host_unlink.argtypes = [vp]
    L.rlo_host_proxy.argtypes = [vp]
    L.rlo_host_wait_started.argtypes = [vp, ctypes.c_uint32]
    L.rlo_host_fail.argtypes = [vp]
    L.rlo_client_attach.argtypes = [ctypes.c_char_p, ctypes.c_int, ctypes.POINTER(vp)]
    L.rlo_client_detach.argtypes = [vp]
    L.rlo_client_state.argtypes = [vp]
    L.rlo_client_post.argtypes = [vp, ctypes.POINTER(Cmd), vp, ctypes.c_uint32]
    L.rlo_client_poll.argtypes = [vp, ctypes.POINTER(LogRec), vp, ctypes.c_uint32]
    L.rlo_client_cmd_count.argtypes = [vp, ctypes.POINTER(ctypes.c_uint64), ctypes.POINTER(ctypes.c_uint64)]
    L.rlo_client_bulk_put.argtypes = [vp, vp, ctypes.c_uint64, ctypes.c_uint32, ctypes.POINTER(ctypes.c_uint32)]
    L.rlo_client_bulk_get.argtypes = [vp, ctypes.POINTER(LogRec), vp]
    L.rlo_client_debug.argtypes = [vp, ctypes.POINTER(ctypes.c_uint64)]
    L.rlo_client_hdiag.argtypes = [vp, ctypes.POINTER(ctypes.c_uint64)]
    L.rlo_client_fwd.argtypes = [vp, ctypes.POINTER(ctypes.c_uint64), ctypes.POINTER(ctypes.c_int64)]
    L.rlo_bulk_debug.argtypes = [vp, ctypes.POINTER(ctypes.c_uint64), ctypes.c_uint32]
    L.rlo_device_error.argtypes = [vp, ctypes.POINTER(ctypes.c_uint32), ctypes.POINTER(ctypes.c_uint32)]
    L.rlo_strerror.argtypes = [ctypes.c_int]
    L.rlo_strerror.restype = ctypes.c_char_p
    _lib = L
    return L


class RloError(RuntimeError):
    pass


def check(rc, what=""):
    if rc < 0:
        L = load()
        msg = L.rlo_strerror(rc).decode()
        if rc == RLO_E_HIP:
            msg += " (hipError %d)" % L.rlo_last_hip_error()
        raise RloError("%s failed: %s [%d]" % (what, msg, rc))
    return rc
```

rootless-coll-mpi-ops_amd/rlo/world.py:

```python
import ctypes

import numpy as np

from . import _lib as L
from ._lib import check


class World:

    def __init__(self, n, max_payload=4096, ring_slots=0, device=-1, _part=None, bulk_max=0, bulk_slots=0, movers=0,
                 proposal_pool=0, pend_hbm=False, one_xcd=False):
        self.lib = L.load()
        h = ctypes.c_void_p()
        if _part is None:
            cfg = L.WorldCfg(n, max_payload, ring_slots, device, bulk_max, bulk_slots, movers, proposal_pool,
                             (L.RLO_PART_PEND_HBM if pend_hbm else 0) | (L.RLO_PART_ONE_XCD if one_xcd else 0))
            check(self.lib.rlo_world_create(ctypes.byref(cfg), ctypes.byref(h)), "rlo_world_create")
        else:
            n_parts, part, begin, flags = _part
            self._pb = None
            pb = None
            if begin is not None:
                self._pb = (ctypes.c_int32 * (n_parts + 1))(*begin)
                pb = ctypes.cast(self._pb, ctypes.c_void_p)
# ... 191 lines not shown
        stride = ctypes.c_uint32()
        check(self.lib.rlo_timeline(self.h, (ctypes.c_uint32 * 1)(), 0, ctypes.byref(stride)), "rlo_timeline")
        cap = 64 * stride.value
        arr = (ctypes.c_uint32 * cap)()
        n = check(self.lib.rlo_timeline(self.h, arr, cap, ctypes.byref(stride)), "rlo_timeline")
        return np.array(arr[:n * stride.value], dtype=np.uint32).reshape(n, stride.value)


def pool_trim(what):
    lib = L.load()
    freed = ctypes.c_uint64()
    check(lib.rlo_pool_trim(what, ctypes.byref(freed)), "rlo_pool_trim")
    return int(freed.value)


def pool_stats():
    lib = L.load()
    out = (ctypes.c_uint64 * 6)()
    check(lib.rlo_pool_stats(out, 6), "rlo_pool_stats")
    return dict(zip(("live", "free", "free_exported", "retired", "imports_used", "imports_idle"), [int(x) for x in out]))


def hist_percentile(hist, p):
    hist = np.asarray(hist, dtype=np.float64)
    tot = hist.sum()
    if tot == 0:
        return 0.0
    c = np.cumsum(hist)
    b = int(np.searchsorted(c, p / 100.0 * tot))
    if b < 4:
        return float(b)
    o, sub = b // 4 + 1, b % 4
    lo = (4 + sub) << (o - 2)
    hi = (5 + sub) << (o - 2)
    return 0.5 * (lo + hi)


def bulk_plan(n, nbytes, cross=False):
    out = L.BulkPlan()
    check(L.load().rlo_bulk_plan(n, nbytes, 1 if cross else 0, ctypes.byref(out)), "rlo_bulk_plan")
    return {"nchunks": out.nchunks, "stripe": out.stripe, "chunk": out.chunk, "tile": out.tile,
            "total_tiles": out.total_tiles, "direct": out.direct}


def layout_plan(n, n_parts=1, part=0, max_payload=4096, ring_slots=0, bulk_max=0, bulk_slots=0, movers=0,
                proposal_pool=0, pend_hbm=False, cus=256):
    cfg = L.PlanCfg(n, n_parts, part, max_payload, ring_slots, L.RLO_PART_PEND_HBM if pend_hbm else 0, bulk_max,
                    bulk_slots, movers, proposal_pool, cus)
    out = L.WorldInfo()
    check(L.load().rlo_layout_plan(ctypes.byref(cfg), ctypes.byref(out)), "rlo_layout_plan")
    return {f: getattr(out, f) for f, _ in L.WorldInfo._fields_}


def storm_lengths(seed, k, length, len_max=0):
    out = np.zeros(max(k, 1), dtype=np.uint32)
    check(L.load().rlo_storm_lengths(seed, k, length, len_max, out.ctypes.data_as(ctypes.POINTER(ctypes.c_uint32))),
          "rlo_storm_lengths")
    return out[:k]


def topology(n, rank):
    lib = L.load()
    v = [ctypes.c_int() for _ in range(4)]
    sl = (ctypes.c_int * 16)()
    check(lib.rlo_topology(n, rank, *[ctypes.byref(x) for x in v], sl), "rlo_topology")
    level, lw, scc, sll = (x.value for x in v)
    return {"level": level, "last_wall": lw, "send_channel_cnt": scc, "send_list_len": sll, "send_list": list(sl[:sll])}


def children(n, rank, origin, frm):
    out = (ctypes.c_int * 16)()
    k = check(L.load().rlo_children(n, rank, origin, frm, out), "rlo_children")
    return list(out[:k])
```

Before: 28.67 million msgs/s.

## Delegate outbound ring copies from busy ranks to helper ranks via descriptor rings

Adds a delegation mode for the 8-wave storm kernel. Selected ranks no longer copy payloads into some outbound rings. They write small slot descriptors and publish a tail, and helper ranks copy the payload into the target ring and publish its progress. The aim is to spread the per-rank fanout copy cost across less-loaded workgroups. In exchange it adds extra polling, gating of input-head publication on helper completion, disables the single-message fast path for delegators, and makes the layout planning more involved.

```diff
diff --git a/include/rlo_hip.h b/include/rlo_hip.h
--- a/include/rlo_hip.h
+++ b/include/rlo_hip.h
@@ -66,7 +66,9 @@
     uint32_t pend_hbm;
     uint32_t dyn_lds, static_lds;
     uint32_t last_kernel;
-    uint32_t info_pad;
+    uint32_t delegators;
+    uint32_t helpers;
+    uint32_t delegated_rings;
 } rlo_world_info_t;
 
 int rlo_world_create(const rlo_world_cfg_t* cfg, rlo_world_t** out);
@@ -203,6 +205,8 @@
     int32_t cus;
 } rlo_plan_cfg_t;
 int rlo_layout_plan(const rlo_plan_cfg_t* cfg, rlo_world_info_t* out);
+typedef struct { int32_t rank, oi, helper, k; } rlo_deleg_ring_t;
+int rlo_delegate_plan(const rlo_plan_cfg_t* cfg, int32_t level, rlo_deleg_ring_t* out, uint32_t cap, uint32_t* words);
 int rlo_storm_lengths(uint64_t seed, uint64_t k, uint32_t len, uint32_t len_max, uint32_t* out);
 int rlo_host_bulk_stage(rlo_world_t* w, int rank, const void* data, uint64_t len, uint32_t timeout_us, uint32_t* q);
 int rlo_host_bulk_copy(rlo_world_t* w, int rank, const rlo_log_rec_t* ev, void* dst);
@@ -248,6 +252,7 @@
     uint64_t dbg[8];
     uint32_t hist[128];
     uint64_t unmarked_slots;
+    uint64_t helper_copies;
 } rlo_rank_stats_t;
 
 
diff --git a/rootless-coll-mpi-ops_amd/csrc/rlo_device.hpp b/rootless-coll-mpi-ops_amd/csrc/rlo_device.hpp
--- a/rootless-coll-mpi-ops_amd/csrc/rlo_device.hpp
+++ b/rootless-coll-mpi-ops_amd/csrc/rlo_device.hpp
@@ -8,6 +8,8 @@
 constexpr int kMaxFanout = 16;
 constexpr int kMaxIn = 32;
 constexpr int kMaxOut = 2 * kMaxFanout;
+constexpr int kMaxHelp = 16;
+constexpr uint64_t kDgClosed = 1ull << 63;
 constexpr int kHdr = 16;
 constexpr int kVoteSlot = 16;
 constexpr int kMaxCand = 256;
@@ -46,6 +48,7 @@
     MODE_TL = 32768u,
     MODE_HOPPROF = 131072u,
     MODE_NOHPW = 262144u,
+    MODE_DELEG = 1048576u,
     MODE_XCD1 = 524288u,
     MODE_CORRUPT = 65536u,
     MODE_HOST = 128u,
@@ -90,6 +93,14 @@
     uint32_t in_bell, vin_bell;
     uint64_t out_bell[kMaxFanout];
     uint64_t vout_bell[kMaxIn];
+    uint32_t dg_mask;
+    uint32_t dg_nhelp;
+    uint32_t dg_desc[kMaxOut];
+    uint64_t dg_tail[kMaxOut];
+    uint32_t dh_desc[kMaxHelp];
+    uint64_t dh_ring[kMaxHelp];
+    uint64_t dh_tail[kMaxHelp];
+    uint64_t dh_done[kMaxHelp];
 };
 
 constexpr uint32_t kBellChunks = 8;
@@ -107,6 +118,7 @@
     uint64_t dbg[8];
     uint32_t hist[kHistBins];
     uint64_t unmarked_slots;
+    uint64_t helper_copies;
 };
 
 constexpr uint32_t kPkRecBytes = 32, kPkMaxSlots = 16384, kPkNoPayload = 0xffffu, kPkTaggedPayload = 0x8000u;
diff --git a/rootless-coll-mpi-ops_amd/csrc/rlo_kernel.hip b/rootless-coll-mpi-ops_amd/csrc/rlo_kernel.hip
--- a/rootless-coll-mpi-ops_amd/csrc/rlo_kernel.hip
+++ b/rootless-coll-mpi-ops_amd/csrc/rlo_kernel.hip
@@ -38,6 +38,19 @@
     uint32_t bulk_q;
 };
 struct NoBulkSh {};
+constexpr uint32_t kDq = 8;
+struct DgSh {
+    uint64_t hp_done[kMaxHelp], hp_pub[kMaxHelp];
+    uint32_t hp_start[kMaxHelp], hp_n[kMaxHelp];
+    uint64_t gate[2 * kMaxIn];
+    uint64_t dq_out[kDq][kMaxOut], dq_in[kDq][2 * kMaxIn];
+    uint32_t dq_n, dq_h;
+    uint32_t dmask, nhelp, hclosed;
+    uint32_t hpend;
+    uint64_t snap[64];
+    unsigned long long copies;
+};
+struct NoDgSh {};
 struct BulkPend {
     uint32_t bid, len, ntiles;
     int32_t from;
@@ -47,6 +60,7 @@
 template <int W, bool BULK>
 struct Shared {
     typename std::conditional<BULK, BulkSh, NoBulkSh>::type b;
+    typename std::conditional<W == 8 && !BULK, DgSh, NoDgSh>::type d;
     static constexpr int kWaves = W, kMaxCand = 64 * W;
     RankTopo t;
     uint64_t ring_head[2 * kMaxIn];
@@ -671,6 +685,7 @@
 #define PMODE(x) ((PM & (uint32_t)(x)) ? (P.mode & (uint32_t)(x)) : 0u)
 #define PULL_ON (W == 4 && !BULK && P.pull != 0u)
     constexpr int kWaves = W, kBlock = 64 * W, kMaxCand = 64 * W;
+    constexpr bool kDg = W == 8 && !BULK && !LL && !PH && PM == kPmStorm;
     constexpr uint32_t kHostBase = kMaxCand - kPass;
     extern __shared__ __attribute__((aligned(16))) uint8_t dyn_lds[];
     __shared__ Shared<W, BULK> S;
@@ -737,6 +752,16 @@
         for (int i = tid; i < kHistBins; i += kBlock) S.hist[i] = 0;
         for (int i = tid; i < 4 * 64; i += kBlock) { (&S.pubw[0][0])[i] = 0; (&S.snap[0][0])[i] = 0; }
         if (tid < kMaxIn) { S.vout_tail[tid] = 0; S.vout_head[tid] = 0; }
+        if constexpr (kDg) {
+            if (tid < kMaxHelp) { S.d.hp_done[tid] = 0; S.d.hp_pub[tid] = 0; S.d.hp_start[tid] = 0; S.d.hp_n[tid] = 0; }
+            if (tid < 64) { S.d.gate[tid] = 0; S.d.snap[tid] = 0; }
+            if (tid == 0) {
+                const bool on = (P.mode & MODE_DELEG) != 0;
+                S.d.dq_n = 0; S.d.dq_h = 0; S.d.copies = 0; S.d.hclosed = 1; S.d.hpend = 0;
+                S.d.dmask = on ? P.topo[lr].dg_mask : 0u;
+                S.d.nhelp = on && !P.topo[lr].dg_mask ? P.topo[lr].dg_nhelp : 0u;
+            }
+        }
         if (tid < 8) { S.prof[tid] = 0; S.dbg[tid] = 0; S.hd[tid] = 0; }
         if (tid == 0) S.tl_bfid = 0;
         if (tid == 0) {
@@ -782,6 +807,16 @@
     const uint32_t sl_r = lane < sll ? (uint32_t)t.send_list[lane] : 0u;
     const bool sys = P.sys_scope != 0;
     const uint32_t oring_bytes = P.fwd_cap * P.fwd_stride;
+    auto dg_dmask = [&]() -> uint32_t {
+        if constexpr (kDg) return (uint32_t)uni((int)S.d.dmask);
+        else return 0u;
+    };
+    auto dg_nhelp = [&]() -> uint32_t {
+        if constexpr (kDg) return (uint32_t)uni((int)S.d.nhelp);
+        else return 0u;
+    };
+#define DMASK dg_dmask()
+#define NHELP dg_nhelp()
 #define OTPTR t.out_tail[lane >> 1][lane & 1]
 #define IHPTR t.in_head[lane >> 1][lane & 1]
 #define VHPTR t.vin_head[lane]
@@ -1442,6 +1477,7 @@
         lt_mask = (1ull << lane) - 1ull;
         a_it++;
         uint64_t in_tail_r = 0, out_head_r = 0, vin_tail_r = 0, vout_head_r = 0;
+        [[maybe_unused]] uint64_t dgx = 0;
         uint32_t errf = 0, sid = 0, latr = 0;
         if (w == 0) {
             uint32_t ll_run = 0;
@@ -1470,6 +1506,9 @@
                 vin_tail_r = ld64_sc1(rc, lane < sll ? (inbox + (uint32_t)(n_in2 + lane)) * 8u : kOob);
                 out_head_r = ld64_sc1(rc, lane < nout ? (outbox + (uint32_t)lane) * 8u : kOob);
                 vout_head_r = ld64_sc1(rc, lane < n_in ? (outbox + (uint32_t)(nout + lane)) * 8u : kOob);
+                if constexpr (kDg)
+                    dgx = ld64_sc1(rc, (uint32_t)lane < S.d.nhelp ? (inbox + (uint32_t)(n_in2 + sll + lane)) * 8u
+                                       : (S.d.dmask && lane < nout ? (outbox + (uint32_t)(nout + n_in + lane)) * 8u : kOob));
                 errf = ld32_sc1(rc, 0u);
                 if constexpr (BULK) {
                     const __amdgpu_buffer_rsrc_t rd = mk_rsrc(reinterpret_cast<void*>(uni64(S.b.dbase)), bsl * kBulkLine);
@@ -1511,11 +1550,38 @@
                               (latr != p_lat && rdl32(latr, 1) == S.lat_own_next) || errf != 0
                         : in_tail_r != S.snap[0][lane] || vin_tail_r != S.snap[1][lane] || out_head_r != S.snap[2][lane] ||
                               vout_head_r != S.snap[3][lane] || hpoll != p_h || latr != p_lat || errf != 0 || bmoved;
-                if (__ballot(moved)) { SPIN_WHY(6); break; }
+                bool dmoved = false;
+                if constexpr (kDg) dmoved = dgx != S.d.snap[lane];
+                if (__ballot(moved || dmoved)) { SPIN_WHY(6); break; }
             }
             if (hpw && lane == 0) S.a_done = a_it;
             S.snap[0][lane] = in_tail_r; S.snap[1][lane] = vin_tail_r; S.snap[2][lane] = out_head_r;
             S.snap[3][lane] = vout_head_r; p_h = hpoll; p_lat = latr;
+            if constexpr (kDg) {
+                const uint32_t nhelp = NHELP;
+                S.d.snap[lane] = dgx;
+                if (nhelp) {
+                    bool open = false;
+                    uint32_t n = 0;
+                    if ((uint32_t)lane < nhelp) {
+                        const uint64_t tl = dgx & ~kDgClosed, dn = S.d.hp_done[lane];
+                        n = tl > dn ? (uint32_t)min(tl - dn, (uint64_t)P.fwd_cap) : 0u;
+                        S.d.hp_start[lane] = (uint32_t)dn;
+                        S.d.hp_n[lane] = n;
+                        S.d.hp_done[lane] = dn + n;
+                        open = !(dgx & kDgClosed) || dn + n != tl;
+                    }
+                    const uint64_t opn = __ballot(open);
+                    if (lane == 0) S.d.hclosed = opn == 0ull ? 1u : 0u;
+                    uint32_t ntot = 0;
+                    if (__ballot(n != 0u)) wave_excl_scan(n, &ntot);
+                    if (lane == 0) S.d.hpend = ntot;
+                    if (ntot) {
+                        ll_prog = true;
+                        if (lane == 0) S.d.copies += ntot;
+                    }
+                }
+            }
             if (host && (n_iter & 4095u) == 0 && lane < 3) pub64_sys(&hctl[kHctlBeat + lane], lane == 2 ? n_iter : hpoll);
             if constexpr (BULK) {
                 if (lane < (int)bsl) S.b.sdone[lane] = dnw;
@@ -1578,9 +1644,88 @@
         BAR();
         PROF_STAMP(0);
 
+        if constexpr (kDg) {
+            const uint32_t nhelp = w != 0 ? NHELP : 0u;
+            if (nhelp) {
+                bool bad = false;
+                const uint32_t hq = (kHdr + P.len + 15u) >> 4;
+                const uint32_t hmagic = hq > 1 ? 0xFFFFFFFFu / hq + 1u : 0u;
+                for (uint32_t k = 0; k < nhelp; k++) {
+                    const uint32_t n = (uint32_t)uni((int)S.d.hp_n[k]);
+                    if (!n) continue;
+                    const uint32_t s0 = (uint32_t)uni((int)S.d.hp_start[k]), doff = (uint32_t)uni((int)t.dh_desc[k]);
+                    const __amdgpu_buffer_rsrc_t ro = mk_rsrc(reinterpret_cast<void*>(uni64(t.dh_ring[k])), oring_bytes);
+                    const uint32_t items = n * hq;
+#pragma unroll 1
+                    for (uint32_t i0 = (uint32_t)(w - 1) * 64u; i0 < items; i0 += (uint32_t)(kWaves - 1) * 128u) {
+                        uint32_t sl[2], qq[2], dsc[2];
+                        u32x4 v[2];
+#pragma unroll
+                        for (int u = 0; u < 2; u++) {
+                            const uint32_t i = i0 + (uint32_t)u * (uint32_t)(kWaves - 1) * 64u + (uint32_t)lane;
+                            const uint32_t r = div_small(i, hmagic);
+                            qq[u] = i - r * hq;
+                            sl[u] = i < items ? (s0 + r) & fcap_m : ~0u;
+                            dsc[u] = ld32_sc1(rf, sl[u] != ~0u ? doff + 4u * sl[u] : kOob);
+                        }
+#pragma unroll
+                        for (int u = 0; u < 2; u++) {
+                            const bool on = sl[u] != ~0u && dsc[u] != ~0u;
+                            v[u] = ld_sc1(rf, on ? dsc[u] + 16u * qq[u] : kOob);
+                            dsc[u] = on ? 1u : 0u;
+                        }
+#pragma unroll
+                        for (int u = 0; u < 2; u++) {
+                            const bool ok = !(qq[u] == 0u && ((v[u].z >> 16) & 0xffu) != kSlotMark);
+                            bad |= dsc[u] && !ok;
+                            if (dsc[u] && ok) st_ring(ro, __umul24(sl[u], P.fwd_stride) + (qq[u] << 4), v[u], sys);
+                        }
+                    }
+                }
+                if (__ballot(bad) && lane == 0) {
+                    atomicAdd(&S.stale, 1ull);
+                    set_error(S, P, ERR_BAD_SLOT, 0xDE1E6u);
+                }
+            }
+        }
+
         if (w == 0) {
-            if (lane < nout && out_tail_r != PUB_OUT) { PUB_OUT = out_tail_r; pub64(OTPTR, out_tail_r, sys); }
-            if (lane < n_in2 && in_head_r != PUB_IN) { PUB_IN = in_head_r; pub64(IHPTR, in_head_r, sys); }
+            {
+                const uint32_t dmask = DMASK;
+                const bool dl = lane < nout && ((dmask >> lane) & 1u);
+                const uint64_t ov = out_tail_r | (dl && done_w0 ? kDgClosed : 0ull);
+                if (lane < nout && ov != PUB_OUT) {
+                    PUB_OUT = ov;
+                    uint64_t op = OTPTR;
+                    if constexpr (kDg) op = dl ? t.dg_tail[lane] : op;
+                    pub64(op, ov, sys);
+                }
+                uint64_t g = in_head_r;
+                if constexpr (kDg) {
+                    if (dmask) {
+                        const uint32_t nq = S.d.dq_n;
+                        uint32_t np = 0, e = S.d.dq_h;
+                        g = S.d.gate[lane];
+                        for (; np < nq; np++, e = (e + 1u) % kDq) {
+                            if (__ballot(dl && dgx < S.d.dq_out[e][lane & (kMaxOut - 1)])) break;
+                            g = S.d.dq_in[e][lane];
+                        }
+                        if (np) {
+                            S.d.gate[lane] = g;
+                            if (lane == 0) { S.d.dq_h = e; S.d.dq_n = nq - np; }
+                        }
+                    }
+                    if ((uint32_t)lane < S.d.nhelp) {
+                        const uint64_t hv = S.d.hp_done[lane] - S.d.hp_n[lane];
+                        if (hv != S.d.hp_pub[lane]) {
+                            S.d.hp_pub[lane] = hv;
+                            pub64(t.dh_tail[lane], hv, sys);
+                            pub64(t.dh_done[lane], hv, sys);
+                        }
+                    }
+                }
+                if (lane < n_in2 && g != PUB_IN) { PUB_IN = g; pub64(IHPTR, g, sys); }
+            }
             if (lane < sll && vin_head_r != PUB_VIN) { PUB_VIN = vin_head_r; pub64(VHPTR, vin_head_r, sys); }
             if (lane < n_in) {
                 const uint64_t vt = S.vout_tail[lane];
@@ -1891,7 +2036,7 @@
                 if (lat_ok && S.lat_own_next != 0xffffffffu && rdl32(latr, 1) == S.lat_own_next) { lat_id = S.lat_own_next; C++; }
             }
             uint32_t fastdone = 0;
-            if ((!host || hlim >= 2u) && R == 1u && C == 1u && vtot == 0u && !(PMODE(MODE_PROF | MODE_NOFAST))) {
+            if ((!host || hlim >= 2u) && R == 1u && C == 1u && vtot == 0u && !(PMODE(MODE_PROF | MODE_NOFAST)) && !DMASK) {
                 const int fg = __builtin_ctzll(__ballot(lane < n_in2 && take > 0u));
                 const uint64_t h0 = rdl64(in_head_r, fg);
                 const uint32_t fsrc = (uint32_t)uni((int)t.in_data[fg >> 1][fg & 1]) + (uint32_t)(h0 & fcap_m) * P.fwd_stride;
@@ -2264,7 +2409,7 @@
                 if (bit) {
                     const uint32_t rel = rdl32(pre_r, oi) + (uint32_t)__popcll(b & lt_mask);
                     OL(oi, rel) = (uint16_t)(c | (isbig ? kBigFlag : (nch_s << 9)));
-                    if (isbig) S.pos[c][oi >> 1] = (uint16_t)rel;
+                    if (isbig || (kDg && kind != K_RING && DMASK)) S.pos[c][oi >> 1] = (uint16_t)rel;
                 }
             }
             const uint64_t amask = __ballot(admitted);
@@ -2558,7 +2703,8 @@
             const uint32_t qmagic = nq > 1 ? 0xFFFFFFFFu / nq + 1u : 0u;
             const uint32_t dr = div_small(64u, qmagic), dq = 64u - dr * nq;
             const uint32_t stg_msg = nsmall << 4, stride = P.fwd_stride;
-            const uint32_t nit_r = lane < nout ? S.n_oi[lane] * nq : 0u;
+            const uint32_t dmask = DMASK;
+            const uint32_t nit_r = lane < nout ? S.n_oi[lane] * (((dmask >> lane) & 1u) ? 1u : nq) : 0u;
             uint32_t items = 0;
             const uint32_t ibase_r = wave_excl_scan(nit_r, &items);
             const uint32_t lo = items * (uint32_t)w / (uint32_t)kWaves, hi = items * (uint32_t)(w + 1) / (uint32_t)kWaves;
@@ -2567,6 +2713,16 @@
                 const uint32_t ib = rdl32(ibase_r, oi), ie = ib + rdl32(nit_r, oi);
                 const uint32_t a = max(lo, ib) - ib, b = min(hi, ie) - ib;
                 const uint32_t s0 = (uint32_t)S.out_tail0[oi];
+                if constexpr (kDg) {
+                    if ((dmask >> oi) & 1u) {
+                        const uint32_t doff = (uint32_t)uni((int)t.dg_desc[oi]);
+                        for (uint32_t i = a + (uint32_t)lane; i < b; i += 64u) {
+                            const CandL& cl = S.cand[(uint32_t)OL(oi, i) & 0x1ffu];
+                            st_ring32(rf, doff + 4u * ((s0 + i) & fcap_m), cl.kind == K_RING ? cl.src : ~0u, sys);
+                        }
+                        continue;
+                    }
+                }
                 const __amdgpu_buffer_rsrc_t ro = mk_rsrc(reinterpret_cast<void*>(ORING(oi)), oring_bytes);
                 uint32_t i = a + (uint32_t)lane;
                 uint32_t r = div_small(i, qmagic), q = i - r * nq;
@@ -2596,6 +2752,21 @@
                     r = rr[3] + dr;
                     q = qq[3] + dq;
                     if (q >= nq) { q -= nq; r++; }
+                }
+            }
+            if constexpr (kDg) {
+                if (dmask && nstorm) {
+                    for (uint32_t oc = storm_base + (uint32_t)w; oc < storm_base + nstorm; oc += (uint32_t)kWaves) {
+                        const CandL& cl = S.cand[oc];
+                        const uint32_t och = (kHdr + (cl.w2 & 0xffffu) + 15u) >> 4;
+                        for (uint32_t m = (uint32_t)uni((int)cl.need) & dmask; m; m &= m - 1) {
+                            const int oi = __builtin_ctz(m);
+                            const uint32_t slot = ((uint32_t)S.out_tail0[oi] + S.pos[oc][oi >> 1]) & fcap_m;
+                            const __amdgpu_buffer_rsrc_t ro = mk_rsrc(reinterpret_cast<void*>(ORING(oi)), oring_bytes);
+                            if ((uint32_t)lane < och && och <= nsmall)
+                                st_ring(ro, slot * P.fwd_stride + 16u * (uint32_t)lane, *reinterpret_cast<const u32x4*>(STG(oc, lane)), sys);
+                        }
+                    }
                 }
             }
             if (admitted && !isbig && kind == K_RING && tag == TAG_BCAST) {
@@ -2718,12 +2889,14 @@
         }
         if (w == 0) {
             if constexpr (BULK) flush_posts(S.b, P, lane);
+            bool took = false;
             if (lane < n_in2) {
                 const uint32_t bse = rbase_r, tk = rtake_r, fb = S.first_bad[lane];
                 if (fb < bse + tk) n_stalls++;
                 uint32_t adm = fb == 0xffffffffu ? tk : (fb > bse ? fb - bse : 0u);
                 if (adm > tk) adm = tk;
                 in_head_r += adm;
+                took = adm != 0u;
                 if (adm < tk) win_r = max(adm + adm / 2u, 16u);
                 else if (adm == tk && tk == win_r) win_r = min(2u * win_r, (uint32_t)kMaxCand);
                 if (PMODE(MODE_PROF)) atomicAdd((unsigned long long*)&S.dbg[1], (unsigned long long)adm);
@@ -2736,8 +2909,17 @@
                     if (vt != PUB_VOUT) { PUB_VOUT = vt; pub64(VTPTR, vt, sys); }
                 }
             }
+            if (lane < nout) out_tail_r += noi_r;
+            if constexpr (kDg) {
+                if (S.d.dmask && __ballot(took)) {
+                    const uint32_t qn = S.d.dq_n;
+                    const uint32_t e = (S.d.dq_h + (qn == kDq ? qn - 1u : qn)) % kDq;
+                    if (lane < nout) S.d.dq_out[e][lane] = out_tail_r;
+                    S.d.dq_in[e][lane] = in_head_r;
+                    if (lane == 0 && qn < kDq) S.d.dq_n = qn + 1u;
+                }
+            }
             if (lane < nout) {
-                out_tail_r += noi_r;
                 if (PULL_ON && S.ref_any) {
                     const uint32_t qn = S.rq_n;
                     const uint32_t e = (S.rq_h + (qn == (uint32_t)kRelQ ? qn - 1u : qn)) % (uint32_t)kRelQ;
@@ -2816,6 +2998,7 @@
                     done &= (int64_t)S.own_iter == S.own_n && idle && (int64_t)S.dec_delivered == S.expect_dec;
                 }
                 if (host) done = S.quit != 0;
+                if constexpr (kDg) done &= S.d.nhelp == 0u || S.d.hclosed != 0u;
                 if (S.error == ERR_TIMEOUT) done = true;
                 if (peer_failed) done = true;
                 done_w0 = done;
@@ -2823,6 +3006,7 @@
             done_w0 = __builtin_amdgcn_readfirstlane((int)done_w0) != 0;
             sched_next = (int64_t)uni64((uint64_t)sched_next);
             idle_prev = C == 0 && S.vtot == 0 && !done_w0 && !(PMODE(MODE_NOSPIN));
+            if constexpr (kDg) idle_prev = idle_prev && S.d.hpend == 0u;
         }
         PROF_STAMP(6);
     }
@@ -2837,6 +3021,8 @@
 #undef PUB_OUT
 #undef PUB_VIN
 #undef PUB_VOUT
+#undef DMASK
+#undef NHELP
 
     if constexpr (BULK) {
         if (tid == 0 && !(P.mode & (MODE_PROF | MODE_TL | MODE_HOPPROF))) {
@@ -2879,6 +3065,7 @@
         st.busy_iterations = n_busy;
         st.stalls = S.stalls;
         st.unmarked_slots = S.stale;
+        if constexpr (kDg) st.helper_copies = S.d.copies;
         st.log_count = S.log_count;
         st.t_start = t_start;
         st.t_end = now_ticks();
diff --git a/rootless-coll-mpi-ops_amd/csrc/rlo_kernel_common.hpp b/rootless-coll-mpi-ops_amd/csrc/rlo_kernel_common.hpp
--- a/rootless-coll-mpi-ops_amd/csrc/rlo_kernel_common.hpp
+++ b/rootless-coll-mpi-ops_amd/csrc/rlo_kernel_common.hpp
@@ -92,6 +92,10 @@
 __device__ __forceinline__ void st_ring(__amdgpu_buffer_rsrc_t r, uint32_t off, u32x4 v, bool sys) {
     if (sys) __builtin_amdgcn_raw_buffer_store_b128(v, r, off, 0, kAuxSc1 | 1);
     else __builtin_amdgcn_raw_buffer_store_b128(v, r, off, 0, kAuxSc1);
+}
+__device__ __forceinline__ void st_ring32(__amdgpu_buffer_rsrc_t r, uint32_t off, uint32_t v, bool sys) {
+    if (sys) __builtin_amdgcn_raw_buffer_store_b32(v, r, off, 0, kAuxSc1 | 1);
+    else __builtin_amdgcn_raw_buffer_store_b32(v, r, off, 0, kAuxSc1);
 }
 __device__ __forceinline__ void st_sys16(void* p, u32x4 v) {
     gu64* q = gptr64(reinterpret_cast<uint64_t>(p));
diff --git a/rootless-coll-mpi-ops_amd/csrc/rlo_world.cpp b/rootless-coll-mpi-ops_amd/csrc/rlo_world.cpp
--- a/rootless-coll-mpi-ops_amd/csrc/rlo_world.cpp
+++ b/rootless-coll-mpi-ops_amd/csrc/rlo_world.cpp
@@ -161,7 +161,50 @@
     bool pull = false;
     uint32_t relay_cap = 0;
     std::vector<uint64_t> orig_off;
+    int dg_req = 0;
+    struct DgRing { int src, oi, helper, k; uint64_t desc; };
+    std::vector<DgRing> dg;
+    std::vector<uint32_t> dg_mask, dg_nhelp;
+    int dg_delegators = 0, dg_helpers = 0;
 };
+
+void plan_delegation(Layout& L, int lvl, int edges_max) {
+    const int n = L.n;
+    L.dg.clear();
+    L.dg_mask.assign(n, 0u);
+    L.dg_nhelp.assign(n, 0u);
+    L.dg_delegators = L.dg_helpers = 0;
+    if (lvl < 1 || n < 4) return;
+    std::vector<int> leaves, dels;
+    for (int r = 0; r < n; r++) {
+        if (L.T[r].level == 0) leaves.push_back(r);
+        else if (L.T[r].level >= lvl && 4 * L.T[r].sll + (int)L.in_edges[r].size() <= 64) dels.push_back(r);
+    }
+    if (leaves.empty() || dels.empty()) return;
+    std::stable_sort(dels.begin(), dels.end(), [&](int a, int b) { return L.T[a].level > L.T[b].level; });
+    edges_max = std::min(edges_max, rlo::kMaxHelp / 2);
+    size_t next = 0;
+    for (int d : dels) {
+        for (int j = 0; j < L.T[d].sll; j++) {
+            int h = -1;
+            for (size_t tries = 0; tries < leaves.size() && h < 0; tries++, next = (next + 1) % leaves.size()) {
+                const int c = leaves[next];
+                const uint32_t words = 2u * (uint32_t)L.in_edges[c].size() + (uint32_t)L.T[c].sll + L.dg_nhelp[c] + 2u;
+                if ((int)L.dg_nhelp[c] + 2 <= 2 * edges_max && words <= 64u) h = c;
+            }
+            if (h < 0) continue;
+            for (int vc = 0; vc < 2; vc++) {
+                L.dg.push_back({d, 2 * j + vc, h, (int)L.dg_nhelp[h], 0});
+                L.dg_nhelp[h]++;
+                L.dg_mask[d] |= 1u << (2 * j + vc);
+            }
+        }
+    }
+    for (int r = 0; r < n; r++) {
+        if (L.dg_mask[r]) L.dg_delegators++;
+        if (L.dg_nhelp[r]) L.dg_helpers++;
+    }
+}
 
 int build_layout(int n, int nparts, const int32_t* pb, uint32_t max_payload, uint32_t ring_slots, uint64_t bulk_max,
                  uint32_t bulk_slots, Layout& L) {
@@ -247,6 +290,15 @@
         }
     }
     if (*std::max_element(L.vote_bytes.begin(), L.vote_bytes.end()) > limit) return RLO_E_INVAL;
+    plan_delegation(L, 0, 0);
+    if (L.dg_req > 0 && nparts == 1 && !bulk_max && !L.pull && L.stride <= 8u * 16u) {
+        plan_delegation(L, L.dg_req, rlo::kMaxHelp / 2);
+        if (L.fwd_bytes[0] + (uint64_t)L.dg.size() * cap * 4u > limit) plan_delegation(L, 0, 0);
+        for (auto& g : L.dg) {
+            g.desc = L.fwd_bytes[0];
+            L.fwd_bytes[0] += (uint64_t)cap * 4u;
+        }
+    }
 
     L.ctrl_words.assign(nparts, 0);
     L.lat_base.clear();
@@ -258,9 +310,9 @@
         uint64_t words = rlo::kCtrlHdrWords;
         for (int r = L.pb[p]; r < L.pb[p + 1]; r++) {
             L.inbox[r] = (uint32_t)words;
-            words += (2 * L.in_edges[r].size() + L.T[r].sll + 15) & ~15ull;
+            words += (2 * L.in_edges[r].size() + L.T[r].sll + L.dg_nhelp[r] + 15) & ~15ull;
             L.outbox[r] = (uint32_t)words;
-            words += (2 * L.T[r].sll + L.in_edges[r].size() + 15) & ~15ull;
+            words += (2 * L.T[r].sll + L.in_edges[r].size() + (L.dg_mask[r] ? 2 * L.T[r].sll : 0) + 15) & ~15ull;
         }
         L.lat_base.push_back(words);
         words += rlo::kLatWords;
@@ -672,9 +724,11 @@
         for (int j = 0; j < L.T[r].sll; j++) t.send_list[j] = L.T[r].send_list[j];
         t.n_in = (int)L.in_edges[r].size();
         t.inbox_ctrl = L.inbox[r];
-        t.n_inbox = 2 * t.n_in + t.sll;
+        t.n_inbox = 2 * t.n_in + t.sll + L.dg_nhelp[r];
         t.outbox_ctrl = L.outbox[r];
-        t.n_outbox = 2 * t.sll + t.n_in;
+        t.n_outbox = 2 * t.sll + t.n_in + (L.dg_mask[r] ? 2 * t.sll : 0);
+        t.dg_mask = L.dg_mask[r];
+        t.dg_nhelp = L.dg_nhelp[r];
         t.orig_data = (uint32_t)L.orig_off[r];
         t.in_bell = L.fbell[r];
         t.vin_bell = L.vbell[r];
@@ -705,6 +759,25 @@
             t.vout_bell[ed.k] = (uint64_t)(uintptr_t)(w->pc[ps] + L.vbell[ed.src] + 2 * ed.j);
         }
     }
+    for (const Layout::DgRing& g : L.dg) {
+        rlo::RankTopo& d = w->topo[g.src - w->rb];
+        rlo::RankTopo& h = w->topo[g.helper - w->rb];
+        const uint32_t hin0 = 2u * (uint32_t)L.in_edges[g.helper].size() + (uint32_t)L.T[g.helper].sll;
+        const uint32_t dout0 = 2u * (uint32_t)L.T[g.src].sll + (uint32_t)L.in_edges[g.src].size();
+        d.dg_desc[g.oi] = (uint32_t)g.desc;
+        d.dg_tail[g.oi] = (uint64_t)(uintptr_t)(w->ctrl + L.inbox[g.helper] + hin0 + g.k);
+        h.dh_desc[g.k] = (uint32_t)g.desc;
+        h.dh_ring[g.k] = d.out_ring[g.oi >> 1][g.oi & 1];
+        h.dh_tail[g.k] = d.out_tail[g.oi >> 1][g.oi & 1];
+        h.dh_done[g.k] = (uint64_t)(uintptr_t)(w->ctrl + L.outbox[g.src] + dout0 + g.oi);
+    }
+}
+
+int delegate_env() {
+    const char* e = std::getenv("RLO_DELEGATE");
+    if (!e || !*e || !std::strcmp(e, "auto")) return -1;
+    const int v = std::atoi(e);
+    return v < 0 ? -1 : std::min(v, 16);
 }
 
 }
@@ -777,17 +850,18 @@
         if ((pp & (pp - 1u)) || pp > (uint32_t)rlo::kPoolMax) { delete w; return RLO_E_INVAL; }
         w->L.pend_slots = pp;
     }
+    if (cfg->device >= 0 && hipSetDevice(cfg->device) != hipSuccess) { delete w; return RLO_E_HIP; }
+    (void)hipGetDevice(&w->device);
+    hipDeviceProp_t prop;
+    if (hipGetDeviceProperties(&prop, w->device) != hipSuccess) { delete w; return RLO_E_HIP; }
+    w->cus = prop.multiProcessorCount;
+    w->L.dg_req = (one_xcd || cfg->n_ranks > w->cus) ? 0 : delegate_env();
     int rc = build_layout(cfg->n_ranks, cfg->n_parts, cfg->part_begin, w->max_payload, cfg->ring_slots, cfg->bulk_max,
                           cfg->bulk_slots, w->L);
     if (rc) { delete w; return rc; }
     w->part = cfg->part;
     w->rb = w->L.pb[w->part];
     w->nl = w->L.pb[w->part + 1] - w->rb;
-    if (cfg->device >= 0 && hipSetDevice(cfg->device) != hipSuccess) { delete w; return RLO_E_HIP; }
-    (void)hipGetDevice(&w->device);
-    hipDeviceProp_t prop;
-    if (hipGetDeviceProperties(&prop, w->device) != hipSuccess) { delete w; return RLO_E_HIP; }
-    w->cus = prop.multiProcessorCount;
     if (w->L.bulk_max) {
         int mv = (int)cfg->movers;
         if (mv == 0) mv = std::max(16, w->cus - w->nl) & ~1;
@@ -1204,6 +1278,11 @@
     o->dyn_lds = (uint32_t)w->dyn_lds;
     o->last_kernel = w->last_hop ? 1u : 0u;
     o->static_lds = (uint32_t)rlo_kernel_static_lds(w->variant);
+    if (w->variant == 8) {
+        o->delegators = (uint32_t)w->L.dg_delegators;
+        o->helpers = (uint32_t)w->L.dg_helpers;
+        o->delegated_rings = (uint32_t)w->L.dg.size();
+    }
     return RLO_OK;
 }
 
@@ -1311,6 +1390,7 @@
     if (w->d_sched_off.upload(off) || w->d_sched_ids.upload(ids) || w->d_expect_bcast.upload(expect)) return RLO_E_HIP;
     P.mode = rlo::MODE_STORM | ((cfg->flags & RLO_FLAG_HIST) ? rlo::MODE_HIST : 0u) |
              ((cfg->flags & RLO_FLAG_PROF) ? rlo::MODE_PROF : 0u);
+    if (!w->L.dg.empty() && w->variant == 8 && (rlo::kHdr + hi + 15u) / 16u <= w->nsmall) P.mode |= rlo::MODE_DELEG;
     P.seed = cfg->seed;
     P.len = cfg->len;
     P.len_lo = cfg->len;
@@ -2008,9 +2088,10 @@
     const uint32_t pp = cfg->proposal_pool ? cfg->proposal_pool : 2u;
     if ((pp & (pp - 1u)) || pp > (uint32_t)rlo::kPoolMax) return RLO_E_INVAL;
     L.pend_slots = pp;
+    const int cus = cfg->cus > 0 ? cfg->cus : 256;
+    L.dg_req = ((cfg->flags & RLO_PART_ONE_XCD) || cfg->n_ranks > cus) ? 0 : delegate_env();
     int rc = build_layout(cfg->n_ranks, cfg->n_parts, nullptr, mp, cfg->ring_slots, cfg->bulk_max, cfg->bulk_slots, L);
     if (rc) return rc;
-    const int cus = cfg->cus > 0 ? cfg->cus : 256;
     const int nl = L.pb[cfg->part + 1] - L.pb[cfg->part];
     int nmov = 0;
     if (L.bulk_max) nmov = cfg->movers ? (int)cfg->movers : (std::max(16, cus - nl) & ~1);
@@ -2047,7 +2128,34 @@
     o->pend_hbm = p.pend_hbm ? 1u : 0u;
     o->dyn_lds = (uint32_t)p.dyn_lds;
     o->static_lds = (uint32_t)rlo_kernel_static_lds(p.variant);
-    return RLO_OK;
+    if (p.variant == 8) {
+        o->delegators = (uint32_t)L.dg_delegators;
+        o->helpers = (uint32_t)L.dg_helpers;
+        o->delegated_rings = (uint32_t)L.dg.size();
+    }
+    return RLO_OK;
+}
+
+int rlo_delegate_plan(const rlo_plan_cfg_t* cfg, int32_t level, rlo_deleg_ring_t* out, uint32_t cap, uint32_t* words) {
+    if (!cfg || cfg->n_parts < 1 || cfg->part < 0 || cfg->part >= cfg->n_parts || (cap && !out)) return RLO_E_INVAL;
+    Layout L;
+    const uint32_t mp = (std::max<uint32_t>(cfg->max_payload ? cfg->max_payload : 4096u, 16u) + 15u) & ~15u;
+    if (mp > 65520u) return RLO_E_INVAL;
+    const uint32_t pp = cfg->proposal_pool ? cfg->proposal_pool : 2u;
+    if ((pp & (pp - 1u)) || pp > (uint32_t)rlo::kPoolMax) return RLO_E_INVAL;
+    L.pend_slots = pp;
+    const int cus = cfg->cus > 0 ? cfg->cus : 256;
+    L.dg_req = ((cfg->flags & RLO_PART_ONE_XCD) || cfg->n_ranks > cus) ? 0 : (level < 0 ? -1 : std::min(level, 16));
+    const int rc = build_layout(cfg->n_ranks, cfg->n_parts, nullptr, mp, cfg->ring_slots, cfg->bulk_max, cfg->bulk_slots, L);
+    if (rc) return rc;
+    if (words)
+        for (int r = 0; r < L.n; r++) {
+            words[2 * r] = 2u * (uint32_t)L.in_edges[r].size() + (uint32_t)L.T[r].sll + L.dg_nhelp[r];
+            words[2 * r + 1] = 2u * (uint32_t)L.T[r].sll + (uint32_t)L.in_edges[r].size() + (L.dg_mask[r] ? 2u * L.T[r].sll : 0u);
+        }
+    for (size_t i = 0; i < L.dg.size() && i < cap; i++)
+        out[i] = rlo_deleg_ring_t{L.dg[i].src, L.dg[i].oi, L.dg[i].helper, L.dg[i].k};
+    return (int)L.dg.size();
 }
 
 int rlo_storm_lengths(uint64_t seed, uint64_t k, uint32_t len, uint32_t len_max, uint32_t* out) {
diff --git a/rootless-coll-mpi-ops_amd/rlo/__init__.py b/rootless-coll-mpi-ops_amd/rlo/__init__.py
--- a/rootless-coll-mpi-ops_amd/rlo/__init__.py
+++ b/rootless-coll-mpi-ops_amd/rlo/__init__.py
@@ -1,5 +1,5 @@
 from ._lib import load, RloError, LIB_PATH
-from .world import World, topology, children, hist_percentile, bulk_plan, storm_lengths, layout_plan, pool_trim, pool_stats
+from .world import World, topology, children, hist_percentile, bulk_plan, storm_lengths, layout_plan, delegate_plan, pool_trim, pool_stats
 from . import _lib as abi
 from .host import HostWorld
 
diff --git a/rootless-coll-mpi-ops_amd/rlo/_lib.py b/rootless-coll-mpi-ops_amd/rlo/_lib.py
--- a/rootless-coll-mpi-ops_amd/rlo/_lib.py
+++ b/rootless-coll-mpi-ops_amd/rlo/_lib.py
@@ -25,7 +25,7 @@
 RLO_FLAG_LOG, RLO_FLAG_HIST, RLO_FLAG_PROF, RLO_FLAG_TIMELINE = 1, 2, 4, 8
 RLO_JUDGE_APPROVE, RLO_JUDGE_MASK, RLO_JUDGE_ISP, RLO_JUDGE_HASH = 0, 1, 2, 3
 DERR = {1: "timeout", 2: "vote ring", 3: "pid collision", 4: "vote orphan", 5: "log full", 6: "bad slot", 7: "host command",
-        8: "bulk index"}
+        8: "bulk index", 9: "not on one XCD"}
 RLO_CMD_BCAST, RLO_CMD_PROPOSAL, RLO_CMD_JUDGE, RLO_CMD_OWN_JUDGE, RLO_CMD_QUIT = 0, 2, 16, 17, 18
 RLO_CMD_BULK, RLO_CMD_BULK_RELEASE = 10, 19
 RLO_EV_DELIVER_BCAST, RLO_EV_DELIVER_DECISION, RLO_EV_DELIVER_BULK = 1, 1 | (4 << 8), 1 | (10 << 8)
@@ -51,7 +51,8 @@
                 ("bulk_max", ctypes.c_uint64), ("heap_bytes", ctypes.c_uint64), ("proposal_pool", ctypes.c_uint32),
                 ("pull", ctypes.c_uint32), ("nsmall", ctypes.c_uint32), ("stage2_bytes", ctypes.c_uint32),
                 ("ll_ok", ctypes.c_uint32), ("pend_hbm", ctypes.c_uint32), ("dyn_lds", ctypes.c_uint32),
-                ("static_lds", ctypes.c_uint32), ("last_kernel", ctypes.c_uint32), ("info_pad", ctypes.c_uint32)]
+                ("static_lds", ctypes.c_uint32), ("last_kernel", ctypes.c_uint32), ("delegators", ctypes.c_uint32),
+                ("helpers", ctypes.c_uint32), ("delegated_rings", ctypes.c_uint32)]
 
 
 class PlanCfg(ctypes.Structure):
@@ -97,7 +98,12 @@
         "own_decided", "own_approved", "proposals_recv", "iterations", "busy_iterations", "stalls", "log_count",
         "t_start", "t_end")] + [("error", ctypes.c_uint32), ("error_aux", ctypes.c_uint32), ("prof", ctypes.c_uint64 * 8),
                            ("dbg", ctypes.c_uint64 * 8),
-                           ("hist", ctypes.c_uint32 * 128), ("unmarked_slots", ctypes.c_uint64)]
+                           ("hist", ctypes.c_uint32 * 128), ("unmarked_slots", ctypes.c_uint64),
+                           ("helper_copies", ctypes.c_uint64)]
+
+
+class DelegRing(ctypes.Structure):
+    _fields_ = [("rank", ctypes.c_int32), ("oi", ctypes.c_int32), ("helper", ctypes.c_int32), ("k", ctypes.c_int32)]
 
 
 class BulkPlan(ctypes.Structure):
@@ -117,7 +123,7 @@
            "rlo_last_kernel_ms", "rlo_stats", "rlo_log", "rlo_latencies", "rlo_round_ticks", "rlo_timeline", "rlo_strerror", "rlo_last_hip_error",
            "rlo_device_error", "rlo_bulk_debug",
            "rlo_program_host", "rlo_host_post", "rlo_host_poll", "rlo_host_running", "rlo_host_cmd_count",
-           "rlo_device_count", "rlo_device_numa_node", "rlo_host_bulk_stage", "rlo_host_bulk_copy", "rlo_bulk_plan", "rlo_layout_plan",
+           "rlo_device_count", "rlo_device_numa_node", "rlo_host_bulk_stage", "rlo_host_bulk_copy", "rlo_bulk_plan", "rlo_layout_plan", "rlo_delegate_plan",
            "rlo_storm_lengths", "rlo_host_share", "rlo_host_unlink", "rlo_host_proxy", "rlo_host_wait_started",
            "rlo_host_fail", "rlo_client_attach", "rlo_client_detach", "rlo_client_state", "rlo_client_post",
            "rlo_client_poll", "rlo_client_cmd_count", "rlo_client_bulk_put", "rlo_client_bulk_get", "rlo_client_debug", "rlo_client_hdiag", "rlo_client_fwd", "rlo_host_device_judge",
@@ -175,6 +181,8 @@
     L.rlo_host_bulk_copy.argtypes = [vp, ctypes.c_int, ctypes.POINTER(LogRec), vp]
     L.rlo_bulk_plan.argtypes = [ctypes.c_int, ctypes.c_uint64, ctypes.c_int, ctypes.POINTER(BulkPlan)]
     L.rlo_layout_plan.argtypes = [ctypes.POINTER(PlanCfg), ctypes.POINTER(WorldInfo)]
+    L.rlo_delegate_plan.argtypes = [ctypes.POINTER(PlanCfg), ctypes.c_int32, ctypes.POINTER(DelegRing), ctypes.c_uint32,
+                                    ctypes.POINTER(ctypes.c_uint32)]
     L.rlo_storm_lengths.argtypes = [ctypes.c_uint64, ctypes.c_uint64, ctypes.c_uint32, ctypes.c_uint32,
                                     ctypes.POINTER(ctypes.c_uint32)]
     L.rlo_host_device_judge.argtypes = [vp, ctypes.POINTER(IarCfg)]
diff --git a/rootless-coll-mpi-ops_amd/rlo/world.py b/rootless-coll-mpi-ops_amd/rlo/world.py
--- a/rootless-coll-mpi-ops_amd/rlo/world.py
+++ b/rootless-coll-mpi-ops_amd/rlo/world.py
@@ -267,6 +267,17 @@
     return {f: getattr(out, f) for f, _ in L.WorldInfo._fields_}
 
 
+def delegate_plan(n, level=-1, n_parts=1, part=0, max_payload=64, ring_slots=0, bulk_max=0, flags=0, cus=256):
+    cfg = L.PlanCfg(n, n_parts, part, max_payload, ring_slots, flags, bulk_max, 0, 0, 0, cus)
+    lib = L.load()
+    words = (ctypes.c_uint32 * (2 * n))()
+    cnt = check(lib.rlo_delegate_plan(ctypes.byref(cfg), level, None, 0, words), "rlo_delegate_plan")
+    out = (L.DelegRing * max(cnt, 1))()
+    check(lib.rlo_delegate_plan(ctypes.byref(cfg), level, out, cnt, words), "rlo_delegate_plan")
+    return ([(out[i].rank, out[i].oi, out[i].helper, out[i].k) for i in range(cnt)],
+            [(words[2 * r], words[2 * r + 1]) for r in range(n)])
+
+
 def storm_lengths(seed, k, length, len_max=0):
     out = np.zeros(max(k, 1), dtype=np.uint32)
     check(L.load().rlo_storm_lengths(seed, k, length, len_max, out.ctypes.data_as(ctypes.POINTER(ctypes.c_uint32))),
```

New measurement: 27.34 million msgs/s. 4.6% lower.
